# philgzl/brever

Hardware: AMD Instinct MI355X
Metric: utterances/sec (4 s @16 kHz) Conv-TasNet train (higher is better)
Workload: dtype bf16

## Files before the change

brever_amd/csrc/convtasnet.hip:

```cpp
#include <hip/hip_runtime.h>
#include <stdio.h>
#include <stdlib.h>
#include <string.h>
#include <algorithm>
#include <string>
#include <vector>

#include "../../include/brever_hip.h"
#include "status.h"
#include "ctn_layout.h"
#include "gemm_rows.cuh"
#include "gemm_wgrad.cuh"
#include "gemm_ws.cuh"
#include "dwpw2_fused.cuh"
#include "gemm_wgrad_full.cuh"
#include "gemm_wgrad_full128.cuh"

constexpr int kWgSplit = 4;
#include "prep.cuh"
#include "tcn_kernels.cuh"
#include "bwd_fused.cuh"
#include "pw1_bwd.cuh"
#include "cln_kernels.cuh"

using namespace brv;

namespace {

inline long long align_up(long long x, long long a) { return (x + a - 1)/a*a; }

const brv_launch_opts kDefaultOpts = {sizeof(brv_launch_opts), 0u, 8, 0, nullptr};
thread_local const brv_launch_opts* t_opts = &kDefaultOpts;
struct OptsScope {
  const brv_launch_opts* prev;
  explicit OptsScope(const brv_launch_opts* o) : prev(t_opts) {
    t_opts = (o && o->size >= sizeof(brv_launch_opts)) ? o : &kDefaultOpts;
  }
  ~OptsScope() { t_opts = prev; }
  int check() const {
    const uint32_t unknown = t_opts->flags & ~BRV_OPT_KNOWN;
    if (!unknown) return 0;
    char bits[16]; snprintf(bits, sizeof(bits), "0x%x", unknown);
    return fail(-1, std::string("unknown option bits ") + bits + " in brv_launch_opts.flags");
  }
};
inline bool opt(uint32_t flag) { return (t_opts->flags & flag) != 0; }
inline bool fwd_fuse_requested() { return !opt(BRV_OPT_NO_FWD_FUSE) && !opt(BRV_OPT_NO_WS); }
inline bool bwd_fuse_requested() { return !opt(BRV_OPT_NO_BWD_FUSE); }
inline bool pw1_rc_requested() { return !opt(BRV_OPT_NO_PW1_RC) && !opt(BRV_OPT_NO_DZ1_FUSE); }
inline bool pw1_rc_wgrad() { return opt(BRV_OPT_PW1_RC_WGRAD) || opt(BRV_OPT_PW1_RC_TILES); }

struct ProfEntry { const char* label; hipEvent_t a, b; double flops, bytes; };
struct Prof { std::vector<ProfEntry> entries; bool by_dil; };
struct ProfScope {
  hipStream_t st; Prof* prof;
  ProfScope(const char* label, double flops, double bytes, hipStream_t s)
      : st(s), prof(static_cast<Prof*>(t_opts->prof)) {
    if (!prof) return;
    ProfEntry e; e.label = label; e.flops = flops; e.bytes = bytes;
    (void)hipEventCreate(&e.a); (void)hipEventCreate(&e.b);
    (void)hipEventRecord(e.a, st);
    prof->entries.push_back(e);
  }
  ~ProfScope() { if (prof) (void)hipEventRecord(prof->entries.back().b, st); }
};
inline bool prof_by_dil() { return t_opts->prof && static_cast<Prof*>(t_opts->prof)->by_dil; }

struct BlockOff : CtnBlockOff {
  long long p_c1_f, p_c1_b, p_rs_f, p_rs_b;
  long long p_c1_fp, p_rs_fp, p_rs_bp;
  long long p_rs_g, p_rs_gp, p_lazy;
};

struct Layout : CtnLayout<BlockOff> {
  int Np, Kfp, Bnp, Hp, Scp;
  long long p_enc, p_dec_f, p_dec_b, p_bott_f, p_bott_b, p_out_f, p_out_b, p_stamp, n_prepared;

  bool fusable() const {
    return !causal && P == 3 && H == 512 && Bn == 128 && Sc == 128 && nb <= 24 ;
  }
  bool fused_fwd() const { return fusable() && fwd_fuse_requested(); }
  bool pw1_rc() const { return !causal && Hp == RC_H && Bnp == RC_N && pw1_rc_requested(); }

  static int limits(const brv_ctn_config* c) {
    return c->kernel_size < 1 || c->kernel_size > 5 ? fail(-2, "kernel_size must be in [1, 5] in the HIP path") : 0;
  }
  int init(const brv_ctn_config* c) {
    if (int r = CtnLayout::init(c, limits)) return r;
    Np = round_up(N, 64); Kfp = round_up(K, 64); Bnp = round_up(Bn, 64);
    Hp = round_up(H, 64); Scp = round_up(Sc, 64);
    long long q = 0;
    auto ptake = [&](long long n) { long long r = q; q += align_up(n, 128); return r; };
    p_enc = ptake((long long)Np*Kfp);
    p_dec_f = ptake((long long)Kfp*Np);
    p_dec_b = ptake((long long)Np*Kfp);
    p_bott_f = ptake((long long)Bnp*Np);
    p_bott_b = ptake((long long)Np*Bnp);
    for (int i = 0; i < nb; ++i) {
      const int rs = (i < nb - 1 ? Bnp : 0) + Scp;
      blk[i].p_c1_f = ptake((long long)Hp*Bnp);
      blk[i].p_c1_b = ptake((long long)Bnp*Hp);
      blk[i].p_rs_f = ptake((long long)rs*Hp);
      blk[i].p_rs_b = ptake((long long)Hp*rs);
      blk[i].p_c1_fp = ptake((long long)Hp*Bnp);
      blk[i].p_rs_fp = ptake((long long)rs*Hp);
      blk[i].p_rs_bp = ptake((long long)Hp*rs);
      blk[i].p_rs_g = ptake((long long)(Bnp + Scp)*Hp);
      blk[i].p_rs_gp = ptake((long long)(Bnp + Scp)*Hp);
      blk[i].p_lazy = ptake(4LL*(Bnp + Scp));
    }
    p_out_f = ptake((long long)S*Np*Scp);
    p_out_b = ptake((long long)Scp*S*Np);
    p_stamp = ptake(128);
    n_prepared = q;
    return 0;
  }
};

struct Workspace {
  long long w, x, z1, z2, skip, m, y, stats, sums, dpre, dw1, gskip, gout, eA, eB,
      e0, dwt, vg, gcopy, total;
  long long gcopy_stride, eB_stride;
  long long wgpart;
  long long h1, h2, wn, ctab, ctab_stride, cfs, cbt, ident, fake_stats, scratch_stats;
  long long vg_stride, vg_bytes;
  long long x_stride, z_stride;
  long long u, u_stride;
  long long stamp;
  long long stats_bytes;
  void init(const Layout& l, long long B, long long T) {
    long long o = 0;
    auto take = [&](long long bytes) { long long r = o; o += align_up(bytes, 256); return r; };
    const long long BT = B*T;
    w = take(BT*l.Np*2);
    x_stride = align_up(BT*l.Bnp*2, 256);
    x = take(x_stride*l.nb);
    z_stride = align_up(BT*l.Hp*2, 256);
    z1 = take(z_stride*l.nb);
    z2 = take(z_stride*l.nb);
    skip = take(BT*l.Scp*4);
    m = take(BT*l.S*l.Np*2);
    y = take(BT*l.S*l.Np*2);
    stats_bytes = (long long)(1 + 2*l.nb)*B*kStatStride*8;
    stats = take(stats_bytes);
    sums = take(stats_bytes);
    dpre = take(BT*l.S*l.Np*2);
    dw1 = take(BT*l.S*l.Np*2);
    gout = take(BT*(l.Bnp + l.Scp)*2);
    gskip = gout + (long long)l.Bnp*2;
    eA = take(BT*l.Hp*2);
    eB_stride = align_up(BT*l.Hp*2, 256);
    eB = take(eB_stride*l.nb);
    gcopy_stride = align_up(BT*l.Bnp*2, 256);
    gcopy = take(gcopy_stride*l.nb);
    e0 = take(BT*l.Np*2);
    dwt = take(BT*l.Np*2);
    vg_stride = align_up(2LL*l.N + (long long)l.nb*l.H*(5 + l.P) + 1 + 2*l.nb + 2LL*l.Hp, 64);
    vg_bytes = vg_stride*kReplicas*4;
    vg = take(vg_bytes);
    wgpart = take((long long)2*kWgSplit*l.nb*W2_G*l.H*4);
    u_stride = align_up(BT*(l.Bnp + l.Scp)*2, 256);
    u = l.fusable() ? take(u_stride*l.nb) : 0;
    stamp = take(256);
    h1 = h2 = wn = ctab = cfs = cbt = ident = fake_stats = scratch_stats = 0; ctab_stride = 0;
    if (l.causal) {
      h1 = take(z_stride*l.nb);
      h2 = take(z_stride*l.nb);
      wn = take(BT*l.Np*2);
      ctab_stride = align_up(BT*2*4, 256);
      ctab = take(ctab_stride*(1 + 2*l.nb));
      cfs = take(BT*2*4);
      cbt = take(BT*2*4);
      const long long cmax = l.Hp > l.Np ? l.Hp : l.Np;
      ident = take((2*cmax + 64)*4);
      fake_stats = take(B*kStatStride*8);
      scratch_stats = take(B*kStatStride*8);
    }
    total = o;
  }
};

struct Views {
  const Layout& l; Workspace ws; char* base; const bf16_t* prep; int B; long long T;
  Views(const Layout& l_, void* workspace, const void* prepared, int B_, long long T_)
      : l(l_), base((char*)workspace), prep((const bf16_t*)prepared), B(B_), T(T_) { ws.init(l, B, T); }
  double BT() const { return (double)B*(double)T; }
  int ldg() const { return l.Bnp + l.Scp; }
  bf16_t* bf(long long off) const { return (bf16_t*)(base + off); }
  float* f32(long long off) const { return (float*)(base + off); }
  double* stat(int i) const { return (double*)(base + ws.stats) + (long long)i*B*kStatStride; }
  double* sum(int i) const { return (double*)(base + ws.sums) + (long long)i*B*kStatStride; }
  bf16_t* w() const { return bf(ws.w); }
  bf16_t* x(int i) const { return bf(ws.x + ws.x_stride*i); }
  bf16_t* z1(int i) const { return bf(ws.z1 + ws.z_stride*i); }
  bf16_t* z2(int i) const { return bf(ws.z2 + ws.z_stride*i); }
  bf16_t* u(int i) const { return bf(ws.u + ws.u_stride*i); }
  float* skip() const { return f32(ws.skip); }
  bf16_t* m() const { return bf(ws.m); }
  bf16_t* y() const { return bf(ws.y); }
  bf16_t* dpre() const { return bf(ws.dpre); }
  bf16_t* dw1() const { return bf(ws.dw1); }
  bf16_t* gskip() const { return bf(ws.gskip); }
  bf16_t* gout() const { return bf(ws.gout); }
  bf16_t* eA() const { return bf(ws.eA); }
  bf16_t* eB(int i) const { return bf(ws.eB + ws.eB_stride*i); }
  bf16_t* gcopy(int i) const { return bf(ws.gcopy + ws.gcopy_stride*i); }
  bf16_t* e0() const { return bf(ws.e0); }
  bf16_t* dwt() const { return bf(ws.dwt); }
  float* vg() const { return f32(ws.vg); }
  float* vslot(int i) const { return vg() + 2LL*l.N + (long long)l.H*(5 + l.P)*i; }
  float* vslope() const { return vslot(l.nb); }
  float* vscratch() const { return vslope() + 1 + 2*l.nb; }
  bf16_t* wn() const { return bf(ws.wn); }
  bf16_t* h1(int i) const { return bf(ws.h1 + ws.z_stride*i); }
  bf16_t* h2(int i) const { return bf(ws.h2 + ws.z_stride*i); }
  long long cmax() const { return l.Hp > l.Np ? l.Hp : l.Np; }
  float* ones() const { return f32(ws.ident); }
  float* zeros() const { return ones() + cmax(); }
  float* one() const { return zeros() + cmax(); }
  double* fake_stats() const { return (double*)(base + ws.fake_stats); }
  double* scratch_stats() const { return (double*)(base + ws.scratch_stats); }
  float* cfs() const { return f32(ws.cfs); }
  float* cbt() const { return f32(ws.cbt); }
  float* tab(int i) const { return f32(ws.ctab + ws.ctab_stride*i); }
};

template <int BN, int AK, int EM>
int launch_gemm_rows_t(const GemmRowsParams& p0, int batch, hipStream_t st) {
  GemmRowsParams p = p0;
  p.n_ttiles = ceil_div(p.T, GR_BM); p.n_ntiles = ceil_div(p.Np, BN); p.batch = batch;
  dim3 grid(p.n_ttiles*p.n_ntiles*batch);
  hipLaunchKernelGGL((gemm_rows_kernel<BN, AK, EM>), grid, dim3(256), 0, st, p);
  BRV_HIP_OK(hipGetLastError());
  return 0;
}

#ifdef BRV_DIAG
__global__ void diag_stamp_kernel(long long* out, int slot) {
  const long long t = stamp_realtime();
  if (threadIdx.x == 0) {
    out[slot] = t;
    if (slot == 0) { out[2] = 0x7fffffffffffffffLL; out[3] = 0; }
  }
}
long long* debug_buffer() {
  static long long* buf = nullptr;
  if (!buf) {
    if (hipMalloc(&buf, 1 << 20) != hipSuccess) return nullptr;
    (void)hipMemset(buf, 0, 1 << 20);
  }
  return buf;
}
#endif

inline int mode_stamp(bool fused_fwd) { return fused_fwd ? 0x46555345 : 0x504c4149; }
__global__ void stamp_write_kernel(int* dst, int value) { *dst = value; }
__global__ void stamp_check_f64_kernel(const int* stamp, int expect, double* poison, long long n) {
  if (*stamp == expect) return;
  const double nan = __longlong_as_double(0x7ff8000000000000LL);
  for (long long i = threadIdx.x; i < n; i += blockDim.x) poison[i] = nan;
}
struct CallInitParams {
  double* a; long long a_n; void* b; long long b_bytes;
  const int* check; int expect; int* write; int value;
};
__global__ __launch_bounds__(256) void call_init_kernel(const CallInitParams p) {
  const bool bad = *p.check != p.expect;
  const double fill = bad ? __longlong_as_double(0x7ff8000000000000LL) : 0.0;
  const long long tid = (long long)blockIdx.x*256 + threadIdx.x, nth = (long long)gridDim.x*256;
  for (long long i = tid; i < p.a_n; i += nth) p.a[i] = fill;
  if (p.b) {
    unsigned char* b = (unsigned char*)p.b;
    long long head = (16 - ((unsigned long long)b & 15)) & 15;
    if (head > p.b_bytes) head = p.b_bytes;
    const long long n16 = (p.b_bytes - head) >> 4, tail0 = head + (n16 << 4);
    uint4* mid = reinterpret_cast<uint4*>(b + head);
    const uint4 z = make_uint4(0, 0, 0, 0);
    for (long long i = tid; i < n16; i += nth) mid[i] = z;
    for (long long i = tid*4; i < head; i += nth*4) *reinterpret_cast<unsigned int*>(b + i) = 0u;
    for (long long i = tail0 + tid*4; i < p.b_bytes; i += nth*4) *reinterpret_cast<unsigned int*>(b + i) = 0u;
  }
  if (tid == 0 && p.write) *p.write = p.value;
}
inline int launch_call_init(double* a, long long a_n, void* b, long long b_bytes, const int* check, int expect,
                            int* write, int value, hipStream_t st) {
  CallInitParams ip; ip.a = a; ip.a_n = a_n; ip.b = b; ip.b_bytes = b_bytes; ip.check = check; ip.expect = expect;
  ip.write = write; ip.value = value;
  const long long units = a_n + (b_bytes >> 4);
  int gx = (int)std::min<long long>(512, (units + 1023)/1024);
  if (gx < 1) gx = 1;
  hipLaunchKernelGGL(call_init_kernel, dim3(gx), dim3(256), 0, st, ip);
  BRV_HIP_OK(hipGetLastError());
  return 0;
}

int device_cus() {
  static const int n = [] {
    int dev = 0, v = 0;
    if (hipGetDevice(&dev) != hipSuccess ||
        hipDeviceGetAttribute(&v, hipDeviceAttributeMultiprocessorCount, dev) != hipSuccess || v <= 0)
      v = 256;
    return v;
  }();
  return n;
}
int num_cus() {
  const int n = device_cus();
  const int e = t_opts->cu_eighths >= 1 && t_opts->cu_eighths <= 8 ? t_opts->cu_eighths : 8;
  const int m = n*e/8/8*8;
  return m >= 8 ? m : n;
}

template <int KP, int NSL, int WM, int EM, int AT, bool CAT, int NW = 8>
int launch_gemm_ws(const GemmRowsParams& p0, int batch, hipStream_t st) {
  using C = GemmWsCfg<KP, NSL, WM, NW>;
  GemmRowsParams p = p0;
  p.batch = batch;
#ifdef BRV_DIAG
  if (const char* d = getenv("BRV_DBG")) p.dbg = atoi(d);
  if (p.dbg & (64 | 512)) p.dbg_out = debug_buffer();
#endif
  if (!CAT && p.a.K0 <= 0) {
    p.a.p0 = p.a.p1; p.a.ld0 = p.a.ld1; p.a.bs0 = p.a.bs1; p.a.K0 = 1 << 30;
  }
  const int total = ceil_div(p.T, C::BMW)*batch;
  const int groups = p.Np / C::NP;
  int grid = (NW == 8 ? num_cus() : 2*num_cus())/groups;
  if (grid > total) grid = total;
  if (grid < 1) grid = 1;
#ifdef BRV_DIAG
  if (p.dbg & 512) hipLaunchKernelGGL(diag_stamp_kernel, dim3(1), dim3(64), 0, st, debug_buffer() + 131000, 0);
#endif
  hipLaunchKernelGGL((gemm_ws_kernel<KP, NSL, WM, EM, AT, CAT, NW>), dim3(grid, groups),
                     dim3(64*NW), 0, st, p);
#ifdef BRV_DIAG
  if (p.dbg & 512) hipLaunchKernelGGL(diag_stamp_kernel, dim3(1), dim3(64), 0, st, debug_buffer() + 131000, 1);
#endif
  BRV_HIP_OK(hipGetLastError());
  return 0;
}

template <int AK, int EM>
int launch_gemm_rows(const GemmRowsParams& p, int batch, hipStream_t st,
                     const char* label = "gemm_rows", double bytes = 0) {
  if (p.T <= 0 || batch <= 0) return 0;
  ProfScope prof(label, 2.0*batch*p.T*(double)p.Np*p.Kp, bytes, st);
  if (AK == A_BF16 && p.a.nsrc <= 1 && !opt(BRV_OPT_NO_WS)) {
    const bool plain = p.a.slope == nullptr && p.a.stats == nullptr;
    const bool full = p.a.slope != nullptr && p.a.stats != nullptr;
    const bool one_src = p.a.K0 >= p.Kp || p.a.K0 <= 0;
    if ((EM == E_STORE || EM == E_GLN_BWD) && p.Kp == 128 && p.Np == 512 && plain && one_src)
      return launch_gemm_ws<128, 64, 1, (EM == E_STORE ? E_STORE : E_GLN_BWD), 0, false, 8>(p, batch, st);
    if (EM == E_RES_SKIP && p.Kp == 512 && p.Np == 256 && full && one_src)
      return launch_gemm_ws<512, 32, 1, E_RES_SKIP, 1, false>(p, batch, st);
    if (EM == E_GLN_BWD && p.Kp == 256 && p.Np == 512 && plain && one_src)
      return launch_gemm_ws<256, 32, 1, E_GLN_BWD, 0, false, 8>(p, batch, st);
  }
  if (p.Kp % GR_BK != 0 || p.Np % 64 != 0) return fail(-1, "gemm_rows: unpadded dims");
  if (p.Np % 128 == 0) return launch_gemm_rows_t<128, AK, EM>(p, batch, st);
  return launch_gemm_rows_t<64, AK, EM>(p, batch, st);
}

inline int wgrad_target(const char* label, int dflt) {
  (void)label;
  return t_opts->wg_target != 0 ? t_opts->wg_target : dflt;
}

template <int BH, int HK>
int launch_wgrad_t(WgradGroupParams& gp, hipStream_t st, int target) {
  WgradParams& p = gp.base;
  const int nprob = gp.nprob > 0 ? gp.nprob : 1;
  const int tiles = ceil_div(p.Gp, WG_BG)*(p.Hp/BH);
  const int total = p.B*ceil_div(p.T, WG_BT);
  int ns = ceil_div(target > 0 ? target : 384, tiles*nprob);
  if (target < 0) {
    int nb = p.B;
    while (tiles*nprob*nb > 2048 && nb % 2 == 0) nb /= 2;
    if (nb > ns) ns = nb;
  }
  if (ns > total) ns = total;
  if (ns < 1) ns = 1;
  p.nsplit = ns;
  dim3 grid(tiles, ns, nprob);
  hipLaunchKernelGGL((gemm_wgrad_kernel<BH, HK>), grid, dim3(256), 0, st, gp);
  BRV_HIP_OK(hipGetLastError());
  return 0;
}
template <int HK>
int launch_wgrad_group(WgradGroupParams& gp, hipStream_t st, const char* label,
                       double bytes, int target_dflt = 384) {
  const WgradParams& p = gp.base;
  if (p.T <= 0 || p.B <= 0) return 0;
  const int nprob = gp.nprob > 0 ? gp.nprob : 1;
  ProfScope prof(label, 2.0*nprob*p.B*p.T*(double)p.Gp*p.Hp, bytes*nprob, st);
  if (p.Hp % 64 != 0) return fail(-1, "wgrad: unpadded dims");
  const int target = wgrad_target(label, target_dflt);
  if (p.Hp % 128 == 0) return launch_wgrad_t<128, HK>(gp, st, target);
  return launch_wgrad_t<64, HK>(gp, st, target);
}
template <int HK>
int launch_wgrad(WgradParams& p, hipStream_t st, const char* label = "wgrad",
                 double bytes = 0, int target_dflt = 384) {
  WgradGroupParams gp;
  gp.base = p; gp.nprob = 0;
  return launch_wgrad_group<HK>(gp, st, label, bytes, target_dflt);
}

template <template <int> class F, typename... Args>
int dispatch_p(int P, Args&&... args) {
  switch (P) {
    case 1: return F<1>::run(args...);
    case 2: return F<2>::run(args...);
    case 3: return F<3>::run(args...);
    case 4: return F<4>::run(args...);
    case 5: return F<5>::run(args...);
  }
  return fail(-2, "unsupported kernel_size");
}
template <int P> struct DwFwd {
  static int run(const DwParams& p, hipStream_t st) {
    ProfScope prof("dwconv_fwd", 2.0*P*p.B*p.T*(double)p.Cp, 4.0*p.B*p.T*(double)p.Cp, st);
    dim3 grid(ceil_div(p.T, DW_TT_F)*p.B);
    hipLaunchKernelGGL((dwconv_fwd_kernel<P>), grid, dim3(256), 0, st, p);
    BRV_HIP_OK(hipGetLastError());
    return 0;
  }
};
template <int P> struct DwBwd {
  static int run(const DwParams& p, hipStream_t st) {
    if (p.z2in != nullptr) {
      static const char* by_dil[9] = {"dwconv_bwd_d1", "dwconv_bwd_d2", "dwconv_bwd_d4", "dwconv_bwd_d8", "dwconv_bwd_d16",
                                      "dwconv_bwd_d32", "dwconv_bwd_d64", "dwconv_bwd_d128", "dwconv_bwd_dx"};
      int lg = 0; while ((1 << lg) < p.dil && lg < 8) ++lg;
      ProfScope prof(prof_by_dil() ? by_dil[lg] : "dwconv_bwd", 4.0*P*p.B*p.T*(double)p.Cp, 8.0*p.B*p.T*(double)p.Cp, st);
      const int R = hl_rows_per_tooth(p.dil), K = HL_TT/R;
      const int tiles = ceil_div(p.dil, R)*ceil_div((p.T - 1)/p.dil + 1, K);
      dim3 grid(tiles*p.B*(p.Cp/HL_CG));
      const size_t lds = (size_t)hl_window_rows(p.dil, P)*HL_CG*2;
      hipLaunchKernelGGL((dwconv_bwd_halo_kernel<P>), grid, dim3(256), lds, st, p);
      BRV_HIP_OK(hipGetLastError());
      return 0;
    }
    ProfScope prof("dwconv_bwd", 4.0*P*p.B*p.T*(double)p.Cp, 6.0*p.B*p.T*(double)p.Cp, st);
    dim3 grid(ceil_div(p.T, DW_TT_B)*p.B);
    hipLaunchKernelGGL((dwconv_bwd_kernel<P>), grid, dim3(256), 0, st, p);
    BRV_HIP_OK(hipGetLastError());
    return 0;
  }
};

template <int P> struct DwBwdFused {
  static int run(const BwdFusedParams& p0, hipStream_t st) {
    BwdFusedParams p = p0;
    const DwParams& d = p.d;
#ifdef BF_STAMP
    p.dbg = debug_buffer();
#endif
    bf_tile_shape(d.T, d.dil, P, p.K, p.R);
    const int tiles = ceil_div(d.dil, p.R)*ceil_div((d.T - 1)/d.dil + 1, p.K);
    static const char* by_dil[9] = {"dwpw2_bwd_d1", "dwpw2_bwd_d2", "dwpw2_bwd_d4", "dwpw2_bwd_d8", "dwpw2_bwd_d16",
                                    "dwpw2_bwd_d32", "dwpw2_bwd_d64", "dwpw2_bwd_d128", "dwpw2_bwd_dx"};
    int lg = 0; while ((1 << lg) < d.dil && lg < 8) ++lg;
    ProfScope prof(prof_by_dil() ? by_dil[lg] : "dwpw2_bwd", 2.0*d.B*d.T*(double)d.Cp*(p.Kg + 2*P),
                   2.0*d.B*d.T*((double)p.Kg + 3.0*d.Cp), st);
    dim3 grid(ceil_div(tiles*d.B, 8)*8*(d.Cp/HL_CG));
    if (d.C != d.Cp) return fail(-1, "fused backward: channel count must be a multiple of 64");
    if (p.Kg == 256) hipLaunchKernelGGL((dwconv_bwd_fused_kernel<P, 256>), grid, dim3(256), BF_LDS, st, p);
    else if (p.Kg == 128) hipLaunchKernelGGL((dwconv_bwd_fused_kernel<P, 128>), grid, dim3(256), BF_LDS, st, p);
    else return fail(-1, "fused backward: unexpected [res | skip] width");
    BRV_HIP_OK(hipGetLastError());
    return 0;
  }
};

int launch_dz(const DzParams& p, hipStream_t st) {
  ProfScope prof("gln_prelu_bwd", 0, 6.0*p.B*p.T*(double)p.Cp, st);
  const long long per_item = (long long)p.T*(p.Cp/8);
  int gx = (int)((per_item + 256*8 - 1)/(256*8));
  const int cap = 1024/p.B > 1 ? 1024/p.B : 1;
  if (gx > cap) gx = cap;
  if (gx < 1) gx = 1;
  hipLaunchKernelGGL(dz_kernel, dim3(gx, p.B), dim3(256), 0, st, p);
  BRV_HIP_OK(hipGetLastError());
  return 0;
}

ASpec rows_bf16(const void* ptr, int ld, long long T) {
  ASpec a; memset(&a, 0, sizeof(a));
  a.p0 = ptr; a.ld0 = ld; a.bs0 = T*ld; a.K0 = 1 << 30; a.nsrc = 1;
  return a;
}
void set_affine(ASpec& a, const double* stats, const float* g, const float* b, int C,
                long long T) {
  a.stats = stats; a.gamma = g; a.beta = b; a.C = C;
  a.inv_n = 1.0/((double)T*(double)C); a.eps = 1e-8f;
}
ASpec frames_of(const float* wav, long long L, int hop, int K, long long stride = 0) {
  ASpec a; memset(&a, 0, sizeof(a));
  a.p0 = wav; a.hop = hop; a.Kf = K; a.wav_stride = stride > 0 ? stride : L; a.wav_len = (int)L;
  a.K0 = 1 << 30; a.nsrc = 1;
  return a;
}

struct PrepJobC { int src_off, dst_off, scale_off; unsigned short R, C, rows, cols, dst_ld, tr; };
constexpr int kPrepBatch = 168;
struct PrepBatch { PrepJobC jobs[kPrepBatch]; int n; };
static_assert(sizeof(PrepBatch) <= 4096, "kernel argument size");

struct PackJob { long long src_off, dst_off; int N, K, nsl; };
struct PackBatch { PackJob jobs[96]; int n; };
__global__ __launch_bounds__(256) void pack_frag_kernel(bf16_t* prepared, const PackBatch pb) {
  const PackJob j = pb.jobs[blockIdx.y];
  const long long total = (long long)j.N*j.K/8;
  const int KS = j.K/16;
  for (long long i = (long long)blockIdx.x*256 + threadIdx.x; i < total; i += (long long)gridDim.x*256) {
    const int n = (int)(i / (j.K/8)), k = (int)(i % (j.K/8))*8;
    const int slice = n / j.nsl, f = (n % j.nsl)/32, fr = n % 32, s = k/16, fh = (k % 16)/8;
    const long long dst = (long long)slice*j.nsl*j.K + ((long long)(f*KS + s)*64 + fr + 32*fh)*8;
    *reinterpret_cast<uint4*>(prepared + j.dst_off + dst) =
        *reinterpret_cast<const uint4*>(prepared + j.src_off + (long long)n*j.K + k);
  }
}
__global__ __launch_bounds__(256) void prep_weights_kernel(const float* params,
                                                           bf16_t* prepped,
                                                           const PrepBatch pb) {
  const PrepJobC& c = pb.jobs[blockIdx.y];
  PrepJob j;
  j.src_off = c.src_off; j.dst_off = c.dst_off; j.scale_off = c.scale_off;
  j.R = c.R; j.C = c.C; j.rows = c.rows; j.cols = c.cols; j.dst_ld = c.dst_ld; j.tr = c.tr;
  prep_job_run(params, prepped, j, blockIdx.x, gridDim.x);
}

struct LazyPrepBlk { long long res_w, res_b, skip_w, skip_b, beta, wg, out; };
struct LazyPrepParams {
  int nb, H, Hp, Bn, Sc, Bnp, Scp;
  int* stamp; int stamp_value;
  LazyPrepBlk blk[kWgMaxProb];
};
__global__ __launch_bounds__(256) void lazy_prep_kernel(const float* params, bf16_t* prepped,
                                                        const LazyPrepParams p) {
  const LazyPrepBlk& b = p.blk[blockIdx.y];
  float* out = reinterpret_cast<float*>(prepped + b.out);
  const int NP = p.Bnp + p.Scp;
  const int n = blockIdx.x*4 + (threadIdx.x >> 6), lane = threadIdx.x & 63;
  if (blockIdx.x == 0 && blockIdx.y == 0 && threadIdx.x == 0) *p.stamp = p.stamp_value;
  if (n >= NP) return;
  const bool res = n < p.Bnp;
  const int r = res ? n : n - p.Bnp;
  const bool ok = res ? (r < p.Bn && b.res_w >= 0) : r < p.Sc;
  float v0 = 0.f, v1 = 0.f;
  if (ok) {
    const float* W = params + (res ? b.res_w : b.skip_w) + (long long)r*p.H;
    const bf16_t* wg = prepped + b.wg + (long long)n*p.Hp;
    for (int k = lane; k < p.H; k += 64) {
      v0 = __builtin_fmaf(W[k], params[b.beta + k], v0);
      v1 += bf2f(wg[k]);
    }
  }
  for (int o = 32; o; o >>= 1) { v0 += __shfl_xor(v0, o); v1 += __shfl_xor(v1, o); }
  if (lane == 0) {
    out[n] = ok ? v0 + params[(res ? b.res_b : b.skip_b) + r] : 0.f;
    out[NP + n] = v1;
  }
}

struct SkipCombineParams {
  const bf16_t* u; long long u_stride;
  const double* stats; long long stats_stride;
  const bf16_t* prepared; long long lazy_off[kWgMaxProb];
  float* skip; int nb, B, T, Bnp, Scp; double inv_n; float eps;
};
__global__ __launch_bounds__(256) void skip_combine_kernel(const SkipCombineParams p) {
  __shared__ float rs[kWgMaxProb];
  __shared__ float cs[128];
  const int b = blockIdx.y, tid = threadIdx.x;
  const int NP = p.Bnp + p.Scp;
  __shared__ float ms[kWgMaxProb];
  for (int i = tid; i < p.nb; i += 256) {
    const NormStat ns = norm_stat(p.stats + (2 + 2*i)*p.stats_stride, b, p.inv_n, p.eps);
    rs[i] = ns.rstd; ms[i] = ns.mean*ns.rstd;
  }
  __syncthreads();
  for (int n = tid; n < p.Scp; n += 256) {
    float c = 0.f;
    int i = 0;
    for (; i + 8 <= p.nb; i += 8) {
      float a[8], v[8];
#pragma unroll
      for (int k = 0; k < 8; ++k) {
        const float* lz = reinterpret_cast<const float*>(p.prepared + p.lazy_off[i + k]);
        a[k] = lz[p.Bnp + n]; v[k] = lz[NP + p.Bnp + n];
      }
#pragma unroll
      for (int k = 0; k < 8; ++k) c += a[k] - ms[i + k]*v[k];
    }
    for (; i < p.nb; ++i) {
      const float* lz = reinterpret_cast<const float*>(p.prepared + p.lazy_off[i]);
      c += lz[p.Bnp + n] - ms[i]*lz[NP + p.Bnp + n];
    }
    cs[n] = c;
  }
  __syncthreads();
  const int cpr = p.Scp/8;
  const long long per_item = (long long)p.T*cpr;
  for (long long e = (long long)blockIdx.x*256 + tid; e < per_item; e += (long long)gridDim.x*256) {
    const int c0 = (int)(e % cpr)*8; const long long t = e / cpr;
    float acc[8];
#pragma unroll
    for (int j = 0; j < 8; ++j) acc[j] = cs[c0 + j];
    const bf16_t* src = p.u + ((long long)b*p.T + t)*NP + p.Bnp + c0;
    int i = 0;
    for (; i + 8 <= p.nb; i += 8) {
      uint4 q[8];
#pragma unroll
      for (int k = 0; k < 8; ++k) q[k] = *reinterpret_cast<const uint4*>(src + (i + k)*p.u_stride);
#pragma unroll
      for (int k = 0; k < 8; ++k) {
        float f[8];
        unpack8(q[k], f);
        const float r = rs[i + k];
#pragma unroll
        for (int j = 0; j < 8; ++j) acc[j] = __builtin_fmaf(r, f[j], acc[j]);
      }
    }
    for (; i < p.nb; ++i) {
      float f[8];
      unpack8(*reinterpret_cast<const uint4*>(src + i*p.u_stride), f);
      const float r = rs[i];
#pragma unroll
      for (int j = 0; j < 8; ++j) acc[j] = __builtin_fmaf(r, f[j], acc[j]);
    }
    float* dst = p.skip + ((long long)b*p.T + t)*p.Scp + c0;
    *reinterpret_cast<float4*>(dst) = make_float4(acc[0], acc[1], acc[2], acc[3]);
    *reinterpret_cast<float4*>(dst + 4) = make_float4(acc[4], acc[5], acc[6], acc[7]);
  }
}

}

int reduce_vector_grads(const Views& v, float* grads, hipStream_t st, int blk_lo = 0, int blk_hi = 1 << 30,
                        bool do_ln = true, bool do_tcn = true) {
  const Layout& l = v.l;
  const long long vper = (long long)l.H*(5 + l.P);
  {
    VgradParams vp; memset(&vp, 0, sizeof(vp));
    vp.vg = v.vg(); vp.grads = grads; vp.rep_stride = v.ws.vg_stride;
    vp.N = l.N; vp.H = l.H; vp.P = l.P; vp.nb = l.nb;
    vp.ln_g_off = l.ln_g; vp.blk0_off = l.blk[0].conv_w;
    vp.blk_full = l.nb > 1 ? l.blk[1].conv_w - l.blk[0].conv_w : 0;
    const BlockOff& b0 = l.blk[0];
    const BlockOff& bl = l.blk[l.nb - 1];
    vp.o_dconv_w = b0.dconv_w - b0.conv_w; vp.o_dconv_b = b0.dconv_b - b0.conv_w;
    vp.o_n1_g_full = b0.n1_g - b0.conv_w; vp.o_n1_g_last = bl.n1_g - bl.conv_w;
    vp.tcn_prelu_off = l.tcn_prelu;
    vp.blk_lo = blk_lo; vp.blk_hi = blk_hi; vp.do_ln = do_ln; vp.do_tcn = do_tcn;
    if (b0.prelu1 != b0.n1_g + 4LL*l.H || b0.prelu2 != b0.prelu1 + 1)
      return fail(-1, "vgrad_reduce: unexpected PReLU offsets");
    const long long total = 2LL*l.N + vper*l.nb + 1 + 2*l.nb;
    int gx = (int)((total + 255)/256);
    if (gx > 1024) gx = 1024;
    ProfScope prof("vgrad_reduce", 0, 4.0*total*(kReplicas + 2), st);
    hipLaunchKernelGGL(vgrad_reduce_kernel, dim3(gx), dim3(256), 0, st, vp);
    BRV_HIP_OK(hipGetLastError());
  }
  return 0;
}

__global__ void fill_identity_kernel(float* ones, float* zeros, float* one, int n,
                                     double* fake_stats, int B, double sumsq) {
  const int i = blockIdx.x*256 + threadIdx.x;
  if (i < n) { ones[i] = 1.f; zeros[i] = 0.f; }
  if (i == 0) *one = 1.f;
  if (i < B) { fake_stats[stat_sum(i)] = 0.0; fake_stats[stat_sq(i)] = sumsq; }
}

namespace {

int causal_init(const Views& v, hipStream_t st) {
  const Layout& l = v.l;
  const double sumsq = (1.0 - (double)1e-8f)*(double)v.T*(double)l.H;
  const int cmax = (int)v.cmax(), n = cmax > v.B ? cmax : v.B;
  hipLaunchKernelGGL(fill_identity_kernel, dim3((n + 255)/256), dim3(256), 0, st, v.ones(), v.zeros(),
                     v.one(), cmax, v.fake_stats(), v.B, sumsq);
  BRV_HIP_OK(hipGetLastError());
  BRV_HIP_OK(hipMemsetAsync(v.scratch_stats(), 0, (size_t)v.B*kStatStride*8, st));
  return 0;
}

int cln_forward(const Views& v, const bf16_t* z, const float* slope, const float* gain,
                const float* bias, bf16_t* y, float* table, int B, long long T, int Cp, int C,
                hipStream_t st) {
  ClnParams p; memset(&p, 0, sizeof(p));
  p.z = z; p.slope = slope; p.y = y; p.fsum = v.cfs(); p.table = table; p.gain = gain;
  p.bias = bias; p.B = B; p.T = (int)T; p.Cp = Cp; p.C = C; p.eps = 1e-8f;
  ProfScope prof("cln_fwd", 0, 6.0*B*T*(double)Cp, st);
  hipLaunchKernelGGL(cln_frame_sums_kernel, dim3(ceil_div((int)T, CLN_FPB)*B), dim3(256), 0, st, p);
  hipLaunchKernelGGL(cln_scan_kernel, dim3(B), dim3(256), 0, st, p);
  int gx = (int)(((long long)B*T*(Cp/8) + 255)/256);
  if (gx > 4096) gx = 4096;
  hipLaunchKernelGGL(cln_apply_kernel, dim3(gx), dim3(256), 0, st, p);
  BRV_HIP_OK(hipGetLastError());
  return 0;
}

int cln_backward(const Views& v, const bf16_t* g, const bf16_t* z, const float* slope,
                 const float* gain, const float* fwd_table, bf16_t* dz, const bf16_t* add_in,
                 int n_add, float* dgain, float* dbias, float* dslope, long long rep_stride,
                 int B, long long T, int Cp, int C, hipStream_t st) {
  ClnParams p; memset(&p, 0, sizeof(p));
  p.z = z; p.slope = slope; p.g = g; p.fsum = v.cfs(); p.table = v.cbt(); p.fwd_table = fwd_table;
  p.gain = gain; p.B = B; p.T = (int)T; p.Cp = Cp; p.C = C; p.eps = 1e-8f;
  p.dz = dz; p.add_in = add_in; p.n_add = n_add;
  p.dgain = dgain; p.dbias = dbias; p.dslope = dslope; p.rep_stride = rep_stride;
  ProfScope prof("cln_bwd", 0, 10.0*B*T*(double)Cp, st);
  hipLaunchKernelGGL(cln_bwd_sums_kernel, dim3(ceil_div((int)T, CLN_FPB)*B), dim3(256), 0, st, p);
  hipLaunchKernelGGL(cln_bwd_scan_kernel, dim3(B), dim3(256), 0, st, p);
  int gx = (int)(((long long)B*T*(Cp/8) + 255)/256);
  if (gx > 2048) gx = 2048;
  hipLaunchKernelGGL(cln_bwd_apply_kernel, dim3(gx), dim3(256), 0, st, p);
  BRV_HIP_OK(hipGetLastError());
  return 0;
}

int forward_encoder(const Views& v, const float* params, const float* wave, long long wave_stride, float* out,
                    long long L, hipStream_t st) {
  const Layout& l = v.l; const int B = v.B; const long long T = v.T; const double BT = v.BT();
  if (int r = launch_call_init(v.stat(0), (long long)(v.ws.stats_bytes/8), out, (long long)B*l.S*L*(long long)sizeof(float),
                               reinterpret_cast<const int*>(v.prep + l.p_stamp), mode_stamp(l.fused_fwd()),
                               reinterpret_cast<int*>(v.base + v.ws.stamp), mode_stamp(l.fused_fwd()), st))
    return fail(r, "forward: call_init launch");

  GemmRowsParams g;
  memset(&g, 0, sizeof(g));
  g.a = frames_of(wave, L, l.hop, l.K, wave_stride);
  g.W = v.prep + l.p_enc; g.T = (int)T; g.Np = l.Np; g.Kp = l.Kfp;
  g.e.out = v.w(); g.e.ldo = l.Np; g.e.N = l.N; g.e.stats_out = v.stat(0);
  if (int r = launch_gemm_rows<A_FRAMES, E_STORE>(g, B, st, "enc_fwd", 4.0*B*L + 2.0*BT*l.Np)) return r;
  memset(&g, 0, sizeof(g));
  g.a = rows_bf16(v.w(), l.Np, T);
  set_affine(g.a, v.stat(0), params + l.ln_g, params + l.ln_b, l.N, T);
  g.W = v.prep + l.p_bott_f; g.T = (int)T; g.Np = l.Bnp; g.Kp = l.Np;
  g.e.out = v.x(0); g.e.ldo = l.Bnp; g.e.bias = params + l.bott_b; g.e.N = l.Bn;
  if (int r = launch_gemm_rows<A_BF16, E_STORE>(g, B, st, "bottleneck_fwd", 2.0*BT*(l.Np + l.Bnp))) return r;
  return 0;
}

int forward_block_fused(const Views& v, const float* params, int i, hipStream_t st) {
  const Layout& l = v.l; const int B = v.B; const long long T = v.T; const double BT = v.BT();
  const int NPu = l.Bnp + l.Scp;
  GemmRowsParams g;
  const BlockOff& b = l.blk[i];
  const int dil = 1 << (i % l.layers);
  memset(&g, 0, sizeof(g));
  g.W = v.prep + b.p_c1_f; g.T = (int)T; g.Np = l.Hp; g.Kp = l.Bnp;
  g.Wp = v.prep + b.p_c1_fp; g.wp_nsl = 64;
  g.e.out = v.z1(i); g.e.ldo = l.Hp; g.e.bias = params + b.conv_b; g.e.N = l.H;
  g.e.stats_out = v.stat(1 + 2*i); g.e.stats_slope = params + b.prelu1;
  if (i == 0) {
    g.a = rows_bf16(v.x(0), l.Bnp, T);
    ProfScope prof("pw1_fwd", 2.0*BT*l.Hp*l.Bnp, 2.0*BT*(l.Bnp + l.Hp), st);
    if (int r = launch_gemm_ws<128, 64, 1, E_STORE, 0, false, 8>(g, B, st)) return r;
  } else {
    const BlockOff& pb = l.blk[i - 1];
    g.a = rows_bf16(v.x(i - 1), l.Bnp, T);
    g.a.p1 = v.u(i - 1); g.a.ld1 = NPu; g.a.bs1 = T*NPu;
    g.a.xout = v.x(i);
    g.a.stats = v.stat(2 + 2*(i - 1)); g.a.inv_n = 1.0/((double)T*l.H); g.a.eps = 1e-8f;
    const float* lz = reinterpret_cast<const float*>(v.prep + pb.p_lazy);
    g.a.lazy_v0 = lz; g.a.lazy_v1 = lz + NPu;
    ProfScope prof("pw1_fwd", 2.0*BT*l.Hp*l.Bnp, 2.0*BT*(3*l.Bnp + l.Hp), st);
#ifndef PW1F_NSL
#define PW1F_NSL 64
#define PW1F_WM 1
#endif
    if (int r = launch_gemm_ws<128, PW1F_NSL, PW1F_WM, E_STORE, 2, false, 8>(g, B, st)) return r;
  }
  memset(&g, 0, sizeof(g));
  g.a = rows_bf16(v.z1(i), l.Hp, T);
  g.a.slope = params + b.prelu1; g.a.stats = v.stat(1 + 2*i);
  g.a.gamma = params + b.n1_g; g.a.beta = params + b.n1_b; g.a.C = l.H;
  g.a.inv_n = 1.0/((double)T*l.H); g.a.eps = 1e-8f;
  g.a.z2out = v.z2(i); g.a.taps = params + b.dconv_w; g.a.dbias = params + b.dconv_b;
  g.a.slope2 = params + b.prelu2; g.a.stats2_out = v.stat(2 + 2*i);
  g.a.dil = dil; g.a.left = ((l.P - 1)*dil)/2;
  g.W = v.prep + b.p_rs_g; g.Wp = v.prep + b.p_rs_gp; g.wp_nsl = 32;
  g.T = (int)T; g.Np = NPu; g.Kp = l.Hp;
  g.e.out = v.u(i); g.e.ldo = NPu; g.e.N = NPu;
  {
    ProfScope prof("dwpw2_fwd", 2.0*BT*l.Hp*(NPu + l.P), 2.0*BT*(2*l.Hp + NPu), st);
    const bool old_stage = opt(BRV_OPT_DWPW2_WS);
    if (old_stage || l.Hp != DP_H || NPu != DP_N) {
      if (int r = launch_gemm_ws<512, 32, 1, E_STORE, 3, false, 8>(g, B, st)) return r;
    } else {
      DwPw2Params dp; memset(&dp, 0, sizeof(dp));
      dp.z1 = v.z1(i); dp.z2 = v.z2(i); dp.u = v.u(i);
      dp.Wp = v.prep + b.p_rs_gp;
      dp.slope1 = params + b.prelu1; dp.slope2 = params + b.prelu2;
      dp.stats1 = v.stat(1 + 2*i); dp.stats2 = v.stat(2 + 2*i);
      dp.gamma1 = params + b.n1_g; dp.beta1 = params + b.n1_b;
      dp.taps = params + b.dconv_w; dp.dbias = params + b.dconv_b;
      dp.B = B; dp.T = (int)T; dp.dil = dil; dp.left = ((l.P - 1)*dil)/2; dp.C = l.H;
      dp.inv_n = 1.0/((double)T*l.H); dp.eps = 1e-8f;
      const int n_tiles = B*(int)((T + DP_TT - 1)/DP_TT);
      const int cap = num_cus() >= 8 ? num_cus()/8*8 : 8;
      const int n_wg = n_tiles < cap ? (n_tiles + 7)/8*8 : cap;
      hipLaunchKernelGGL(dwpw2_fused_kernel, dim3(n_wg), dim3(512), 0, st, dp);
      BRV_HIP_OK(hipGetLastError());
    }
  }
  return 0;
}

int forward_skip_combine(const Views& v, hipStream_t st) {
  const Layout& l = v.l; const int B = v.B; const long long T = v.T; const double BT = v.BT();
  SkipCombineParams sc; memset(&sc, 0, sizeof(sc));
  sc.u = v.u(0); sc.u_stride = v.ws.u_stride/2; sc.stats = v.stat(0); sc.stats_stride = (long long)B*kStatStride;
  sc.prepared = v.prep; sc.skip = v.skip(); sc.nb = l.nb; sc.B = B; sc.T = (int)T; sc.Bnp = l.Bnp; sc.Scp = l.Scp;
  sc.inv_n = 1.0/((double)T*l.H); sc.eps = 1e-8f;
  for (int i = 0; i < l.nb; ++i) sc.lazy_off[i] = l.blk[i].p_lazy;
  {
    ProfScope prof("skip_combine", 0, 2.0*BT*l.Scp*l.nb + 4.0*BT*l.Scp, st);
    int gx = (int)((T*(l.Scp/8) + 255)/256);
    if (gx > 128) gx = 128;
    hipLaunchKernelGGL(skip_combine_kernel, dim3(gx, B), dim3(256), 0, st, sc);
    BRV_HIP_OK(hipGetLastError());
  }
  return 0;
}

int forward_block_plain(const Views& v, const float* params, int i, hipStream_t st) {
  const Layout& l = v.l; const int B = v.B; const long long T = v.T; const double BT = v.BT();
  GemmRowsParams g;
  const BlockOff& b = l.blk[i];
  const bool has_res = i < l.nb - 1;
  const int dil = 1 << (i % l.layers);
  memset(&g, 0, sizeof(g));
  g.a = rows_bf16(v.x(i), l.Bnp, T);
  g.W = v.prep + b.p_c1_f; g.T = (int)T; g.Np = l.Hp; g.Kp = l.Bnp;
  g.Wp = v.prep + b.p_c1_fp; g.wp_nsl = 64;
  g.e.out = v.z1(i); g.e.ldo = l.Hp; g.e.bias = params + b.conv_b; g.e.N = l.H;
  g.e.stats_out = v.stat(1 + 2*i); g.e.stats_slope = params + b.prelu1;
  if (int r = launch_gemm_rows<A_BF16, E_STORE>(g, B, st, "pw1_fwd", 2.0*BT*(l.Bnp + l.Hp))) return r;
  DwParams d; memset(&d, 0, sizeof(d));
  d.z1 = v.z1(i); d.z2 = v.z2(i); d.B = B; d.T = (int)T; d.Cp = l.Hp; d.C = l.H;
  d.slope1 = params + b.prelu1; d.stats1 = v.stat(1 + 2*i);
  d.gamma1 = params + b.n1_g; d.beta1 = params + b.n1_b;
  d.inv_n = 1.0/((double)T*l.H); d.eps = 1e-8f;
  d.taps = params + b.dconv_w; d.bias = params + b.dconv_b;
  d.dil = dil; d.left = ((l.P - 1)*dil)/2;
  d.stats2 = v.stat(2 + 2*i); d.slope2 = params + b.prelu2;
  if (int r = dispatch_p<DwFwd>(l.P, d, st)) return r;
  memset(&g, 0, sizeof(g));
  g.a = rows_bf16(v.z2(i), l.Hp, T);
  g.a.slope = params + b.prelu2;
  set_affine(g.a, v.stat(2 + 2*i), params + b.n2_g, params + b.n2_b, l.H, T);
  const int rs0 = has_res ? l.Bnp : 0;
  g.W = v.prep + b.p_rs_f; g.T = (int)T; g.Np = rs0 + l.Scp; g.Kp = l.Hp;
  g.Wp = v.prep + b.p_rs_fp; g.wp_nsl = 32;
  g.e.out = has_res ? v.x(i + 1) : nullptr; g.e.ldo = l.Bnp;
  g.e.bias = has_res ? params + b.res_b : nullptr; g.e.N = has_res ? l.Bn : 0;
  g.e.Nsplit = rs0; g.e.bias2 = params + b.skip_b; g.e.N2 = l.Sc;
  g.e.res_in = v.x(i); g.e.ld_res = l.Bnp;
  g.e.skip = v.skip(); g.e.ld_skip = l.Scp; g.e.skip_init = (i == 0);
  if (int r = launch_gemm_rows<A_BF16, E_RES_SKIP>(g, B, st, "pw2_fwd", 2.0*BT*(l.Hp + l.Bnp + rs0) + 4.0*BT*l.Scp*(i == 0 ? 1 : 2))) return r;
  return 0;
}

int forward_decoder(const Views& v, const float* params, float* out, long long L, hipStream_t st) {
  const Layout& l = v.l; const int B = v.B; const long long T = v.T; const double BT = v.BT();
  GemmRowsParams g;
  memset(&g, 0, sizeof(g));
  g.a = rows_bf16(v.skip(), l.Scp, T);
  g.a.slope = params + l.tcn_prelu;
  g.W = v.prep + l.p_out_f; g.T = (int)T; g.Np = l.S*l.Np; g.Kp = l.Scp;
  g.e.out = v.y(); g.e.ldo = l.Np; g.e.bias = params + l.out_b; g.e.N = l.N;
  g.e.w_in = v.w(); g.e.ld_w = l.Np; g.e.m_out = v.m(); g.e.S = l.S; g.e.Np_src = l.Np;
  if (int r = launch_gemm_rows<A_F32, E_MASK>(g, B, st, "mask_fwd", 4.0*BT*l.Scp + 2.0*BT*l.Np*(1 + 2*l.S))) return r;
  memset(&g, 0, sizeof(g));
  g.a = rows_bf16(v.y(), l.Np, T);
  g.W = v.prep + l.p_dec_f; g.T = (int)T; g.Np = l.Kfp; g.Kp = l.Np;
  g.e.wave_out = out; g.e.hop = l.hop; g.e.Kf = l.K; g.e.wave_stride = L;
  g.e.wave_len = (int)L;
  if (int r = launch_gemm_rows<A_BF16, E_OLA>(g, B*l.S, st, "dec_fwd", 2.0*BT*l.S*l.Np + 4.0*B*l.S*L)) return r;
  return 0;
}

int forward_causal(const Views& v, const float* params, const float* wave, long long wave_stride, float* out,
                   long long L, hipStream_t st) {
  const Layout& l = v.l; const int B = v.B; const long long T = v.T; const double BT = v.BT();
  if (int r = causal_init(v, st)) return r;
  BRV_HIP_OK(hipMemsetAsync(out, 0, (size_t)B*l.S*L*sizeof(float), st));

  GemmRowsParams g;
  memset(&g, 0, sizeof(g));
  g.a = frames_of(wave, L, l.hop, l.K, wave_stride);
  g.W = v.prep + l.p_enc; g.T = (int)T; g.Np = l.Np; g.Kp = l.Kfp;
  g.e.out = v.w(); g.e.ldo = l.Np; g.e.N = l.N;
  if (int r = launch_gemm_rows<A_FRAMES, E_STORE>(g, B, st, "enc_fwd", 4.0*B*L + 2.0*BT*l.Np)) return r;
  if (int r = cln_forward(v, v.w(), nullptr, params + l.ln_g, params + l.ln_b, v.wn(), v.tab(0), B, T,
                          l.Np, l.N, st)) return r;
  memset(&g, 0, sizeof(g));
  g.a = rows_bf16(v.wn(), l.Np, T);
  g.W = v.prep + l.p_bott_f; g.T = (int)T; g.Np = l.Bnp; g.Kp = l.Np;
  g.e.out = v.x(0); g.e.ldo = l.Bnp; g.e.bias = params + l.bott_b; g.e.N = l.Bn;
  if (int r = launch_gemm_rows<A_BF16, E_STORE>(g, B, st, "bottleneck_fwd", 2.0*BT*(l.Np + l.Bnp))) return r;

  for (int i = 0; i < l.nb; ++i) {
    const BlockOff& b = l.blk[i];
    const bool has_res = i < l.nb - 1;
    const int dil = 1 << (i % l.layers);
    memset(&g, 0, sizeof(g));
    g.a = rows_bf16(v.x(i), l.Bnp, T);
    g.W = v.prep + b.p_c1_f; g.T = (int)T; g.Np = l.Hp; g.Kp = l.Bnp;
    g.e.out = v.z1(i); g.e.ldo = l.Hp; g.e.bias = params + b.conv_b; g.e.N = l.H;
    if (int r = launch_gemm_rows<A_BF16, E_STORE>(g, B, st, "pw1_fwd", 2.0*BT*(l.Bnp + l.Hp))) return r;
    if (int r = cln_forward(v, v.z1(i), params + b.prelu1, params + b.n1_g, params + b.n1_b,
                            v.h1(i), v.tab(1 + 2*i), B, T, l.Hp, l.H, st)) return r;
    DwParams d; memset(&d, 0, sizeof(d));
    d.z1 = v.h1(i); d.z2 = v.z2(i); d.B = B; d.T = (int)T; d.Cp = l.Hp; d.C = l.H;
    d.slope1 = v.one(); d.stats1 = v.fake_stats(); d.gamma1 = v.ones(); d.beta1 = v.zeros();
    d.inv_n = 1.0/((double)T*l.H); d.eps = 1e-8f;
    d.taps = params + b.dconv_w; d.bias = params + b.dconv_b;
    d.dil = dil; d.left = (l.P - 1)*dil;
    d.stats2 = v.scratch_stats(); d.slope2 = v.one();
    if (int r = dispatch_p<DwFwd>(l.P, d, st)) return r;
    if (int r = cln_forward(v, v.z2(i), params + b.prelu2, params + b.n2_g, params + b.n2_b,
                            v.h2(i), v.tab(2 + 2*i), B, T, l.Hp, l.H, st)) return r;
    memset(&g, 0, sizeof(g));
    g.a = rows_bf16(v.h2(i), l.Hp, T);
    const int rs0 = has_res ? l.Bnp : 0;
    g.W = v.prep + b.p_rs_f; g.T = (int)T; g.Np = rs0 + l.Scp; g.Kp = l.Hp;
    g.e.out = has_res ? v.x(i + 1) : nullptr; g.e.ldo = l.Bnp;
    g.e.bias = has_res ? params + b.res_b : nullptr; g.e.N = has_res ? l.Bn : 0;
    g.e.Nsplit = rs0; g.e.bias2 = params + b.skip_b; g.e.N2 = l.Sc;
    g.e.res_in = v.x(i); g.e.ld_res = l.Bnp;
    g.e.skip = v.skip(); g.e.ld_skip = l.Scp; g.e.skip_init = (i == 0);
    if (int r = launch_gemm_rows<A_BF16, E_RES_SKIP>(g, B, st, "pw2_fwd", 2.0*BT*(l.Hp + l.Bnp + rs0) + 4.0*BT*l.Scp*(i == 0 ? 1 : 2))) return r;
  }
  return forward_decoder(v, params, out, L, st);
}

void wgrad_rs_prob(const Views& v, const float* params, float* grads, int i, WgradProb& pr) {
  const BlockOff& b = v.l.blk[i];
  const bool has_res = i < v.l.nb - 1;
  pr.g0 = has_res ? v.gcopy(i) : nullptr; pr.g1 = v.gskip(); pr.h = v.z2(i);
  pr.out0 = has_res ? grads + b.res_w : nullptr; pr.out1 = grads + b.skip_w;
  pr.gbias0 = has_res ? grads + b.res_b : nullptr; pr.gbias1 = grads + b.skip_b;
  pr.slope = params + b.prelu2; pr.stats = v.stat(2 + 2*i);
  pr.gamma = params + b.n2_g; pr.beta = params + b.n2_b;
}

int wgrad_rs_full(const Views& v, const float* params, float* grads, int blk_lo, int blk_hi, hipStream_t st) {
  const Layout& l = v.l; const int B = v.B; const long long T = v.T; const double BT = v.BT();
  const int ldg = v.ldg();
  WgradFullParams fp; memset(&fp, 0, sizeof(fp));
  const int nblk = blk_hi - blk_lo + 1;
  fp.B = B; fp.T = (int)T; fp.nprob = nblk; fp.n_htiles = l.Hp/W2_BH;
  fp.ldg0 = l.Bnp; fp.bsg0 = T*l.Bnp; fp.ldg1 = ldg; fp.bsg1 = T*ldg;
  fp.ldh = l.Hp; fp.bsh = T*l.Hp;
  fp.N0 = l.Bn; fp.N1 = l.Sc; fp.Kout = l.H; fp.ldo = l.H;
  fp.inv_n = 1.0/((double)T*l.H); fp.eps = 1e-8f;
  for (int i = blk_lo; i <= blk_hi; ++i) wgrad_rs_prob(v, params, grads, i, fp.prob[i - blk_lo]);
  ProfScope prof("pw2_wgrad", 2.0*nblk*BT*(double)(l.Bnp + l.Scp)*l.Hp,
                 2.0*BT*(l.Bnp + l.Scp + l.Hp)*nblk, st);
#ifdef BRV_DIAG
  if (const char* d = getenv("BRV_DBG_WG")) fp.dbg = atoi(d);
#endif
  fp.n_split = (B >= kWgSplit && !opt(BRV_OPT_NO_WGRAD_SPLIT)) ? kWgSplit : 1;
  fp.part = reinterpret_cast<float*>(v.base + v.ws.wgpart);
  const bool wide = !opt(BRV_OPT_NO_WGRAD_128) && l.Hp % W3_BH == 0;
  if (wide) {
    fp.n_htiles = l.Hp/W3_BH;
    if (fp.n_split > 1 && B >= 4*kWgSplit) fp.n_split = 2*kWgSplit;
    const int grid = 8*ceil_div(nblk, 8)*fp.n_htiles*fp.n_split;
    hipLaunchKernelGGL(wgrad_full128_kernel, dim3(grid), dim3(64*W2_NW), 0, st, fp);
  } else {
    const int grid = 8*ceil_div(nblk, 8)*fp.n_htiles*fp.n_split;
    hipLaunchKernelGGL(wgrad_full_kernel, dim3(grid), dim3(64*W2_NW), 0, st, fp);
  }
  if (fp.n_split > 1)
    hipLaunchKernelGGL(wgrad_full_reduce_kernel, dim3(128, (unsigned)nblk), dim3(256), 0, st, fp);
  BRV_HIP_OK(hipGetLastError());
  return 0;
}

int wgrad_rs_grouped(const Views& v, const float* params, float* grads, int i0, int n, hipStream_t st) {
  const Layout& l = v.l; const int B = v.B; const long long T = v.T; const double BT = v.BT();
  const int ldg = v.ldg(); WgradParams wg;
  WgradGroupParams gp; memset(&gp, 0, sizeof(gp));
  WgradParams& q = gp.base;
  q.g = rows_bf16(nullptr, l.Bnp, T); q.g.K0 = l.Bnp;
  q.g.ld1 = ldg; q.g.bs1 = T*ldg;
  q.h = rows_bf16(nullptr, l.Hp, T);
  set_affine(q.h, nullptr, nullptr, nullptr, l.H, T);
  q.B = B; q.T = (int)T; q.Gp = l.Bnp + l.Scp; q.Hp = l.Hp;
  q.G0p = l.Bnp; q.N0 = l.Bn; q.N1 = l.Sc; q.Kout = l.H; q.ldo = l.H;
  int np = 0;
  for (int i = i0; i < i0 + n; ++i)
    if (i != l.nb - 1) wgrad_rs_prob(v, params, grads, i, gp.prob[np++]);
  gp.nprob = np;
  if (np > 0)
    if (int r = launch_wgrad_group<A_BF16>(gp, st, "pw2_wgrad",
                                           2.0*BT*(l.Bnp + l.Scp + l.Hp))) return r;
  if (i0 + n == l.nb) {
    const BlockOff& b = l.blk[l.nb - 1];
    memset(&wg, 0, sizeof(wg));
    wg.g = rows_bf16(v.gskip(), ldg, T);
    wg.h = rows_bf16(v.z2(l.nb - 1), l.Hp, T); wg.h.slope = params + b.prelu2;
    set_affine(wg.h, v.stat(2 + 2*(l.nb - 1)), params + b.n2_g, params + b.n2_b, l.H, T);
    wg.B = B; wg.T = (int)T; wg.Gp = l.Scp; wg.Hp = l.Hp;
    wg.out1 = grads + b.skip_w; wg.G0p = 0; wg.N0 = 0; wg.N1 = l.Sc;
    wg.Kout = l.H; wg.ldo = l.H; wg.gbias1 = grads + b.skip_b;
    if (int r = launch_wgrad<A_BF16>(wg, st, "pw2_wgrad", 2.0*BT*(l.Scp + l.Hp))) return r;
  }
  return 0;
}

int wgrad_pw1(const Views& v, const float* params, float* grads, int i0, int n, hipStream_t st) {
  const Layout& l = v.l; const int B = v.B; const long long T = v.T; const double BT = v.BT();
  WgradGroupParams gp;
  memset(&gp, 0, sizeof(gp));
  WgradParams& q1 = gp.base;
  q1.g = rows_bf16(nullptr, l.Hp, T); q1.h = rows_bf16(nullptr, l.Bnp, T);
  q1.B = B; q1.T = (int)T; q1.Gp = l.Hp; q1.Hp = l.Bnp;
  q1.G0p = l.Hp; q1.N0 = l.H; q1.Kout = l.Bn; q1.ldo = l.Bn;
  for (int i = i0; i < i0 + n; ++i) {
    const BlockOff& b = l.blk[i];
    WgradProb& pr = gp.prob[i - i0];
    pr.g0 = v.eB(i); pr.h = v.x(i);
    pr.out0 = grads + b.conv_w; pr.gbias0 = grads + b.conv_b;
  }
  gp.nprob = n;
  if (l.pw1_rc() && pw1_rc_wgrad()) {
    Pw1WgradRcParams rp; memset(&rp, 0, sizeof(rp));
    rp.B = B; rp.T = (int)T; rp.nprob = n; rp.C = l.H; rp.Kout = l.Bn; rp.ldo = l.Bn;
    rp.lde = l.Hp; rp.ldx = l.Bnp; rp.bse = T*l.Hp; rp.bsx = T*l.Bnp;
    rp.inv_n = 1.0/((double)T*l.H); rp.eps = 1e-8f;
    for (int i = i0; i < i0 + n; ++i) {
      const BlockOff& b = l.blk[i];
      Pw1WgradRcProb& pr = rp.prob[i - i0];
      pr.e1 = v.eB(i); pr.x = v.x(i); pr.Wfp = v.prep + b.p_c1_fp; pr.bias = params + b.conv_b;
      pr.out = grads + b.conv_w; pr.gbias = grads + b.conv_b;
      pr.stats = v.stat(1 + 2*i); pr.sums = v.sum(1 + 2*i); pr.slope = params + b.prelu1;
    }
    const int tiles = l.Hp/WG_BG;
    int ns = B;
    while (tiles*n*ns > 2048 && ns % 2 == 0) ns /= 2;
    if (t_opts->wg_target > 0) ns = ceil_div(t_opts->wg_target, tiles*n);
    const int total = B*ceil_div((int)T, WG_BT);
    if (ns > total) ns = total;
    if (ns < 1) ns = 1;
    rp.nsplit = ns;
    ProfScope prof("pw1_wgrad", 2.0*n*BT*(double)l.Hp*l.Bnp*2, 2.0*BT*(l.Hp + l.Bnp)*n, st);
    hipLaunchKernelGGL(pw1_wgrad_rc_kernel, dim3(tiles, ns, n), dim3(256), 0, st, rp);
    BRV_HIP_OK(hipGetLastError());
  }
  else
  if (int r = launch_wgrad_group<A_BF16>(gp, st, "pw1_wgrad", 2.0*BT*(l.Hp + l.Bnp), -1))
    return r;
  return 0;
}

int deferred_wgrads(const Views& v, const float* params, float* grads, int blk_lo, int blk_hi, hipStream_t st) {
  const Layout& l = v.l;
  const bool full_rs = l.Bnp == 128 && l.Scp == 128 && l.Hp % W2_BH == 0 && l.nb <= kWgMaxProb &&
                       !opt(BRV_OPT_NO_WGRAD_FULL);
  if (full_rs && blk_lo <= blk_hi)
    if (int r = wgrad_rs_full(v, params, grads, blk_lo, blk_hi, st)) return r;
  for (int i0 = blk_lo; i0 <= blk_hi; i0 += kWgMaxProb) {
    const int n = std::min(kWgMaxProb, blk_hi + 1 - i0);
    if (!full_rs)
      if (int r = wgrad_rs_grouped(v, params, grads, i0, n, st)) return r;
    if (int r = wgrad_pw1(v, params, grads, i0, n, st)) return r;
  }
  return 0;
}

int backward_head(const Views& v, const float* params, const float* d_out, float* grads, long long L,
                  bool bwd_fused, hipStream_t st) {
  const Layout& l = v.l; const int B = v.B; const long long T = v.T; const double BT = v.BT();
  const int BS = B*l.S, ldg = v.ldg(); GemmRowsParams g; WgradParams wg;
  if (!l.causal)
    if (int r = launch_call_init(v.sum(0), (long long)(v.ws.stats_bytes/8), v.vg(), (long long)v.ws.vg_bytes,
                                 reinterpret_cast<const int*>(v.base + v.ws.stamp), mode_stamp(l.fused_fwd()), nullptr, 0, st))
      return fail(r, "backward: call_init launch");
  memset(&g, 0, sizeof(g));
  g.a = frames_of(d_out, L, l.hop, l.K);
  g.W = v.prep + l.p_dec_b; g.T = (int)T; g.Np = l.Np; g.Kp = l.Kfp;
  g.e.out = v.dpre(); g.e.ldo = l.Np; g.e.out2 = v.dw1(); g.e.w_in = v.w(); g.e.ld_w = l.Np;
  g.e.m_in = v.m(); g.e.S = l.S;
  if (int r = launch_gemm_rows<A_FRAMES, E_MASK_BWD>(g, BS, st, "dec_bwd", 4.0*BS*L + 2.0*BT*l.Np*(1 + 3*l.S))) return r;
  memset(&wg, 0, sizeof(wg));
  wg.g = rows_bf16(v.y(), l.Np, T); wg.h = frames_of(d_out, L, l.hop, l.K);
  wg.B = BS; wg.T = (int)T; wg.Gp = l.Np; wg.Hp = l.Kfp;
  wg.out0 = grads + l.dec_w; wg.G0p = l.Np; wg.N0 = l.N; wg.Kout = l.K; wg.ldo = l.K;
  if (int r = launch_wgrad<A_FRAMES>(wg, st, "wgrad_dec", 2.0*BT*l.S*l.Np + 4.0*BS*L, l.causal ? 384 : 768)) return r;
  memset(&g, 0, sizeof(g));
  g.a = rows_bf16(v.dpre(), l.Np, T); g.a.nsrc = l.S;
  g.W = v.prep + l.p_out_b; g.T = (int)T; g.Np = l.Scp; g.Kp = l.S*l.Np;
  g.e.out = v.gskip(); g.e.ldo = ldg; g.e.src_f32 = v.skip(); g.e.ld_srcf = l.Scp;
  g.e.src_slope = params + l.tcn_prelu; g.e.dslope = v.vslope();
  g.e.rep_stride = v.ws.vg_stride; g.e.n_rep = kReplicas;
  if (int r = launch_gemm_rows<A_BF16, E_PRELU_BWD>(g, B, st, "mask_bwd", 2.0*BT*l.S*l.Np + 6.0*BT*l.Scp)) return r;
  if (bwd_fused) {
    GuDotsParams gu; memset(&gu, 0, sizeof(gu));
    gu.g = v.gskip(); gu.ldg = ldg; gu.u = v.u(l.nb - 1) + l.Bnp; gu.ldu = ldg;
    gu.v1 = reinterpret_cast<const float*>(v.prep + l.blk[l.nb - 1].p_lazy) + ldg + l.Bnp;
    gu.ncols = l.Scp; gu.B = B; gu.T = (int)T; gu.out = v.sum(2 + 2*(l.nb - 1));
    ProfScope prof("gu_dots", 0, 4.0*BT*l.Scp, st);
    int gx = (int)((T*(l.Scp/8) + 255)/256);
    if (gx > 64) gx = 64;
    hipLaunchKernelGGL(gu_dots_kernel, dim3(gx, B), dim3(256), 0, st, gu);
    BRV_HIP_OK(hipGetLastError());
  }
  for (int s = 0; s < l.S; ++s) {
    memset(&wg, 0, sizeof(wg));
    wg.g = rows_bf16(v.dpre() + (long long)s*T*l.Np, l.Np, T); wg.g.bs0 = (long long)l.S*T*l.Np;
    wg.h = rows_bf16(v.skip(), l.Scp, T); wg.h.slope = params + l.tcn_prelu;
    wg.B = B; wg.T = (int)T; wg.Gp = l.Np; wg.Hp = l.Scp;
    wg.out0 = grads + l.out_w + (long long)s*l.N*l.Sc; wg.G0p = l.Np; wg.N0 = l.N;
    wg.Kout = l.Sc; wg.ldo = l.Sc; wg.gbias0 = grads + l.out_b + (long long)s*l.N;
    if (int r = launch_wgrad<A_F32>(wg, st, "wgrad_out", 2.0*BT*l.Np + 4.0*BT*l.Scp, l.causal ? 384 : 256)) return r;
  }
  return 0;
}

int backward_block_dw(const Views& v, const float* params, int i, bool bwd_fused, hipStream_t st) {
  const Layout& l = v.l; const int B = v.B; const long long T = v.T; const double BT = v.BT();
  const int ldg = v.ldg(); GemmRowsParams g;
  const BlockOff& b = l.blk[i];
  const bool has_res = i < l.nb - 1;
  const int dil = 1 << (i % l.layers);
  const int rs0 = has_res ? l.Bnp : 0;
  const bool blk_fused = bwd_fused && (((l.P - 1)*dil)/2) % dil == 0;
  if (!blk_fused) {
    memset(&g, 0, sizeof(g));
    g.a = rows_bf16(has_res ? v.gout() : v.gskip(), ldg, T);
    g.W = v.prep + b.p_rs_b; g.T = (int)T; g.Np = l.Hp; g.Kp = rs0 + l.Scp;
    g.Wp = v.prep + b.p_rs_bp; g.wp_nsl = 32;
    g.e.out = v.eA(); g.e.ldo = l.Hp; g.e.N = l.H;
    g.e.src = v.z2(i); g.e.ld_src = l.Hp; g.e.src_slope = params + b.prelu2;
    g.e.src_stats = v.stat(2 + 2*i); g.e.inv_n = 1.0/((double)T*l.H); g.e.eps = 1e-8f;
    g.e.gamma = params + b.n2_g;
    g.e.dgamma = v.vslot(i) + 2*l.H; g.e.dbeta = v.vslot(i) + 3*l.H;
    g.e.rep_stride = v.ws.vg_stride; g.e.n_rep = kReplicas;
    g.e.sums_out = v.sum(2 + 2*i);
    if (int r = launch_gemm_rows<A_BF16, E_GLN_BWD>(g, B, st, "pw2_dgrad", 2.0*BT*(rs0 + l.Scp + 2*l.Hp))) return r;
  }
  const bool fuse_dz2 = blk_fused || (!opt(BRV_OPT_NO_DZ_FUSE) && l.Hp % HL_CG == 0 &&
                        (((l.P - 1)*dil)/2) % dil == 0 && hl_window_rows(dil, l.P) <= HL_MAXROWS);
  DzParams dz; memset(&dz, 0, sizeof(dz));
  if (!fuse_dz2) {
    dz.e = v.eA(); dz.z = v.z2(i); dz.B = B; dz.T = (int)T; dz.Cp = l.Hp; dz.C = l.H;
    dz.slope = params + b.prelu2; dz.stats = v.stat(2 + 2*i); dz.sums = v.sum(2 + 2*i);
    dz.inv_n = 1.0/((double)T*l.H); dz.eps = 1e-8f; dz.dslope = v.vslope() + 2 + 2*i; dz.rep_stride = v.ws.vg_stride;
    if (int r = launch_dz(dz, st)) return r;
  }
  DwParams d; memset(&d, 0, sizeof(d));
  bf16_t* eB = v.eB(i);
  d.z1 = v.z1(i); d.dz2 = v.eA(); d.e1 = eB; d.B = B; d.T = (int)T; d.Cp = l.Hp; d.C = l.H;
  d.slope1 = params + b.prelu1; d.stats1 = v.stat(1 + 2*i);
  d.gamma1 = params + b.n1_g; d.beta1 = params + b.n1_b;
  d.inv_n = 1.0/((double)T*l.H); d.eps = 1e-8f;
  d.taps = params + b.dconv_w; d.dil = dil; d.left = ((l.P - 1)*dil)/2;
  d.dgamma1 = v.vslot(i); d.dbeta1 = v.vslot(i) + l.H;
  d.dtaps = v.vslot(i) + 4*l.H; d.dbias = v.vslot(i) + 4*l.H + (long long)l.H*l.P;
  d.rep_stride = v.ws.vg_stride; d.sums1 = v.sum(1 + 2*i);
  if (fuse_dz2) {
    d.z2in = v.z2(i); d.stats2 = v.stat(2 + 2*i); d.sums2 = v.sum(2 + 2*i);
    d.slope2 = params + b.prelu2; d.dslope2 = v.vslope() + 2 + 2*i;
  }
  if (blk_fused) {
    BwdFusedParams bf; memset(&bf, 0, sizeof(bf));
    bf.d = d; bf.d.dz2 = nullptr;
    bf.g = has_res ? v.gout() : v.gskip(); bf.ldg = ldg; bf.Kg = rs0 + l.Scp;
    bf.Wp = v.prep + b.p_rs_bp; bf.gamma2 = params + b.n2_g;
    bf.dgamma2 = v.vslot(i) + 2*l.H; bf.dbeta2 = v.vslot(i) + 3*l.H;
    if (int r = DwBwdFused<3>::run(bf, st)) return r;
  } else
  if (int r = dispatch_p<DwBwd>(l.P, d, st)) return r;
  return 0;
}

int backward_block_pw1_rc(const Views& v, const float* params, int i, const EpiSpec& e, bool bwd_fused,
                          hipStream_t st) {
  const Layout& l = v.l; const int B = v.B; const long long T = v.T; const double BT = v.BT();
  const BlockOff& b = l.blk[i];
  const bool has_res = i < l.nb - 1;
  bf16_t* eB = v.eB(i);
  Pw1DgradRcParams rp; memset(&rp, 0, sizeof(rp));
  rp.e1 = eB; rp.lde = l.Hp; rp.bse = T*l.Hp;
  rp.x = v.x(i); rp.ldx = l.Bnp; rp.bsx = T*l.Bnp;
  rp.Wfp = v.prep + b.p_c1_fp; rp.bias = params + b.conv_b; rp.Wb = v.prep + b.p_c1_b;
  rp.stats = v.stat(1 + 2*i); rp.sums = v.sum(1 + 2*i); rp.slope = params + b.prelu1;
  rp.inv_n = 1.0/((double)T*l.H); rp.eps = 1e-8f; rp.C = l.H;
  rp.T = (int)T; rp.n_ttiles = ceil_div((int)T, RC_BM); rp.batch = B;
  rp.e = e;
  rp.e.dslope = v.vslope() + 1 + 2*i; rp.e.rep_stride = v.ws.vg_stride; rp.e.n_rep = kReplicas;
  if (opt(BRV_OPT_PW1_RC_TILES)) {
    ProfScope prof("pw1_dgrad", 2.0*BT*(double)l.Hp*l.Bnp*2,
                   2.0*BT*(l.Hp + l.Bnp*(has_res ? 3 : 2)), st);
    hipLaunchKernelGGL(pw1_dgrad_rc_kernel, dim3(rp.n_ttiles*B), dim3(256), 0, st, rp);
  } else {
    Pw1DgradWsParams wp; wp.r = rp;
    wp.dz_out = pw1_rc_wgrad() ? nullptr : eB;
    wp.dbg = nullptr;
#ifdef WSD_STAMP
    wp.dbg = debug_buffer();
#endif
    const double companions = (i > 0 ? l.Bnp : 0) + (bwd_fused && i > 0 ? (double)l.Bnp + 2.0*l.Scp : 0.0);
    ProfScope prof("pw1_dgrad", 2.0*BT*(double)l.Hp*l.Bnp*2,
                   2.0*BT*(l.Hp*(wp.dz_out ? 2 : 1) + l.Bnp*(has_res ? 3 : 2) + companions), st);
    int grid = num_cus();
    const int total = ceil_div((int)T, WSD_TF)*B;
    if (grid > total) grid = total;
    if (l.H == RC_H) hipLaunchKernelGGL(pw1_dgrad_ws_kernel<true>, dim3(grid), dim3(512), 0, st, wp);
    else hipLaunchKernelGGL(pw1_dgrad_ws_kernel<false>, dim3(grid), dim3(512), 0, st, wp);
  }
  BRV_HIP_OK(hipGetLastError());
  return 0;
}

int backward_block_pw1(const Views& v, const float* params, int i, bool bwd_fused, hipStream_t st) {
  const Layout& l = v.l; const int B = v.B; const long long T = v.T; const double BT = v.BT();
  const BlockOff& b = l.blk[i];
  const bool has_res = i < l.nb - 1;
  const int ldg = v.ldg(); bf16_t* eB = v.eB(i); GemmRowsParams g; DzParams dz;
  const bool fuse_dz1 = !opt(BRV_OPT_NO_DZ1_FUSE) && (l.Bnp == 128 || l.Bnp == 64);
  if (!fuse_dz1) {
    memset(&dz, 0, sizeof(dz));
    dz.e = eB; dz.z = v.z1(i); dz.B = B; dz.T = (int)T; dz.Cp = l.Hp; dz.C = l.H;
    dz.slope = params + b.prelu1; dz.stats = v.stat(1 + 2*i); dz.sums = v.sum(1 + 2*i);
    dz.inv_n = 1.0/((double)T*l.H); dz.eps = 1e-8f; dz.dslope = v.vslope() + 1 + 2*i; dz.rep_stride = v.ws.vg_stride;
    if (int r = launch_dz(dz, st)) return r;
  }
  memset(&g, 0, sizeof(g));
  g.a = rows_bf16(eB, l.Hp, T);
  g.W = v.prep + b.p_c1_b; g.T = (int)T; g.Np = l.Bnp; g.Kp = l.Hp;
  g.e.out = v.gout(); g.e.ldo = ldg; g.e.add_in = has_res ? v.gout() : nullptr; g.e.ld_add = ldg;
  g.e.out2 = i > 0 ? v.gcopy(i - 1) : nullptr; g.e.ld_srcf = l.Bnp;
  if (bwd_fused && i > 0) {
    g.e.gu_u = v.u(i - 1); g.e.ld_gu = ldg; g.e.gu_gskip = v.gskip(); g.e.ld_gs = ldg;
    g.e.gu_v1 = reinterpret_cast<const float*>(v.prep + l.blk[i - 1].p_lazy) + ldg;
    g.e.gu_out = v.sum(2 + 2*(i - 1));
  }
  if (fuse_dz1 && l.pw1_rc()) return backward_block_pw1_rc(v, params, i, g.e, bwd_fused, st);
  if (fuse_dz1) {
    g.a.p1 = v.z1(i); g.a.ld1 = l.Hp; g.a.bs1 = T*l.Hp;
    g.a.slope = params + b.prelu1; g.a.stats = v.stat(1 + 2*i); g.a.sums = v.sum(1 + 2*i);
    g.a.inv_n = 1.0/((double)T*l.H); g.a.eps = 1e-8f; g.a.C = l.H;
    g.e.dslope = v.vslope() + 1 + 2*i; g.e.rep_stride = v.ws.vg_stride; g.e.n_rep = kReplicas;
    return launch_gemm_rows<A_DZ, E_ADD>(g, B, st, "pw1_dgrad", 2.0*BT*(3*l.Hp + l.Bnp*(has_res ? 2 : 1)));
  }
  return launch_gemm_rows<A_BF16, E_ADD>(g, B, st, "pw1_dgrad", 2.0*BT*(l.Hp + l.Bnp*(has_res ? 2 : 1)));
}

int backward_block(const Views& v, const float* params, int i, bool bwd_fused, hipStream_t st) {
  if (int r = backward_block_dw(v, params, i, bwd_fused, st)) return r;
  return backward_block_pw1(v, params, i, bwd_fused, st);
}

int backward_tail(const Views& v, const float* params, const float* wave, long long wave_stride, float* grads,
                  long long L, hipStream_t st) {
  const Layout& l = v.l; const int B = v.B; const long long T = v.T; const double BT = v.BT();
  const int ldg = v.ldg(); GemmRowsParams g; WgradParams wg;
  memset(&g, 0, sizeof(g));
  g.a = rows_bf16(v.gout(), ldg, T);
  g.W = v.prep + l.p_bott_b; g.T = (int)T; g.Np = l.Np; g.Kp = l.Bnp;
  g.e.out = v.e0(); g.e.ldo = l.Np; g.e.N = l.N;
  g.e.src = v.w(); g.e.ld_src = l.Np; g.e.src_stats = v.stat(0);
  g.e.inv_n = 1.0/((double)T*l.N); g.e.eps = 1e-8f;
  g.e.gamma = params + l.ln_g; g.e.dgamma = v.vg(); g.e.dbeta = v.vg() + l.N;
  g.e.rep_stride = v.ws.vg_stride; g.e.n_rep = kReplicas;
  g.e.sums_out = v.sum(0);
  if (int r = launch_gemm_rows<A_BF16, E_GLN_BWD>(g, B, st, "bottleneck_dgrad", 2.0*BT*(l.Bnp + 2*l.Np))) return r;
  memset(&wg, 0, sizeof(wg));
  wg.g = rows_bf16(v.gout(), ldg, T); wg.h = rows_bf16(v.w(), l.Np, T);
  set_affine(wg.h, v.stat(0), params + l.ln_g, params + l.ln_b, l.N, T);
  wg.B = B; wg.T = (int)T; wg.Gp = l.Bnp; wg.Hp = l.Np;
  wg.out0 = grads + l.bott_w; wg.G0p = l.Bnp; wg.N0 = l.Bn; wg.Kout = l.N; wg.ldo = l.N;
  wg.gbias0 = grads + l.bott_b;
  if (int r = launch_wgrad<A_BF16>(wg, st, "bottleneck_wgrad", 2.0*BT*(l.Bnp + l.Np), 256)) return r;
  CombineParams cb; memset(&cb, 0, sizeof(cb));
  cb.e0 = v.e0(); cb.w = v.w(); cb.dw1 = v.dw1(); cb.dw = v.dwt(); cb.B = B; cb.T = (int)T;
  cb.Cp = l.Np; cb.C = l.N; cb.S = l.S; cb.stats = v.stat(0); cb.sums = v.sum(0);
  cb.inv_n = 1.0/((double)T*l.N); cb.eps = 1e-8f;
  {
    const long long per_item = T*(l.Np/8);
    int gx = (int)((per_item + 1023)/1024);
    if (gx > 2048) gx = 2048;
    if (gx < 1) gx = 1;
    ProfScope prof("gln0_bwd", 0, 2.0*BT*l.Np*(3 + l.S), st);
    hipLaunchKernelGGL(gln0_bwd_combine_kernel, dim3(gx, B), dim3(256), 0, st, cb);
    BRV_HIP_OK(hipGetLastError());
  }
  memset(&wg, 0, sizeof(wg));
  wg.g = rows_bf16(v.dwt(), l.Np, T); wg.h = frames_of(wave, L, l.hop, l.K, wave_stride);
  wg.B = B; wg.T = (int)T; wg.Gp = l.Np; wg.Hp = l.Kfp;
  wg.out0 = grads + l.enc_w; wg.G0p = l.Np; wg.N0 = l.N; wg.Kout = l.K; wg.ldo = l.K;
  if (int r = launch_wgrad<A_FRAMES>(wg, st, "wgrad_enc", 2.0*BT*l.Np + 4.0*B*L, 768)) return r;
  return 0;
}

int backward_causal_block(const Views& v, const float* params, float* grads, int i, hipStream_t st) {
  const Layout& l = v.l; const int B = v.B; const long long T = v.T; const double BT = v.BT();
  const int ldg = v.ldg(); GemmRowsParams g; WgradParams wg;
  const BlockOff& b = l.blk[i];
  const bool has_res = i < l.nb - 1;
  const int dil = 1 << (i % l.layers);
  const int rs0 = has_res ? l.Bnp : 0;
  memset(&wg, 0, sizeof(wg));
  wg.g = rows_bf16(has_res ? v.gout() : v.gskip(), ldg, T);
  wg.h = rows_bf16(v.h2(i), l.Hp, T);
  wg.B = B; wg.T = (int)T; wg.Gp = rs0 + l.Scp; wg.Hp = l.Hp;
  wg.out0 = has_res ? grads + b.res_w : nullptr; wg.out1 = grads + b.skip_w;
  wg.G0p = rs0; wg.N0 = has_res ? l.Bn : 0; wg.N1 = l.Sc; wg.Kout = l.H; wg.ldo = l.H;
  wg.gbias0 = has_res ? grads + b.res_b : nullptr; wg.gbias1 = grads + b.skip_b;
  if (int r = launch_wgrad<A_BF16>(wg, st, "pw2_wgrad", 2.0*BT*(rs0 + l.Scp + l.Hp))) return r;
  memset(&g, 0, sizeof(g));
  g.a = rows_bf16(has_res ? v.gout() : v.gskip(), ldg, T);
  g.W = v.prep + b.p_rs_b; g.T = (int)T; g.Np = l.Hp; g.Kp = rs0 + l.Scp;
  g.e.out = v.eA(); g.e.ldo = l.Hp; g.e.N = l.H;
  if (int r = launch_gemm_rows<A_BF16, E_STORE>(g, B, st, "pw2_dgrad", 2.0*BT*(rs0 + l.Scp + l.Hp))) return r;
  if (int r = cln_backward(v, v.eA(), v.z2(i), params + b.prelu2, params + b.n2_g,
                           v.tab(2 + 2*i), v.eB(0), nullptr, 0, v.vslot(i) + 2*l.H, v.vslot(i) + 3*l.H,
                           v.vslope() + 2 + 2*i, v.ws.vg_stride, B, T, l.Hp, l.H, st)) return r;
  DwParams d; memset(&d, 0, sizeof(d));
  d.z1 = v.h1(i); d.dz2 = v.eB(0); d.e1 = v.eA(); d.B = B; d.T = (int)T; d.Cp = l.Hp; d.C = l.H;
  d.slope1 = v.one(); d.stats1 = v.fake_stats(); d.gamma1 = v.ones(); d.beta1 = v.zeros();
  d.inv_n = 1.0/((double)T*l.H); d.eps = 1e-8f;
  d.taps = params + b.dconv_w; d.dil = dil; d.left = (l.P - 1)*dil;
  d.dgamma1 = v.vscratch(); d.dbeta1 = v.vscratch() + l.Hp;
  d.dtaps = v.vslot(i) + 4*l.H; d.dbias = v.vslot(i) + 4*l.H + (long long)l.H*l.P;
  d.rep_stride = v.ws.vg_stride; d.sums1 = v.scratch_stats();
  if (int r = dispatch_p<DwBwd>(l.P, d, st)) return r;
  if (int r = cln_backward(v, v.eA(), v.z1(i), params + b.prelu1, params + b.n1_g,
                           v.tab(1 + 2*i), v.eB(0), nullptr, 0, v.vslot(i), v.vslot(i) + l.H,
                           v.vslope() + 1 + 2*i, v.ws.vg_stride, B, T, l.Hp, l.H, st)) return r;
  memset(&wg, 0, sizeof(wg));
  wg.g = rows_bf16(v.eB(0), l.Hp, T); wg.h = rows_bf16(v.x(i), l.Bnp, T);
  wg.B = B; wg.T = (int)T; wg.Gp = l.Hp; wg.Hp = l.Bnp;
  wg.out0 = grads + b.conv_w; wg.G0p = l.Hp; wg.N0 = l.H; wg.Kout = l.Bn; wg.ldo = l.Bn;
  wg.gbias0 = grads + b.conv_b;
  if (int r = launch_wgrad<A_BF16>(wg, st, "pw1_wgrad", 2.0*BT*(l.Hp + l.Bnp))) return r;
  memset(&g, 0, sizeof(g));
  g.a = rows_bf16(v.eB(0), l.Hp, T);
  g.W = v.prep + b.p_c1_b; g.T = (int)T; g.Np = l.Bnp; g.Kp = l.Hp;
  g.e.out = v.gout(); g.e.ldo = ldg; g.e.add_in = has_res ? v.gout() : nullptr; g.e.ld_add = ldg;
  if (int r = launch_gemm_rows<A_BF16, E_ADD>(g, B, st, "pw1_dgrad", 2.0*BT*(l.Hp + l.Bnp*(has_res ? 2 : 1)))) return r;
  return 0;
}

int backward_causal_tail(const Views& v, const float* params, const float* wave, long long wave_stride,
                         float* grads, long long L, hipStream_t st) {
  const Layout& l = v.l; const int B = v.B; const long long T = v.T; const double BT = v.BT();
  const int ldg = v.ldg(); GemmRowsParams g; WgradParams wg;
  memset(&wg, 0, sizeof(wg));
  wg.g = rows_bf16(v.gout(), ldg, T); wg.h = rows_bf16(v.wn(), l.Np, T);
  wg.B = B; wg.T = (int)T; wg.Gp = l.Bnp; wg.Hp = l.Np;
  wg.out0 = grads + l.bott_w; wg.G0p = l.Bnp; wg.N0 = l.Bn; wg.Kout = l.N; wg.ldo = l.N;
  wg.gbias0 = grads + l.bott_b;
  if (int r = launch_wgrad<A_BF16>(wg, st, "bottleneck_wgrad", 2.0*BT*(l.Bnp + l.Np))) return r;
  memset(&g, 0, sizeof(g));
  g.a = rows_bf16(v.gout(), ldg, T);
  g.W = v.prep + l.p_bott_b; g.T = (int)T; g.Np = l.Np; g.Kp = l.Bnp;
  g.e.out = v.e0(); g.e.ldo = l.Np; g.e.N = l.N;
  if (int r = launch_gemm_rows<A_BF16, E_STORE>(g, B, st, "bottleneck_dgrad", 2.0*BT*(l.Bnp + l.Np))) return r;
  if (int r = cln_backward(v, v.e0(), v.w(), nullptr, params + l.ln_g, v.tab(0), v.dwt(), v.dw1(), l.S, v.vg(),
                           v.vg() + l.N, nullptr, v.ws.vg_stride, B, T, l.Np, l.N, st)) return r;
  memset(&wg, 0, sizeof(wg));
  wg.g = rows_bf16(v.dwt(), l.Np, T); wg.h = frames_of(wave, L, l.hop, l.K, wave_stride);
  wg.B = B; wg.T = (int)T; wg.Gp = l.Np; wg.Hp = l.Kfp;
  wg.out0 = grads + l.enc_w; wg.G0p = l.Np; wg.N0 = l.N; wg.Kout = l.K; wg.ldo = l.K;
  if (int r = launch_wgrad<A_FRAMES>(wg, st, "wgrad_enc", 2.0*BT*l.Np + 4.0*B*L)) return r;
  return reduce_vector_grads(v, grads, st);
}

int backward_causal(const Views& v, const float* params, const float* wave, long long wave_stride,
                    const float* d_out, float* grads, long long L, hipStream_t st) {
  if (int r = causal_init(v, st)) return r;
  BRV_HIP_OK(hipMemsetAsync(v.vg(), 0, v.ws.vg_bytes, st));
  if (int r = backward_head(v, params, d_out, grads, L, false, st)) return r;
  for (int i = v.l.nb - 1; i >= 0; --i)
    if (int r = backward_causal_block(v, params, grads, i, st)) return r;
  return backward_causal_tail(v, params, wave, wave_stride, grads, L, st);
}

}

extern "C" {

#ifdef BRV_DIAG
int brv_debug_read(long long* out, int64_t n) {
  (void)hipDeviceSynchronize();
  const int r = (int)hipMemcpy(out, debug_buffer(), (size_t)n*8, hipMemcpyDeviceToHost);
  (void)hipMemset(debug_buffer(), 0, 1 << 20);
  return r;
}
#endif

void* brv_prof_create(int by_dilation) {
  Prof* p = new Prof();
  p->by_dil = by_dilation != 0;
  return p;
}
void brv_prof_destroy(void* prof) {
  Prof* p = static_cast<Prof*>(prof);
  if (!p) return;
  for (auto& e : p->entries) { (void)hipEventDestroy(e.a); (void)hipEventDestroy(e.b); }
  delete p;
}

int64_t brv_prof_collect(void* prof, char* buf, int64_t buflen) {
  Prof* p = static_cast<Prof*>(prof);
  if (!p) return 0;
  struct Agg { std::string label; long long calls; double ms, flops, bytes; };
  std::vector<Agg> agg;
  for (auto& e : p->entries) {
    (void)hipEventSynchronize(e.b);
    float ms = 0.f;
    (void)hipEventElapsedTime(&ms, e.a, e.b);
    Agg* a = nullptr;
    for (auto& x : agg) if (x.label == e.label) { a = &x; break; }
    if (!a) { agg.push_back({e.label, 0, 0, 0, 0}); a = &agg.back(); }
    a->calls += 1; a->ms += ms; a->flops += e.flops; a->bytes += e.bytes;
  }
  std::string out;
  char line[256];
  for (auto& a : agg) {
    snprintf(line, sizeof(line), "%s %lld %.6f %.6e %.6e\n", a.label.c_str(), a.calls, a.ms,
             a.flops, a.bytes);
    out += line;
  }
  if ((int64_t)out.size() + 1 <= buflen && buf) {
    memcpy(buf, out.c_str(), out.size() + 1);
    for (auto& e : p->entries) { (void)hipEventDestroy(e.a); (void)hipEventDestroy(e.b); }
    p->entries.clear();
  }
  return (int64_t)out.size() + 1;
}

int64_t brv_ctn_param_count(const brv_ctn_config* cfg) {
  Layout l; if (l.init(cfg)) return -1; return l.n_params;
}
int64_t brv_ctn_param_tensors(const brv_ctn_config* cfg) {
  Layout l; if (l.init(cfg)) return -1; return (int64_t)l.tensor_offsets.size();
}
int64_t brv_ctn_param_offset(const brv_ctn_config* cfg, int64_t index) {
  Layout l; if (l.init(cfg)) return -1;
  BRV_REFUSE(index < 0 || index >= (int64_t)l.tensor_offsets.size(), "index outside [0, brv_ctn_param_tensors)");
  return l.tensor_offsets[index];
}
int64_t brv_ctn_frames(const brv_ctn_config* cfg, int64_t length) {
  Layout l; if (l.init(cfg)) return -1; return l.frames(length);
}
int64_t brv_ctn_prepared_bytes(const brv_ctn_config* cfg) {
  Layout l; if (l.init(cfg)) return -1; return l.n_prepared*2;
}
int64_t brv_ctn_workspace_bytes(const brv_ctn_config* cfg, int64_t batch, int64_t length) {
  Layout l; if (l.init(cfg)) return -1;
  Workspace ws; ws.init(l, batch, l.frames(length));
  return ws.total;
}
int64_t brv_ctn_workspace_offset(const brv_ctn_config* cfg, int64_t batch, int64_t length,
                                 const char* name, int64_t index) {
  Layout l; if (l.init(cfg)) return -1;
  BRV_REFUSE(!name, "null name");
  Workspace ws; ws.init(l, batch, l.frames(length));
  const std::string n(name);
  if (n == "w") return ws.w;
  if (n == "x") return ws.x + ws.x_stride*index;
  if (n == "z1") return ws.z1 + ws.z_stride*index;
  if (n == "z2") return ws.z2 + ws.z_stride*index;
  if (n == "skip") return ws.skip;
  if (n == "m") return ws.m;
  if (n == "y") return ws.y;
  if (n == "stats") return ws.stats + index*batch*kStatStride*8;
  if (n == "sums") return ws.sums + index*batch*kStatStride*8;
  if (n == "dpre") return ws.dpre;
  if (n == "gskip") return ws.gskip;
  if (n == "gout") return ws.gout;
  if (n == "dwt") return ws.dwt;
  if (n == "h1" && l.causal) return ws.h1 + ws.z_stride*index;
  if (n == "h2" && l.causal) return ws.h2 + ws.z_stride*index;
  return fail(-1, "unknown workspace tensor " + n);
}

int brv_ctn_prepare(const brv_ctn_config* cfg, const float* params, void* prepared,
                    const brv_launch_opts* opts, brv_stream_t stream) {
  OptsScope scope(opts);
  if (int r = scope.check()) return r;
  Layout l; if (int r = l.init(cfg)) return r;
  hipStream_t st = (hipStream_t)stream;
  std::vector<PrepJob> jobs;
  const bool fused = l.fused_fwd();
  auto add = [&](long long src, long long dst, int R, int C, int rows, int cols, int ld,
                 int tr) {
    PrepJob j; j.src_off = src; j.dst_off = dst; j.R = R; j.C = C; j.rows = rows;
    j.cols = cols; j.dst_ld = ld; j.tr = tr; j.scale_off = -1; jobs.push_back(j);
  };
  add(l.enc_w, l.p_enc, l.N, l.K, l.Np, l.Kfp, l.Kfp, 0);
  add(l.dec_w, l.p_dec_f, l.N, l.K, l.Kfp, l.Np, l.Np, 1);
  add(l.dec_w, l.p_dec_b, l.N, l.K, l.Np, l.Kfp, l.Kfp, 0);
  add(l.bott_w, l.p_bott_f, l.Bn, l.N, l.Bnp, l.Np, l.Np, 0);
  add(l.bott_w, l.p_bott_b, l.Bn, l.N, l.Np, l.Bnp, l.Bnp, 1);
  for (int i = 0; i < l.nb; ++i) {
    const BlockOff& b = l.blk[i];
    const bool has_res = i < l.nb - 1;
    const int rs0 = has_res ? l.Bnp : 0, rs = rs0 + l.Scp;
    add(b.conv_w, b.p_c1_f, l.H, l.Bn, l.Hp, l.Bnp, l.Bnp, 0);
    add(b.conv_w, b.p_c1_b, l.H, l.Bn, l.Bnp, l.Hp, l.Hp, 1);
    if (has_res) add(b.res_w, b.p_rs_b, l.Bn, l.H, l.Hp, l.Bnp, rs, 1);
    add(b.skip_w, b.p_rs_b + rs0, l.Sc, l.H, l.Hp, l.Scp, rs, 1);
    if (fused) {
      add(has_res ? b.res_w : 0, b.p_rs_g, has_res ? l.Bn : 0, l.H, l.Bnp, l.Hp, l.Hp, 0);
      jobs.back().scale_off = b.n2_g;
      add(b.skip_w, b.p_rs_g + (long long)l.Bnp*l.Hp, l.Sc, l.H, l.Scp, l.Hp, l.Hp, 0);
      jobs.back().scale_off = b.n2_g;
    } else {
      if (has_res) add(b.res_w, b.p_rs_f, l.Bn, l.H, l.Bnp, l.Hp, l.Hp, 0);
      add(b.skip_w, b.p_rs_f + (long long)rs0*l.Hp, l.Sc, l.H, l.Scp, l.Hp, l.Hp, 0);
    }
  }
  for (int s = 0; s < l.S; ++s) {
    add(l.out_w + (long long)s*l.N*l.Sc, l.p_out_f + (long long)s*l.Np*l.Scp,
        l.N, l.Sc, l.Np, l.Scp, l.Scp, 0);
    add(l.out_w + (long long)s*l.N*l.Sc, l.p_out_b + (long long)s*l.Np,
        l.N, l.Sc, l.Scp, l.Np, l.S*l.Np, 1);
  }
  for (size_t i = 0; i < jobs.size(); i += kPrepBatch) {
    PrepBatch pb;
    pb.n = (int)std::min<size_t>(kPrepBatch, jobs.size() - i);
    for (int k = 0; k < pb.n; ++k) {
      const PrepJob& j = jobs[i + k];
      if (j.src_off > 0x7fffffffLL || j.dst_off > 0x7fffffffLL || j.scale_off > 0x7fffffffLL ||
          (j.R | j.C | j.rows | j.cols | j.dst_ld) > 0xffff)
        return fail(-1, "prepare: layout too large for the compact job form");
      PrepJobC& c = pb.jobs[k];
      c.src_off = (int)j.src_off; c.dst_off = (int)j.dst_off; c.scale_off = (int)j.scale_off;
      c.R = (unsigned short)j.R; c.C = (unsigned short)j.C; c.rows = (unsigned short)j.rows;
      c.cols = (unsigned short)j.cols; c.dst_ld = (unsigned short)j.dst_ld; c.tr = (unsigned short)j.tr;
    }
    hipLaunchKernelGGL(prep_weights_kernel, dim3(8, pb.n), dim3(256), 0, st, params,
                       (bf16_t*)prepared, pb);
    BRV_HIP_OK(hipGetLastError());
  }
  std::vector<PackJob> packs;
  auto pack = [&](long long src, long long dst, int N, int K, int nsl) {
    if (N % nsl || K % 16) return;
    PackJob j; j.src_off = src; j.dst_off = dst; j.N = N; j.K = K; j.nsl = nsl; packs.push_back(j);
  };
  for (int i = 0; i < l.nb; ++i) {
    const BlockOff& b = l.blk[i];
    const int rs = (i < l.nb - 1 ? l.Bnp : 0) + l.Scp;
    pack(b.p_c1_f, b.p_c1_fp, l.Hp, l.Bnp, 64);
    pack(b.p_rs_b, b.p_rs_bp, l.Hp, rs, 32);
    if (fused) pack(b.p_rs_g, b.p_rs_gp, l.Bnp + l.Scp, l.Hp, 32);
    else pack(b.p_rs_f, b.p_rs_fp, rs, l.Hp, 32);
  }
  for (size_t i = 0; i < packs.size(); i += 96) {
    PackBatch pb;
    pb.n = (int)std::min<size_t>(96, packs.size() - i);
    for (int k = 0; k < pb.n; ++k) pb.jobs[k] = packs[i + k];
    hipLaunchKernelGGL(pack_frag_kernel, dim3(16, pb.n), dim3(256), 0, st, (bf16_t*)prepared, pb);
    BRV_HIP_OK(hipGetLastError());
  }
  if (fused) {
    LazyPrepParams lp; memset(&lp, 0, sizeof(lp));
    lp.nb = l.nb; lp.H = l.H; lp.Hp = l.Hp; lp.Bn = l.Bn; lp.Sc = l.Sc; lp.Bnp = l.Bnp; lp.Scp = l.Scp;
    for (int i = 0; i < l.nb; ++i) {
      const BlockOff& b = l.blk[i];
      lp.blk[i].res_w = b.res_w; lp.blk[i].res_b = b.res_b; lp.blk[i].skip_w = b.skip_w;
      lp.blk[i].skip_b = b.skip_b; lp.blk[i].beta = b.n2_b; lp.blk[i].wg = b.p_rs_g; lp.blk[i].out = b.p_lazy;
    }
    lp.stamp = reinterpret_cast<int*>((bf16_t*)prepared + l.p_stamp); lp.stamp_value = mode_stamp(fused);
    hipLaunchKernelGGL(lazy_prep_kernel, dim3((l.Bnp + l.Scp + 3)/4, l.nb), dim3(256), 0, st, params,
                       (bf16_t*)prepared, lp);
    BRV_HIP_OK(hipGetLastError());
  } else {
    hipLaunchKernelGGL(stamp_write_kernel, dim3(1), dim3(1), 0, st,
                       reinterpret_cast<int*>((bf16_t*)prepared + l.p_stamp), mode_stamp(fused));
    BRV_HIP_OK(hipGetLastError());
  }
  return 0;
}

int brv_ctn_forward(const brv_ctn_config* cfg, const float* params, const void* prepared,
                    void* workspace, const float* wave, int64_t wave_stride, float* out, int64_t batch,
                    int64_t length, const brv_launch_opts* opts, brv_stream_t stream) {
  OptsScope scope(opts);
  if (int r = scope.check()) return r;
  if (wave_stride != 0 && wave_stride < length) return fail(-1, "wave_stride shorter than the rows");
  Layout l; if (int r = l.init(cfg)) return r;
  hipStream_t st = (hipStream_t)stream;
  const int B = (int)batch; const long long L = length;
  const long long T = l.frames(L);
  if (B < 1 || T < 1) return fail(-1, "empty batch or input shorter than one frame");
  const Views v(l, workspace, prepared, B, T);
  if (l.causal) return forward_causal(v, params, wave, wave_stride, out, L, st);
  if (int r = forward_encoder(v, params, wave, wave_stride, out, L, st)) return r;

  if (l.fused_fwd()) {
    for (int i = 0; i < l.nb; ++i)
      if (int r = forward_block_fused(v, params, i, st)) return r;
    if (int r = forward_skip_combine(v, st)) return r;
  } else {
    for (int i = 0; i < l.nb; ++i)
      if (int r = forward_block_plain(v, params, i, st)) return r;
  }
  return forward_decoder(v, params, out, L, st);
}

static void part_range(int nb, int part, int nparts, int& lo, int& hi) {
  lo = (int)((long long)nb*(nparts - 1 - part)/nparts);
  hi = (int)((long long)nb*(nparts - part)/nparts) - 1;
}

int brv_ctn_grad_bucket(const brv_ctn_config* cfg, int32_t part, int32_t nparts, int64_t* offset,
                        int64_t* count) {
  Layout l; if (int r = l.init(cfg)) return r;
  if (nparts < 1 || part < 0 || part >= nparts || !offset || !count) return fail(-1, "bad part");
  if (l.causal) {
    *offset = 0; *count = part == nparts - 1 ? l.n_params : 0;
    return 0;
  }
  int lo, hi; part_range(l.nb, part, nparts, lo, hi);
  const long long begin = part == nparts - 1 ? 0 : (lo <= hi ? l.blk[lo].conv_w : -1);
  int plo, phi; long long end = l.n_params;
  if (part > 0) {
    int q = part - 1;
    for (;; --q) { part_range(l.nb, q, nparts, plo, phi); if (plo <= phi || q == 0) break; }
    end = plo <= phi ? l.blk[plo].conv_w : l.n_params;
    if (plo > phi) end = l.tcn_prelu;
  }
  if (begin < 0) { *offset = 0; *count = 0; if (part == 0) { *offset = l.tcn_prelu; *count = l.n_params - l.tcn_prelu; } return 0; }
  *offset = begin; *count = end - begin;
  return 0;
}

int brv_ctn_backward(const brv_ctn_config* cfg, const float* params, const void* prepared,
                     void* workspace, const float* wave, int64_t wave_stride, const float* d_out,
                     float* grads, int64_t batch, int64_t length, const brv_launch_opts* opts,
                     brv_stream_t stream) {
  return brv_ctn_backward_part(cfg, params, prepared, workspace, wave, wave_stride, d_out, grads, batch,
                               length, 0, 1, opts, stream);
}

int brv_ctn_backward_part(const brv_ctn_config* cfg, const float* params, const void* prepared,
                          void* workspace, const float* wave, int64_t wave_stride, const float* d_out,
                          float* grads,
                          int64_t batch, int64_t length, int32_t part, int32_t nparts,
                          const brv_launch_opts* opts, brv_stream_t stream) {
  OptsScope scope(opts);
  if (int r = scope.check()) return r;
  Layout l; if (int r = l.init(cfg)) return r;
  hipStream_t st = (hipStream_t)stream;
  const int B = (int)batch; const long long L = length;
  const long long T = l.frames(L);
  if (B < 1 || T < 1) return fail(-1, "empty batch or input shorter than one frame");
  if (nparts < 1 || part < 0 || part >= nparts) return fail(-1, "bad part");
  const Views v(l, workspace, prepared, B, T);
  if (l.causal) {
    if (part != nparts - 1) return 0;
    return backward_causal(v, params, wave, wave_stride, d_out, grads, L, st);
  }
  int blk_lo, blk_hi; part_range(l.nb, part, nparts, blk_lo, blk_hi);
  const bool head = part == 0, tail = part == nparts - 1;
  const bool bwd_fused = l.fused_fwd() && bwd_fuse_requested() && l.Bnp == 128 && l.Scp == 128 &&
                         l.Hp % HL_CG == 0 && !opt(BRV_OPT_NO_DZ_FUSE) && bf_frames_ok(T);
  if (head)
    if (int r = backward_head(v, params, d_out, grads, L, bwd_fused, st)) return r;
  for (int i = blk_hi; i >= blk_lo; --i)
    if (int r = backward_block(v, params, i, bwd_fused, st)) return r;
  if (int r = deferred_wgrads(v, params, grads, blk_lo, blk_hi, st)) return r;
  if (tail)
    if (int r = backward_tail(v, params, wave, wave_stride, grads, L, st)) return r;
  return reduce_vector_grads(v, grads, st, blk_lo, blk_hi, tail, head);
}

}
```

brever_amd/csrc/gemm_rows.cuh:

```cuda
#pragma once
#include "common.cuh"

namespace brv {

enum AKind { A_BF16 = 0, A_F32 = 1, A_FRAMES = 2, A_DZ = 3 };
enum EMode {
  E_STORE = 0,
  E_RES_SKIP = 1,
  E_MASK = 2,
  E_OLA = 3,
  E_GLN_BWD = 4,
  E_ADD = 5,
  E_MASK_BWD = 6,
  E_PRELU_BWD = 7
};

struct ASpec {
  const void* p0; const void* p1;
  int ld0, ld1;
  long long bs0, bs1;
  int K0;
  int nsrc;
  int hop, Kf; long long wav_stride; int wav_len;
  const float* slope;
  const double* stats;
  const float* gamma; const float* beta; int C;
  double inv_n; float eps;
  const double* sums;
  void* xout; const float* lazy_v0; const float* lazy_v1;
  void* z2out; const float* taps; const float* dbias; const float* slope2; double* stats2_out;
  int dil, left;
};

struct EpiSpec {
  void* out; int ldo;
  const float* bias; const float* bias2; int N, Nsplit, N2;
  double* stats_out; const float* stats_slope;
  const bf16_t* res_in; int ld_res; float* skip; int ld_skip; int skip_init;
  const bf16_t* w_in; int ld_w; bf16_t* m_out; int S; int Np_src;
  float* wave_out; int hop, Kf; long long wave_stride; int wave_len;
  const bf16_t* src; int ld_src; const float* src_slope; const double* src_stats;
  double inv_n; float eps;
  const float* gamma; float* dgamma; float* dbeta; double* sums_out;
  long long rep_stride; int n_rep;
  const bf16_t* add_in; int ld_add;
  const bf16_t* m_in; bf16_t* out2;
  const float* src_f32; int ld_srcf; float* dslope;
  const bf16_t* gu_u; int ld_gu; const bf16_t* gu_gskip; int ld_gs; const float* gu_v1; double* gu_out;
};

struct GemmRowsParams {
  ASpec a;
  const bf16_t* W;
  const bf16_t* Wp;
  int wp_nsl;
  int T, Np, Kp;
  int n_ttiles, n_ntiles, batch;
#ifdef BRV_DIAG
  int dbg;
  long long* dbg_out;
#endif
  EpiSpec e;
};

__device__ __forceinline__ int xcd_remap(int id, int nwg) {
  const int xcd = id & 7, slot = id >> 3;
  const int q = nwg >> 3, r = nwg & 7;
  return (xcd < r ? xcd*(q + 1) : r*(q + 1) + (xcd - r)*q) + slot;
}

constexpr int GR_BM = 128;
constexpr int GR_BK = 64;
constexpr int GR_LDS_K = GR_BK + 8;

template <int BN>
struct GemmRowsSmem {
  static constexpr int kMain = (GR_BM + BN)*GR_LDS_K*2;
  static constexpr int kLdc = BN + 4;
  static constexpr int kEpi = GR_BM*kLdc*4;
  static constexpr int kBytes = kMain > kEpi ? kMain : kEpi;
};

template <int BN, int AK, int EM>
__global__ __launch_bounds__(256) void gemm_rows_kernel(const GemmRowsParams p) {
  __shared__ __attribute__((aligned(16))) unsigned char smem[GemmRowsSmem<BN>::kBytes];
  bf16_t* As = reinterpret_cast<bf16_t*>(smem);
  bf16_t* Ws = As + GR_BM*GR_LDS_K;
  float* Cs = reinterpret_cast<float*>(smem);
  constexpr int LDC = GemmRowsSmem<BN>::kLdc;
  constexpr int NT = BN/32;
  constexpr int WCH = BN/32;

  const int tid = threadIdx.x;
  const int lane = tid & 63, wid = tid >> 6;
  const int vid = xcd_remap(blockIdx.x, gridDim.x);
  const int n_tile = vid % p.n_ntiles;
  const int rest = vid / p.n_ntiles;
  const int b = rest / p.n_ttiles;
  const int t0 = (rest % p.n_ttiles)*GR_BM;
  const int n0 = n_tile*BN;
  const int T = p.T;

  const int kc = tid & 7;
  const int arow = tid >> 3;
  const ASpec& a = p.a;

  NormStat ns = {0.f, 1.f};
  const bool affine = AK != A_DZ && a.stats != nullptr;
  if (a.stats != nullptr) ns = norm_stat(a.stats, b, a.inv_n, a.eps);
  const float slope = a.slope ? *a.slope : 1.f;
  const bool has_prelu = AK != A_DZ && a.slope != nullptr;
  float dz_m1 = 0.f, dz_m2 = 0.f, dz_da = 0.f;
  if (AK == A_DZ) {
    dz_m1 = (float)(a.sums[stat_sum(b)]*a.inv_n);
    dz_m2 = (float)(a.sums[stat_sq(b)]*a.inv_n);
  }
  uint4 araw_z[(AK == A_DZ) ? 4 : 1];

  uint4 araw_b[4];
  float araw_f[(AK == A_BF16) ? 1 : 4][8];
  float asc[8], ash[8];
  uint4 wraw[WCH];

  auto load_tile = [&](int kt) {
    const int kbase = kt*GR_BK + kc*8;
    if (AK == A_FRAMES) {
      const float* wav = reinterpret_cast<const float*>(a.p0) + (long long)b*a.wav_stride;
#pragma unroll
      for (int ci = 0; ci < 4; ++ci) {
        const int t = t0 + arow + 32*ci;
#pragma unroll
        for (int j = 0; j < 8; ++j) {
          const int k = kbase + j;
          const long long idx = (long long)t*a.hop + k;
          float v = 0.f;
          if (t < T && k < a.Kf && idx < a.wav_len) v = wav[idx];
          araw_f[(AK == A_BF16) ? 0 : ci][j] = v;
        }
      }
    } else {
      bool first = kbase < a.K0;
      int ld = first ? a.ld0 : a.ld1;
      int kk = first ? kbase : kbase - a.K0;
      long long boff = (long long)b*(first ? a.bs0 : a.bs1);
      if (a.nsrc > 1) {
        first = true; ld = a.ld0;
        const int s = kbase / a.ld0;
        kk = kbase - s*a.ld0;
        boff = ((long long)b*a.nsrc + s)*a.bs0;
      }
#pragma unroll
      for (int ci = 0; ci < 4; ++ci) {
        const int t = t0 + arow + 32*ci;
        const long long off = boff + (long long)t*ld + kk;
        if (AK == A_DZ) {
          const long long o0 = (long long)b*a.bs0 + (long long)t*a.ld0 + kbase;
          const long long o1 = (long long)b*a.bs1 + (long long)t*a.ld1 + kbase;
          araw_b[ci] = (t < T) ? *reinterpret_cast<const uint4*>(reinterpret_cast<const bf16_t*>(a.p0) + o0)
                               : make_uint4(0, 0, 0, 0);
          araw_z[(AK == A_DZ) ? ci : 0] =
              (t < T) ? *reinterpret_cast<const uint4*>(reinterpret_cast<const bf16_t*>(a.p1) + o1)
                      : make_uint4(0, 0, 0, 0);
        } else if (AK == A_BF16) {
          const bf16_t* src = reinterpret_cast<const bf16_t*>(first ? a.p0 : a.p1);
          araw_b[ci] = (t < T) ? *reinterpret_cast<const uint4*>(src + off)
                               : make_uint4(0, 0, 0, 0);
        } else {
          const float* src = reinterpret_cast<const float*>(first ? a.p0 : a.p1);
          float4 lo = make_float4(0, 0, 0, 0), hi = lo;
          if (t < T) {
            lo = *reinterpret_cast<const float4*>(src + off);
            hi = *reinterpret_cast<const float4*>(src + off + 4);
          }
          float* d = araw_f[(AK == A_BF16) ? 0 : ci];
          d[0] = lo.x; d[1] = lo.y; d[2] = lo.z; d[3] = lo.w;
          d[4] = hi.x; d[5] = hi.y; d[6] = hi.z; d[7] = hi.w;
        }
      }
    }
    if (affine) {
      float g8[8], b8[8];
      load8_masked(a.gamma, kbase, a.C, g8);
      load8_masked(a.beta, kbase, a.C, b8);
#pragma unroll
      for (int j = 0; j < 8; ++j) {
        asc[j] = ns.rstd*g8[j];
        ash[j] = b8[j] - ns.mean*ns.rstd*g8[j];
      }
    }
#pragma unroll
    for (int ci = 0; ci < WCH; ++ci) {
      const int c = tid + 256*ci;
      const int wr = c >> 3;
      const int n = n0 + wr;
      wraw[ci] = (n < p.Np)
          ? *reinterpret_cast<const uint4*>(p.W + (long long)n*p.Kp + kt*GR_BK + kc*8)
          : make_uint4(0, 0, 0, 0);
    }
  };

  auto store_tile = [&](int kt) {
#pragma unroll
    for (int ci = 0; ci < 4; ++ci) {
      const int row = arow + 32*ci;
      uint4 q;
      if (AK == A_DZ) {
        float ev[8], zv[8], o[8];
        unpack8(araw_b[ci], ev);
        unpack8(araw_z[(AK == A_DZ) ? ci : 0], zv);
        const int kbase = kt*GR_BK + kc*8;
        const bool live = t0 + row < T;
#pragma unroll
        for (int j = 0; j < 8; ++j) {
          const bool pos = zv[j] > 0.f;
          const float pv = pos ? zv[j] : slope*zv[j];
          const float xh = (pv - ns.mean)*ns.rstd;
          const float dh = ns.rstd*(ev[j] - dz_m1 - xh*dz_m2);
          const bool ok = live && kbase + j < a.C;
          o[j] = ok ? (pos ? dh : slope*dh) : 0.f;
          if (ok && !pos) dz_da += dh*zv[j];
        }
        q = pack8(o);
        if (live)
          *reinterpret_cast<uint4*>(const_cast<bf16_t*>(reinterpret_cast<const bf16_t*>(a.p0))
              + (long long)b*a.bs0 + (long long)(t0 + row)*a.ld0 + kbase) = q;
      } else if (AK == A_BF16 && !affine && !has_prelu) {
        q = araw_b[ci];
      } else {
        float f[8];
        if (AK == A_BF16) unpack8(araw_b[ci], f);
        else {
#pragma unroll
          for (int j = 0; j < 8; ++j) f[j] = araw_f[(AK == A_BF16) ? 0 : ci][j];
        }
        if (has_prelu) {
#pragma unroll
          for (int j = 0; j < 8; ++j) f[j] = prelu(f[j], slope);
        }
        if (affine) {
#pragma unroll
          for (int j = 0; j < 8; ++j) f[j] = f[j]*asc[j] + ash[j];
        }
        if (t0 + row >= T) {
#pragma unroll
          for (int j = 0; j < 8; ++j) f[j] = 0.f;
        }
        q = pack8(f);
      }
      *reinterpret_cast<uint4*>(As + row*GR_LDS_K + kc*8) = q;
    }
#pragma unroll
    for (int ci = 0; ci < WCH; ++ci) {
      const int c = tid + 256*ci;
      *reinterpret_cast<uint4*>(Ws + (c >> 3)*GR_LDS_K + kc*8) = wraw[ci];
    }
  };

  f32x16 acc[NT];
#pragma unroll
  for (int j = 0; j < NT; ++j)
#pragma unroll
    for (int i = 0; i < 16; ++i) acc[j][i] = 0.f;

  const int nk = p.Kp/GR_BK;
  const int fr = lane & 31, fh = lane >> 5;
  load_tile(0);
  for (int kt = 0; kt < nk; ++kt) {
    __syncthreads();
    store_tile(kt);
    __syncthreads();
    if (kt + 1 < nk) load_tile(kt + 1);
#pragma unroll
    for (int s = 0; s < GR_BK/16; ++s) {
      const bf16x8 af = *reinterpret_cast<const bf16x8*>(
          As + (32*wid + fr)*GR_LDS_K + 16*s + 8*fh);
#pragma unroll
      for (int j = 0; j < NT; ++j) {
        const bf16x8 bfr = *reinterpret_cast<const bf16x8*>(
            Ws + (32*j + fr)*GR_LDS_K + 16*s + 8*fh);
        acc[j] = __builtin_amdgcn_mfma_f32_32x32x16_bf16(af, bfr, acc[j], 0, 0, 0);
      }
    }
  }

  __syncthreads();
#pragma unroll
  for (int j = 0; j < NT; ++j)
#pragma unroll
    for (int i = 0; i < 16; ++i) {
      const int row = 32*wid + (i & 3) + 8*(i >> 2) + 4*fh;
      Cs[row*LDC + 32*j + fr] = acc[j][i];
    }
  __syncthreads();

  constexpr int NCH = BN/8;
  constexpr int RG = 256/NCH;
  const int ch = tid % NCH, rg = tid / NCH;
  const int ncol = n0 + ch*8;
  const EpiSpec& e = p.e;
  const bool col_ok = ncol < p.Np;

  if (EM == E_OLA && p.n_ntiles == 1 && e.hop > 0) {
    const int rows = T - t0 < GR_BM ? T - t0 : GR_BM;
    const int hop = e.hop, Kf = e.Kf;
    const int nsamp = (rows - 1)*hop + Kf;
    float* wo = e.wave_out + (long long)b*e.wave_stride;
    const bool first = t0 == 0, last = t0 + rows >= T;
    for (int s = tid; s < nsamp; s += 256) {
      int r_hi = s / hop; if (r_hi > rows - 1) r_hi = rows - 1;
      int r_lo = s - Kf + 1 <= 0 ? 0 : (s - Kf + hop)/hop;
      float acc_s = 0.f;
      for (int r = r_lo; r <= r_hi; ++r) acc_s += Cs[r*LDC + (s - r*hop)];
      const long long idx = (long long)t0*hop + s;
      if (idx >= e.wave_len) continue;
      const bool owned = (first || s >= Kf - hop) && (last || s < rows*hop);
      if (owned) wo[idx] = acc_s; else atomic_add_f32(wo + idx, acc_s);
    }
    return;
  }

  double st_sum = 0.0, st_sq = 0.0;
  float colA[8], colB[8];
#pragma unroll
  for (int j = 0; j < 8; ++j) { colA[j] = 0.f; colB[j] = 0.f; }
  float red_f = 0.f;

  float biasv[8];
#pragma unroll
  for (int j = 0; j < 8; ++j) biasv[j] = 0.f;
  if (EM == E_STORE || EM == E_RES_SKIP) {
    if (EM == E_RES_SKIP && ncol >= e.Nsplit) load8_masked(e.bias2, ncol - e.Nsplit, e.N2, biasv);
    else load8_masked(e.bias, ncol, e.N, biasv);
  }
  int msrc = 0, mf = 0;
  if (EM == E_MASK) {
    msrc = ncol / e.Np_src; mf = ncol % e.Np_src;
    load8_masked(e.bias ? e.bias + msrc*e.N : nullptr, mf, e.N, biasv);
  }
  float guv[(EM == E_ADD) ? 16 : 1];
  if (EM == E_ADD && e.gu_out) {
#pragma unroll
    for (int j = 0; j < 8; ++j) {
      guv[(EM == E_ADD) ? j : 0] = e.gu_v1[ncol + j];
      guv[(EM == E_ADD) ? 8 + j : 0] = e.gu_v1[p.Np + ncol + j];
    }
  }
  NormStat es = {0.f, 1.f};
  float gam[8];
  if (EM == E_GLN_BWD) {
    es = norm_stat(e.src_stats, b, e.inv_n, e.eps);
    load8_masked(e.gamma, ncol, e.N, gam);
  }
  const float eslope = (EM == E_GLN_BWD && e.src_slope) ? *e.src_slope
                     : (EM == E_PRELU_BWD ? *e.src_slope
                     : (EM == E_STORE && e.stats_slope ? *e.stats_slope : 1.f));

  for (int row = rg; row < GR_BM; row += RG) {
    const int t = t0 + row;
    if (t >= T || !col_ok) continue;
    float v[8];
    {
      const float4 lo = *reinterpret_cast<const float4*>(Cs + row*LDC + ch*8);
      const float4 hi = *reinterpret_cast<const float4*>(Cs + row*LDC + ch*8 + 4);
      v[0] = lo.x; v[1] = lo.y; v[2] = lo.z; v[3] = lo.w;
      v[4] = hi.x; v[5] = hi.y; v[6] = hi.z; v[7] = hi.w;
    }
    const long long rowi = (long long)b*T + t;
    if (EM == E_STORE) {
#pragma unroll
      for (int j = 0; j < 8; ++j) v[j] += biasv[j];
      const uint4 q = pack8(v);
      *reinterpret_cast<uint4*>(reinterpret_cast<bf16_t*>(e.out) + rowi*e.ldo + ncol) = q;
      if (e.stats_out) {
        float r[8]; unpack8(q, r);
#pragma unroll
        for (int j = 0; j < 8; ++j) {
          if (ncol + j < e.N) {
            const float pv = e.stats_slope ? prelu(r[j], eslope) : r[j];
            st_sum += pv; st_sq += (double)pv*pv;
          }
        }
      }
    } else if (EM == E_RES_SKIP) {
#pragma unroll
      for (int j = 0; j < 8; ++j) v[j] += biasv[j];
      if (ncol < e.Nsplit) {
        float r[8];
        unpack8(*reinterpret_cast<const uint4*>(e.res_in + rowi*e.ld_res + ncol), r);
#pragma unroll
        for (int j = 0; j < 8; ++j) v[j] += r[j];
        *reinterpret_cast<uint4*>(reinterpret_cast<bf16_t*>(e.out) + rowi*e.ldo + ncol) = pack8(v);
      } else {
        float* sp = e.skip + rowi*e.ld_skip + (ncol - e.Nsplit);
        if (!e.skip_init) {
          const float4 lo = *reinterpret_cast<const float4*>(sp);
          const float4 hi = *reinterpret_cast<const float4*>(sp + 4);
          v[0] += lo.x; v[1] += lo.y; v[2] += lo.z; v[3] += lo.w;
          v[4] += hi.x; v[5] += hi.y; v[6] += hi.z; v[7] += hi.w;
        }
        *reinterpret_cast<float4*>(sp) = make_float4(v[0], v[1], v[2], v[3]);
        *reinterpret_cast<float4*>(sp + 4) = make_float4(v[4], v[5], v[6], v[7]);
      }
    } else if (EM == E_MASK) {
      float w[8], y[8];
      unpack8(*reinterpret_cast<const uint4*>(e.w_in + rowi*e.ld_w + mf), w);
#pragma unroll
      for (int j = 0; j < 8; ++j) {
        const float m = 1.f/(1.f + __expf(-(v[j] + biasv[j])));
        v[j] = m; y[j] = m*w[j];
      }
      const long long orow = ((long long)b*e.S + msrc)*T + t;
      *reinterpret_cast<uint4*>(e.m_out + orow*e.ldo + mf) = pack8(v);
      *reinterpret_cast<uint4*>(reinterpret_cast<bf16_t*>(e.out) + orow*e.ldo + mf) = pack8(y);
    } else if (EM == E_OLA) {
      float* wo = e.wave_out + (long long)b*e.wave_stride;
#pragma unroll
      for (int j = 0; j < 8; ++j) {
        const int n = ncol + j;
        const long long idx = (long long)t*e.hop + n;
        if (n < e.Kf && idx < e.wave_len) atomic_add_f32(wo + idx, v[j]);
      }
    } else if (EM == E_GLN_BWD) {
      float s[8], o[8];
      unpack8(*reinterpret_cast<const uint4*>(e.src + rowi*e.ld_src + ncol), s);
#pragma unroll
      for (int j = 0; j < 8; ++j) {
        const float pv = e.src_slope ? prelu(s[j], eslope) : s[j];
        const float xh = (pv - es.mean)*es.rstd;
        const float ev = gam[j]*v[j];
        o[j] = ev;
        st_sum += ev; st_sq += (double)ev*xh;
        colA[j] += v[j]*xh; colB[j] += v[j];
      }
      *reinterpret_cast<uint4*>(reinterpret_cast<bf16_t*>(e.out) + rowi*e.ldo + ncol) = pack8(o);
    } else if (EM == E_ADD) {
      if (e.add_in) {
        float r[8];
        unpack8(*reinterpret_cast<const uint4*>(e.add_in + rowi*e.ld_add + ncol), r);
#pragma unroll
        for (int j = 0; j < 8; ++j) v[j] += r[j];
// ... 98 lines not shown
```

brever_amd/csrc/gemm_wgrad.cuh:

```cuda
#pragma once
#include "gemm_rows.cuh"
#include "gfx950.cuh"

namespace brv {

struct WgradParams {
  ASpec g;
  ASpec h;
  int B, T;
  int Gp, Hp;
  float* out0; float* out1; int G0p;
  int N0, N1;
  int Kout, ldo;
  float* gbias0; float* gbias1;
  int nsplit;
};

constexpr int kWgMaxProb = 24;
struct WgradProb {
  const void* g0; const void* g1; const void* h;
  float* out0; float* out1; float* gbias0; float* gbias1;
  const float* slope; const double* stats; const float* gamma; const float* beta;
};
struct WgradGroupParams {
  WgradParams base;
  int nprob;
  WgradProb prob[kWgMaxProb];
};

constexpr int WG_BT = 64;
constexpr int WG_BG = 128;

typedef __attribute__((ext_vector_type(8))) short s16x8;

__device__ __forceinline__ bf16x8 tr_frag(const bf16_t* tile, int ld, int row0,
                                          int col0, int lane) {
  const int g4 = lane >> 4, i = lane & 15, q = i >> 2, pp = i & 3;
  const int col = col0 + 16*(g4 & 1) + 4*pp;
  const int row = row0 + 8*(g4 >> 1) + q;
  const bf16_t* p0 = tile + row*ld + col;
#ifndef BRV_WGRAD_SCALAR_FRAG
  const s16x4 lo = lds_read_tr_tracked(p0);
  const s16x4 hi = lds_read_tr_tracked(p0 + 4*ld);
  const s16x8 v = __builtin_shufflevector(lo, hi, 0, 1, 2, 3, 4, 5, 6, 7);
  return __builtin_bit_cast(bf16x8, v);
#else
  const int r = lane & 31, h = lane >> 5;
  s16x8 v;
#pragma unroll
  for (int j = 0; j < 8; ++j) v[j] = (short)tile[(row0 + 8*h + j)*ld + col0 + r];
  return __builtin_bit_cast(bf16x8, v);
#endif
}

template <int BH, int HK>
__global__ __launch_bounds__(256) void gemm_wgrad_kernel(const WgradGroupParams gp) {
  WgradParams p = gp.base;
  int bx = blockIdx.x, by = blockIdx.y, bz = blockIdx.z;
  {
    const int tiles = gridDim.x, pairs = gridDim.y*gridDim.z;
    if ((pairs & 7) == 0) {
      const int L = bx + tiles*(by + (int)gridDim.y*bz);
      const int xcd = L & 7, slot = L >> 3;
      const int pair = (slot / tiles)*8 + xcd;
      bx = slot % tiles; by = pair % (int)gridDim.y; bz = pair / (int)gridDim.y;
    }
  }
  if (gp.nprob > 0) {
    const WgradProb& q = gp.prob[bz];
    p.g.p0 = q.g0; p.g.p1 = q.g1; p.h.p0 = q.h;
    p.out0 = q.out0; p.out1 = q.out1; p.gbias0 = q.gbias0; p.gbias1 = q.gbias1;
    p.h.slope = q.slope; p.h.stats = q.stats; p.h.gamma = q.gamma; p.h.beta = q.beta;
  }
  constexpr int LDG = WG_BG + 32;
  constexpr int LDH = BH + 32;
  constexpr int NT = BH/32;
  constexpr int HCH = BH/32;
  constexpr int HCPR = BH/8;
  __shared__ __attribute__((aligned(16))) bf16_t Gs[WG_BT*LDG];
  __shared__ __attribute__((aligned(16))) bf16_t Hs[WG_BT*LDH];

  const int tid = threadIdx.x, lane = tid & 63, wid = tid >> 6;
  const int n_htiles = p.Hp/BH;
  const int gtile = bx / n_htiles, htile = bx % n_htiles;
  const int n0 = gtile*WG_BG, k0 = htile*BH;
  const int T = p.T;
  const int cpi = ceil_div(T, WG_BT);
  const int total = p.B*cpi;
  const int per = ceil_div(total, p.nsplit);
  const int c_begin = by*per;
  const int c_end = min(total, c_begin + per);

  const int gcc = tid & 15, grow = tid >> 4;
  const int hcc = tid % HCPR, hrow = tid / HCPR;
  constexpr int HRS = 256/HCPR;

  const ASpec& G = p.g;
  const ASpec& H = p.h;
  const int gch = n0 + gcc*8;
  const bool g_first = gch < G.K0;
  const bf16_t* gsrc = reinterpret_cast<const bf16_t*>(g_first ? G.p0 : G.p1);
  const int gld = g_first ? G.ld0 : G.ld1;
  const long long gbs = g_first ? G.bs0 : G.bs1;
  const int gk = g_first ? gch : gch - G.K0;
  const bool g_ok = gch < p.Gp;

  const int hch = k0 + hcc*8;
  const bool h_ok = hch < p.Hp;
  const bool h_aff = H.stats != nullptr;
  const bool h_prelu = H.slope != nullptr;
  const float hslope = h_prelu ? *H.slope : 1.f;
  float hg[8], hb[8];
  load8_masked(h_aff ? H.gamma : nullptr, hch, H.C, hg);
  load8_masked(h_aff ? H.beta : nullptr, hch, H.C, hb);

  uint4 graw[4];
  uint4 hraw_b[HCH];
  float hraw_f[(HK == A_BF16) ? 1 : HCH][8];
  float bias_acc[8];
#pragma unroll
  for (int j = 0; j < 8; ++j) bias_acc[j] = 0.f;

  auto load_chunk = [&](int c) {
    const int b = c / cpi, t0 = (c % cpi)*WG_BT;
#pragma unroll
    for (int ci = 0; ci < 4; ++ci) {
      const int t = t0 + grow + 16*ci;
      graw[ci] = (g_ok && t < T)
          ? *reinterpret_cast<const uint4*>(gsrc + (long long)b*gbs + (long long)t*gld + gk)
          : make_uint4(0, 0, 0, 0);
    }
#pragma unroll
    for (int ci = 0; ci < HCH; ++ci) {
      const int t = t0 + hrow + HRS*ci;
      if (HK == A_BF16) {
        hraw_b[ci] = (h_ok && t < T)
            ? *reinterpret_cast<const uint4*>(reinterpret_cast<const bf16_t*>(H.p0)
                                              + (long long)b*H.bs0 + (long long)t*H.ld0 + hch)
            : make_uint4(0, 0, 0, 0);
      } else if (HK == A_F32) {
        float4 lo = make_float4(0, 0, 0, 0), hi = lo;
        if (h_ok && t < T) {
          const float* s = reinterpret_cast<const float*>(H.p0) + (long long)b*H.bs0 + (long long)t*H.ld0 + hch;
          lo = *reinterpret_cast<const float4*>(s);
          hi = *reinterpret_cast<const float4*>(s + 4);
        }
        float* d = hraw_f[(HK == A_BF16) ? 0 : ci];
        d[0] = lo.x; d[1] = lo.y; d[2] = lo.z; d[3] = lo.w;
        d[4] = hi.x; d[5] = hi.y; d[6] = hi.z; d[7] = hi.w;
      } else {
        const float* wav = reinterpret_cast<const float*>(H.p0) + (long long)b*H.wav_stride;
#pragma unroll
        for (int j = 0; j < 8; ++j) {
          const int k = hch + j;
          const long long idx = (long long)t*H.hop + k;
          float v = 0.f;
          if (t < T && k < H.Kf && idx < H.wav_len) v = wav[idx];
          hraw_f[(HK == A_BF16) ? 0 : ci][j] = v;
        }
      }
    }
  };

  auto store_chunk = [&](int c) {
    const int b = c / cpi, t0 = (c % cpi)*WG_BT;
#pragma unroll
    for (int ci = 0; ci < 4; ++ci) {
      *reinterpret_cast<uint4*>(Gs + (grow + 16*ci)*LDG + gcc*8) = graw[ci];
      if (p.gbias0 || p.gbias1) {
        float f[8]; unpack8(graw[ci], f);
#pragma unroll
        for (int j = 0; j < 8; ++j) bias_acc[j] += f[j];
      }
    }
    NormStat ns = {0.f, 1.f};
    if (h_aff) ns = norm_stat(H.stats, b, H.inv_n, H.eps);
#pragma unroll
    for (int ci = 0; ci < HCH; ++ci) {
      const int row = hrow + HRS*ci;
      uint4 q;
      if (HK == A_BF16 && !h_aff && !h_prelu) {
        q = hraw_b[ci];
      } else {
        float f[8];
        if (HK == A_BF16) unpack8(hraw_b[ci], f);
        else {
#pragma unroll
          for (int j = 0; j < 8; ++j) f[j] = hraw_f[(HK == A_BF16) ? 0 : ci][j];
        }
        if (h_prelu) {
#pragma unroll
          for (int j = 0; j < 8; ++j) f[j] = prelu(f[j], hslope);
        }
        if (h_aff) {
#pragma unroll
          for (int j = 0; j < 8; ++j)
            f[j] = f[j]*(ns.rstd*hg[j]) + (hb[j] - ns.mean*ns.rstd*hg[j]);
        }
        if (t0 + row >= T) {
#pragma unroll
          for (int j = 0; j < 8; ++j) f[j] = 0.f;
        }
        q = pack8(f);
      }
      *reinterpret_cast<uint4*>(Hs + row*LDH + hcc*8) = q;
    }
  };

  f32x16 acc[NT];
#pragma unroll
  for (int j = 0; j < NT; ++j)
#pragma unroll
    for (int i = 0; i < 16; ++i) acc[j][i] = 0.f;

  if (c_begin < c_end) load_chunk(c_begin);
  for (int c = c_begin; c < c_end; ++c) {
    __syncthreads();
    store_chunk(c);
    __syncthreads();
    if (c + 1 < c_end) load_chunk(c + 1);
#pragma unroll
    for (int s = 0; s < WG_BT/16; ++s) {
      const bf16x8 af = tr_frag(Gs, LDG, 16*s, 32*wid, lane);
#pragma unroll
      for (int j = 0; j < NT; ++j) {
        const bf16x8 bfr = tr_frag(Hs, LDH, 16*s, 32*j, lane);
        acc[j] = __builtin_amdgcn_mfma_f32_32x32x16_bf16(af, bfr, acc[j], 0, 0, 0);
      }
    }
  }

  const int fr = lane & 31, fh = lane >> 5;
#pragma unroll
  for (int j = 0; j < NT; ++j) {
    const int k = k0 + 32*j + fr;
#pragma unroll
    for (int i = 0; i < 16; ++i) {
      const int n = n0 + 32*wid + (i & 3) + 8*(i >> 2) + 4*fh;
      if (k < p.Kout) {
        if (n < p.G0p) {
          if (n < p.N0) atomic_add_f32(p.out0 + (long long)n*p.ldo + k, acc[j][i]);
        } else {
          const int n1 = n - p.G0p;
          if (n1 < p.N1) atomic_add_f32(p.out1 + (long long)n1*p.ldo + k, acc[j][i]);
        }
      }
    }
  }
  if ((p.gbias0 || p.gbias1) && htile == 0) {
    __syncthreads();
    float* sc = reinterpret_cast<float*>(Gs);
#pragma unroll
    for (int j = 0; j < 8; ++j) sc[grow*WG_BG + gcc*8 + j] = bias_acc[j];
    __syncthreads();
    if (tid < WG_BG) {
      float s = 0.f;
      for (int r = 0; r < 16; ++r) s += sc[r*WG_BG + tid];
      const int n = n0 + tid;
      if (n < p.G0p) { if (p.gbias0 && n < p.N0) atomic_add_f32(p.gbias0 + n, s); }
      else if (p.gbias1 && n - p.G0p < p.N1) atomic_add_f32(p.gbias1 + (n - p.G0p), s);
    }
  }
}

}
```

brever_amd/hip.py:

```python
import ctypes
import os
import re

import torch

_HERE = os.path.dirname(os.path.abspath(__file__))


class _c_ptr(ctypes.c_void_p):

    @staticmethod
    def from_param(obj, _tensor=torch.Tensor, _void_p=ctypes.c_void_p, _other=ctypes.c_void_p.from_param):
        if isinstance(obj, _tensor):
            return _void_p(obj.data_ptr())
        return _other(obj)


_SCALARS = {'int64_t': ctypes.c_int64, 'int32_t': ctypes.c_int32, 'int': ctypes.c_int,
            'uint32_t': ctypes.c_uint32, 'float': ctypes.c_float}


def _ctype(decl, proto, ret=False):
    m = re.fullmatch(r'\s*(?:const\s+)?(\w+)\s*(\*?)\s*(\w*)\s*', decl)
    base, star, name = m.groups() if m else ('', '', '')
    if star:
        t = ctypes.c_char_p if base == 'char' else ctypes.c_void_p if ret else _c_ptr
        known = not ret or base in ('char', 'void')
    else:
        t = None if base == 'void' else _c_ptr if base == 'brv_stream_t' else _SCALARS.get(base)
        known = base in _SCALARS or base == ('void' if ret else 'brv_stream_t')
    if not known or (ret and name):
        raise RuntimeError(f'{proto}: no ctypes type for {decl.strip()!r}')
    return t


def parse_header(text):
    text = re.sub(r'/\*.*?\*/', ' ', text, flags=re.S)
    text = re.sub(r'//[^\n]*', ' ', text)
    text = re.sub(r'^[ \t]*#(?:.*\\\n)*.*$', ' ', text, flags=re.M)
    table = {}
    for ret, name, args in re.findall(r'([^;{}()]*)\b(brv_\w+)\s*\(([^;{}]*);', text):
        args = args.rstrip()
        if not args.endswith(')') or '(' in args or ')' in args[:-1]:
            raise RuntimeError(f'{name}: cannot split the argument list ({args!r}')
        args = args[:-1].strip()
        argtypes = [] if args in ('', 'void') else [_ctype(a, name) for a in args.split(',')]
        table[name] = (_ctype(ret, name, ret=True), argtypes)
    for name in re.findall(r'\b(brv_\w+)\s*\(', text):
        if name not in table:
            raise RuntimeError(f'{name}: not a prototype the parser can read')
    return table


def parse_constants(text):
    text = re.sub(r'/\*.*?\*/|//[^\n]*', ' ', text, flags=re.S).replace('\\\n', ' ')
    table = {}
    for name, params, value in re.findall(r'^[ \t]*#[ \t]*define[ \t]+(BRV_\w+)(\(?)(.*)$', text, flags=re.M):
        value = value.strip()
        if params or not value:
            continue
        inner = value[1:-1].strip() if value[0] == '(' and value[-1] == ')' else value
        m = re.fullmatch(r'(-?)\s*(0[xX][0-9a-fA-F]+|0|[1-9][0-9]*)[uUlL]*', inner)
        if not m:
            raise RuntimeError(f'{name}: {value!r} is not an integer literal the parser can read')
        table[name] = int(m.group(1) + m.group(2), 0)
    return table


def _extent(text, constants):
    m = re.fullmatch(r'\s*(?:(\d+)|(\d+)\s*\*\s*([A-Za-z_]\w*)|([A-Za-z_]\w*)(?:\s*\+\s*(\d+))?)\s*', text)
    n, k, scaled, plain, more = m.groups() if m else (None,)*5
    if n:
        return int(n)
    if scaled in constants:
        return int(k)*constants[scaled]
    return constants[plain] + int(more or 0) if plain in constants else None


def parse_structs(text, constants):
    text = re.sub(r'/\*.*?\*/|//[^\n]*', ' ', text, flags=re.S)
    text = re.sub(r'^[ \t]*#(?:.*\\\n)*.*$', ' ', text, flags=re.M)
    table = {}
    for tag, body, name in re.findall(r'\btypedef\s+struct\s+(\w+)\s*\{(.*?)\}\s*(\w*)\s*;', text, flags=re.S):
        *decls, rest = body.split(';')
        if name != tag or not tag.startswith('brv_') or '{' in body or rest.strip() or not decls:
            raise RuntimeError(f'struct {tag}: not a `typedef struct brv_x {{ fields; }} brv_x;`')
        fields = []
        for decl in decls:
            m = re.fullmatch(r'\s*(?:const\s+)?(\w+)\b(.*)', decl, flags=re.S)
            base, declarators = m.groups() if m else ('', decl)
            for d in declarators.split(','):
                m = re.fullmatch(r'\s*(\*?)\s*([A-Za-z_]\w*)\s*((?:\[[^\[\]]*\]\s*){0,3})', d)
                star, field, dims = m.groups() if m else ('', d.strip() or decl.strip(), '')
                t = ctypes.c_void_p if star else _SCALARS.get(base) if base != 'int' else None
                if not m or t is None:
                    raise RuntimeError(f'{tag}.{field}: no ctypes type for {decl.strip()!r}')
                for dim in reversed(re.findall(r'\[([^\[\]]*)\]', dims)):
                    n = _extent(dim, constants)
                    if n is None:
                        raise RuntimeError(f'{tag}.{field}: cannot read the array extent [{dim}]')
                    t = t*n
                fields.append((field, t))
        table[tag] = type(tag, (ctypes.Structure,), {'_fields_': fields, '__doc__': f'``{tag}`` of the C header.'})
    for tag in re.findall(r'\bstruct\s+(\w*)', text):
        if tag not in table:
            raise RuntimeError(f'struct {tag}: not a struct definition the parser can read')
    return table


def _header_text(path):
    if not os.path.exists(path):
        raise RuntimeError(f'{path} is missing: the binding is derived from the C header')
    with open(path) as f:
        return f.read()


class Library:

    def __init__(self, header, soname, env, what, last_error=None):
        self.header_path = os.path.join(os.path.dirname(_HERE), 'include', header)
        self.path = os.environ.get(env) or os.path.join(_HERE, 'csrc', soname)
        text = _header_text(self.header_path)
        self.signatures, self.constants = parse_header(text), parse_constants(text)
        self.structs = parse_structs(text, self.constants)
        if last_error is None:
            last_error, = (name for name in self.signatures if name.endswith('_last_error'))
        handle = None

        def lib():
            nonlocal handle
            if handle is None:
                if not os.path.exists(self.path):
                    raise RuntimeError(
                        f'{self.path} is missing: build it with '
                        '`python -c "import __graft_entry__ as g; g.build()"` or '
                        f'`make -C brever_amd/csrc` (needs hipcc, targets gfx950). {what}')
                loaded = ctypes.CDLL(self.path)
                for name, (restype, argtypes) in self.signatures.items():
                    fn = getattr(loaded, name)
                    fn.restype, fn.argtypes = restype, argtypes
                handle = loaded
            return handle

        def message():
            msg = getattr(lib(), last_error)()
            return msg.decode() if msg else ''

        def check(status, what):
            if status != 0:
                raise RuntimeError(f'{what} failed with status {status}: {message()}')

        def call(name, *args):
            status = getattr(handle or lib(), name)(*args)
            if status:
                check(status, name)

        def query(name, *args):
            n = getattr(handle or lib(), name)(*args)
            if n < 0:
                check(int(n), name)
            return n

        self.lib, self.last_error, self.check, self.call, self.query = lib, message, check, call, query


_LIB = Library('brever_hip.h', 'libbrever_hip.so', 'BRV_LIB_PATH',
               'brever_amd has no CPU/PyTorch fallback for its kernels.')
LIB_PATH, HEADER_PATH, SIGNATURES = _LIB.path, _LIB.header_path, _LIB.signatures
lib, last_error, check, call, query = _LIB.lib, _LIB.last_error, _LIB.check, _LIB.call, _LIB.query
CtnConfig, LaunchOpts = _LIB.structs['brv_ctn_config'], _LIB.structs['brv_launch_opts']
DccrnStreamConfig = _LIB.structs['brv_dccrn_stream_config']
DCCRN_STREAM_MAX_LEVELS = _LIB.constants['BRV_DCCRN_STREAM_MAX_LEVELS']
globals().update((name[4:], value) for name, value in _LIB.constants.items() if name.startswith('BRV_OPT_'))

_ENV_FLAGS = (('BRV_FWD_FUSE', OPT_NO_FWD_FUSE, '0'), ('BRV_BWD_FUSE', OPT_NO_BWD_FUSE, '0'),
              ('BRV_NO_WS', OPT_NO_WS, None), ('BRV_DWPW2_WS', OPT_DWPW2_WS, '1'),
              ('BRV_NO_DZ_FUSE', OPT_NO_DZ_FUSE, None), ('BRV_NO_DZ1_FUSE', OPT_NO_DZ1_FUSE, None),
              ('BRV_NO_WGRAD_FULL', OPT_NO_WGRAD_FULL, None), ('BRV_NO_WGRAD_SPLIT', OPT_NO_WGRAD_SPLIT, None),
              ('BRV_PW1_RC', OPT_NO_PW1_RC, '0'), ('BRV_PW1_RC_WGRAD', OPT_PW1_RC_WGRAD, '1'),
              ('BRV_PW1_RC_TILES', OPT_PW1_RC_TILES, '1'), ('BRV_WGRAD_128', OPT_NO_WGRAD_128, '0'))
_RETIRED_SWITCHES = ('BRV_DWPW2_V2', 'BRV_BWD_PERSIST')
_prof = None


def launch_opts(cu_eighths=8):
    for name in _RETIRED_SWITCHES:
        if os.environ.get(name) == '1':
            raise RuntimeError(f'{name}=1: this kernel variant was retired (DESIGN.md 5m / 5n); unset the switch')
    flags = 0
    for name, flag, on_value in _ENV_FLAGS:
        v = os.environ.get(name)
        if v is not None and (on_value is None or v == on_value):
            flags |= flag
    target = os.environ.get('BRV_WG_TARGET')
    return LaunchOpts(ctypes.sizeof(LaunchOpts), flags, int(cu_eighths),
                      int(target) if target else 0, _prof)


def opts_ptr(opts):
    return ctypes.byref(opts)


def require_device(*tensors):
    for t in tensors:
        if t is not None and not t.is_cuda:
            raise RuntimeError(
                'brever_amd kernels run on a ROCm device only; got a '
                f'{t.device} tensor (there is no CPU fallback)'
            )


def ptr(t):
    return None if t is None else ctypes.c_void_p(t.data_ptr())


def stream():
    return ctypes.c_void_p(torch.cuda.current_stream().cuda_stream)


def gemm_f32(a, b, d, batch, M, N, K, lda, ldb, ldd, a_bs, b_bs, d_bs, trans_a, trans_b, kbatch, a_kbs, b_kbs,
             bias, mode):
    if M >= 32 and N >= 32:
        nbytes = lib().brv_gemm_f32_workspace_bytes(batch, M, N, K, trans_a, trans_b, kbatch)
        if nbytes > 0:
            ws = torch.empty(nbytes//4, dtype=torch.float32, device=d.device)
            call('brv_gemm_f32_ws', a, b, d, batch, M, N, K, lda, ldb, ldd, a_bs, b_bs, d_bs, trans_a, trans_b,
                 kbatch, a_kbs, b_kbs, bias, mode, ws, nbytes, stream())
            return
    call('brv_gemm_f32', a, b, d, batch, M, N, K, lda, ldb, ldd, a_bs, b_bs, d_bs, trans_a, trans_b,
         kbatch, a_kbs, b_kbs, bias, mode, stream())


def prof_enable(mode):
    global _prof
    if _prof is not None:
        lib().brv_prof_destroy(_prof)
        _prof = None
    if mode:
        _prof = ctypes.c_void_p(lib().brv_prof_create(1 if mode == 2 else 0))


def profile_collect():
    if _prof is None:
        return {}
    n = lib().brv_prof_collect(_prof, None, 0)
    buf = ctypes.create_string_buffer(int(n) + 16)
    lib().brv_prof_collect(_prof, buf, len(buf))
    out = {}
    for line in buf.value.decode().splitlines():
        label, calls, ms, flops, nbytes = line.split()
        out[label] = dict(calls=int(calls), ms=float(ms), flops=float(flops),
                          bytes=float(nbytes))
    return out
```

include/brever_hip.h:

```cpp
#ifndef BREVER_HIP_H
#define BREVER_HIP_H

#include <stdint.h>

#ifdef __cplusplus
extern "C" {
#endif

typedef void* brv_stream_t;

int brv_version(void);
const char* brv_last_error(void);

void* brv_prof_create(int by_dilation);
int64_t brv_prof_collect(void* prof, char* buf, int64_t buflen);
void brv_prof_destroy(void* prof);

#define BRV_OPT_NO_FWD_FUSE     0x001u
#define BRV_OPT_NO_BWD_FUSE     0x002u
#define BRV_OPT_NO_WS           0x004u
#define BRV_OPT_DWPW2_WS        0x008u
#define BRV_OPT_NO_DZ_FUSE      0x010u
#define BRV_OPT_NO_DZ1_FUSE     0x020u
#define BRV_OPT_NO_WGRAD_FULL   0x040u
#define BRV_OPT_NO_WGRAD_SPLIT  0x080u
#define BRV_OPT_NO_PW1_RC       0x100u
#define BRV_OPT_PW1_RC_WGRAD    0x200u
#define BRV_OPT_PW1_RC_TILES    0x400u
#define BRV_OPT_NO_WGRAD_128   0x1000u
#define BRV_OPT_KNOWN          0x17ffu
typedef struct brv_launch_opts {
  uint32_t size;
  uint32_t flags;
  int32_t cu_eighths;
  int32_t wg_target;
  void* prof;
} brv_launch_opts;

typedef struct brv_ctn_config {
  int32_t filters, filter_length, bottleneck_channels, hidden_channels,
          skip_channels, kernel_size, layers, repeats, output_sources, causal;
} brv_ctn_config;

int64_t brv_ctn_param_count(const brv_ctn_config* cfg);
int64_t brv_ctn_param_tensors(const brv_ctn_config* cfg);
int64_t brv_ctn_param_offset(const brv_ctn_config* cfg, int64_t index);

int64_t brv_ctn_frames(const brv_ctn_config* cfg, int64_t length);

int64_t brv_ctn_prepared_bytes(const brv_ctn_config* cfg);
int64_t brv_ctn_workspace_bytes(const brv_ctn_config* cfg, int64_t batch,
                                int64_t length);
int64_t brv_ctn_workspace_offset(const brv_ctn_config* cfg, int64_t batch,
                                 int64_t length, const char* name, int64_t index);

int brv_ctn_prepare(const brv_ctn_config* cfg, const float* params,
                    void* prepared, const brv_launch_opts* opts, brv_stream_t stream);

int brv_ctn_forward(const brv_ctn_config* cfg, const float* params,
                    const void* prepared, void* workspace, const float* wave,
                    int64_t wave_stride, float* out, int64_t batch, int64_t length,
                    const brv_launch_opts* opts, brv_stream_t stream);

int brv_ctn_backward(const brv_ctn_config* cfg, const float* params,
                     const void* prepared, void* workspace, const float* wave,
                     int64_t wave_stride, const float* d_out, float* grads, int64_t batch,
                     int64_t length, const brv_launch_opts* opts, brv_stream_t stream);

int brv_ctn_backward_part(const brv_ctn_config* cfg, const float* params,
                          const void* prepared, void* workspace, const float* wave,
                          int64_t wave_stride, const float* d_out, float* grads, int64_t batch,
                          int64_t length, int32_t part, int32_t nparts,
                          const brv_launch_opts* opts, brv_stream_t stream);
int brv_ctn_grad_bucket(const brv_ctn_config* cfg, int32_t part, int32_t nparts,
                        int64_t* offset, int64_t* count);

int64_t brv_ctn_f32_workspace_bytes(const brv_ctn_config* cfg, int64_t batch,
                                    int64_t length);
int brv_ctn_f32_forward(const brv_ctn_config* cfg, const float* params,
                        void* workspace, const float* wave, float* out,
                        int64_t batch, int64_t length, brv_stream_t stream);
int brv_ctn_f32_backward(const brv_ctn_config* cfg, const float* params,
                         void* workspace, const float* wave, const float* d_out,
                         float* grads, int64_t batch, int64_t length,
                         brv_stream_t stream);
int brv_ctn_f32_backward_part(const brv_ctn_config* cfg, const float* params,
                              void* workspace, const float* wave, const float* d_out,
                              float* grads, int64_t batch, int64_t length,
                              int32_t part, int32_t nparts, brv_stream_t stream);

int64_t brv_ctn_stream_state_bytes(const brv_ctn_config* cfg);
int64_t brv_ctn_stream_workspace_bytes(const brv_ctn_config* cfg, int64_t n, int64_t hops, int32_t amp);
int brv_ctn_stream_reset(const brv_ctn_config* cfg, void* state, const int32_t* ids, int64_t n,
                         brv_stream_t stream);
int brv_ctn_stream_step(const brv_ctn_config* cfg, const float* params, void* state, const int32_t* ids,
                        int64_t n, const float* x, int64_t hops, float* y, int32_t amp, void* workspace,
                        int64_t workspace_bytes, const brv_launch_opts* opts, brv_stream_t stream);
int brv_ctn_stream_tail(const brv_ctn_config* cfg, const void* state, const int32_t* ids, int64_t n,
                        float* y, brv_stream_t stream);

#define BRV_DCCRN_STREAM_MAX_LEVELS 8
typedef struct brv_dccrn_stream_config {
  int32_t n_fft, hop, levels, kf, kt, sf, pf, opf;
  int32_t st, pt, opt, complex_bn;
  int32_t channels[BRV_DCCRN_STREAM_MAX_LEVELS];
  int32_t lstm_hidden, lstm_layers;
  float eps[2*BRV_DCCRN_STREAM_MAX_LEVELS];
  int64_t off_block[2*BRV_DCCRN_STREAM_MAX_LEVELS][7];
  int64_t off_lstm[4][2][4];
  int64_t off_linear[4];
  const float* run_mean[2*BRV_DCCRN_STREAM_MAX_LEVELS];
  const float* run_var[2*BRV_DCCRN_STREAM_MAX_LEVELS];
} brv_dccrn_stream_config;

int64_t brv_dccrn_stream_state_bytes(const brv_dccrn_stream_config* cfg);
int64_t brv_dccrn_stream_workspace_bytes(const brv_dccrn_stream_config* cfg, int64_t n, int64_t hops,
                                         int32_t amp);
int brv_dccrn_stream_reset(const brv_dccrn_stream_config* cfg, void* state, const int32_t* ids, int64_t n,
                           brv_stream_t stream);
int brv_dccrn_stream_step(const brv_dccrn_stream_config* cfg, const float* params, const float* window,
                          const double* basis, const double* synthesis, void* state, const int32_t* ids,
                          int64_t n, const float* x, int64_t hops, float* y, int32_t amp, void* workspace,
                          int64_t workspace_bytes, const brv_launch_opts* opts, brv_stream_t stream);
int brv_dccrn_stream_tail(const brv_dccrn_stream_config* cfg, const float* params, const float* window,
                          const double* basis, const double* synthesis, void* state, const int32_t* ids,
                          int64_t n, const float* rest, int64_t r, float* y, int32_t amp, void* workspace,
                          int64_t workspace_bytes, const brv_launch_opts* opts, brv_stream_t stream);

int64_t brv_loss_scratch_bytes(int64_t batch, int64_t sources);

int brv_snr_forward(const float* x, const float* y, const int64_t* lengths,
                    int64_t batch, int64_t sources, int64_t length,
                    int64_t stride, void* scratch, float* loss,
                    brv_stream_t stream);
int brv_snr_backward(const float* x, const float* y, const int64_t* lengths,
                     int64_t batch, int64_t sources, int64_t length,
                     int64_t stride, const void* scratch, const float* gscale,
                     float* dx, brv_stream_t stream);
int brv_snr_forward_strided(const float* x, const float* y, int64_t y_batch_stride,
                            int64_t y_source_stride, const int64_t* lengths, int64_t batch,
                            int64_t sources, int64_t length, int64_t stride, void* scratch,
                            float* loss, brv_stream_t stream);
int brv_snr_backward_strided(const float* x, const float* y, int64_t y_batch_stride,
                             int64_t y_source_stride, const int64_t* lengths, int64_t batch,
                             int64_t sources, int64_t length, int64_t stride, const void* scratch,
                             const float* gscale, float* dx, brv_stream_t stream);
int brv_sisnr_forward(const float* x, const float* y, const int64_t* lengths,
                      int64_t batch, int64_t sources, int64_t length,
                      int64_t stride, void* scratch, float* loss,
                      brv_stream_t stream);
int brv_sisnr_backward(const float* x, const float* y, const int64_t* lengths,
                       int64_t batch, int64_t sources, int64_t length,
                       int64_t stride, const void* scratch, const float* gscale,
                       float* dx, brv_stream_t stream);
int brv_mse_forward(const float* x, const float* y, const int64_t* lengths,
                    const float* weight, int64_t batch, int64_t sources,
                    int64_t length, int64_t stride, void* scratch, float* loss,
                    brv_stream_t stream);
int brv_mse_backward(const float* x, const float* y, const int64_t* lengths,
                     const float* weight, int64_t batch, int64_t sources,
                     int64_t length, int64_t stride, const float* gscale,
                     float* dx, brv_stream_t stream);

int64_t brv_stft_frames(int64_t length, int64_t frame_length, int64_t hop_length);
int brv_stft_forward(const float* x, const float* basis, float* spec, int64_t rows,
                     int64_t length, int64_t frame_length, int64_t hop_length,
                     float compression, float scale, brv_stream_t stream);
int brv_istft_backward(const float* spec, const float* inv_basis, const float* window,
                       float* frames_scratch, float* y, int64_t rows, int64_t frames,
                       int64_t frame_length, int64_t hop_length, float compression,
                       float scale, brv_stream_t stream);
int brv_stft_adjoint(const float* dspec, const float* basis, float* frames_scratch, float* dx,
                     int64_t rows, int64_t length, int64_t frame_length, int64_t hop_length,
                     float scale, brv_stream_t stream);
int brv_framed_dft_forward(const float* x, const float* basis, float* spec, int64_t rows,
                           int64_t length, int64_t frame_length, int64_t hop_length,
                           int64_t pad_left, int64_t frames, float compression, float scale,
                           brv_stream_t stream);
int brv_framed_dft_transpose(const float* spec, const float* basis, float* frames_scratch,
                             float* y, int64_t rows, int64_t frames, int64_t frame_length,
                             int64_t hop_length, int64_t pad_left, int64_t out_len,
                             float compression, float scale, brv_stream_t stream);
int brv_dft64_forward(const float* x, const double* basis, float* spec, int64_t rows,
                      int64_t length, int64_t n, int64_t hop, int64_t pad_left, int64_t frames,
                      int64_t bins, float compression, float scale, brv_stream_t stream);
int brv_dft64_synthesis(const float* spec, const double* tbasis, float* frames_out, int64_t rows,
                        int64_t frames, int64_t n, int64_t bins, float compression, float scale,
                        brv_stream_t stream);
int brv_overlap_add(const float* frames_in, const float* window, float* y, int64_t rows,
                    int64_t frames, int64_t n, int64_t hop, int64_t pad_left, int64_t out_len,
                    brv_stream_t stream);
int brv_spec_compress(const float* x, float* y, int64_t n, float compression, float scale,
                      brv_stream_t stream);
int brv_pad_signal(const float* x, float* y, int64_t rows, int64_t length, int64_t left,
                   int64_t out_len, int mode, brv_stream_t stream);
int brv_polar(const float* mag, const float* phase, float* out, int64_t n, brv_stream_t stream);
int brv_mag_phase(const float* x, float* mag, float* phase, int64_t n, brv_stream_t stream);
int brv_spec_compress_backward(const float* x, const float* gy, float* gx, int64_t n,
                               float compression, float scale, brv_stream_t stream);
int brv_matmul_f32(const float* a, const float* b, float* d, int64_t batch, int64_t M,
                   int64_t N, int64_t K, int64_t a_batch_stride, brv_stream_t stream);

int brv_gemm_f32(const float* a, const float* b, float* d, int64_t batch, int64_t M, int64_t N,
                 int64_t K, int64_t lda, int64_t ldb, int64_t ldd, int64_t a_batch_stride,
                 int64_t b_batch_stride, int64_t d_batch_stride, int trans_a, int trans_b,
                 int64_t kbatch, int64_t a_kbatch_stride, int64_t b_kbatch_stride,
                 const float* row_bias, int accumulate, brv_stream_t stream);
int64_t brv_gemm_f32_workspace_bytes(int64_t batch, int64_t M, int64_t N, int64_t K, int trans_a, int trans_b,
                                     int64_t kbatch);
int brv_gemm_f32_ws(const float* a, const float* b, float* d, int64_t batch, int64_t M, int64_t N,
                    int64_t K, int64_t lda, int64_t ldb, int64_t ldd, int64_t a_batch_stride,
                    int64_t b_batch_stride, int64_t d_batch_stride, int trans_a, int trans_b,
                    int64_t kbatch, int64_t a_kbatch_stride, int64_t b_kbatch_stride,
                    const float* row_bias, int accumulate, float* workspace, int64_t workspace_bytes,
                    brv_stream_t stream);
int brv_gemm_bf16(const float* a, const float* b, float* d, int64_t batch, int64_t M, int64_t N,
                  int64_t K, int64_t lda, int64_t ldb, int64_t ldd, int64_t a_batch_stride,
                  int64_t b_batch_stride, int64_t d_batch_stride, int trans_a, int trans_b,
                  int64_t kbatch, int64_t a_kbatch_stride, int64_t b_kbatch_stride,
                  const float* row_bias, int accumulate, brv_stream_t stream);
int brv_gemm_bf16_conv(const float* a, const float* image, float* d, int64_t batch, int64_t M,
                       int64_t N, int64_t K, int64_t lda, int64_t ldd, int64_t a_batch_stride,
                       int64_t image_batch_stride, int64_t d_batch_stride, int trans_a, int trans_b,
                       int64_t kbatch, int64_t a_kbatch_stride, int64_t image_kbatch_stride,
                       const float* row_bias, int accumulate, int mode, int64_t C, int64_t H,
                       int64_t W, int64_t kh, int64_t kw, int64_t sh, int64_t sw, int64_t ph,
                       int64_t pw, int64_t Ho, int64_t Wo, brv_stream_t stream);
int64_t brv_cconv_packed_bytes(int64_t M, int64_t C);
int brv_cconv_pack(const float* wc, void* wp, int64_t M, int64_t C, int64_t m_stride, int64_t c_stride,
                   brv_stream_t stream);
int brv_cconv_pack_complex(const float* wr, const float* wi, const float* br, const float* bi, int64_t R, int64_t C,
                           int64_t Cb, float sign, float* wc, float* bias, void* wp1, int64_t M1, int64_t C1,
                           int64_t m_stride1, int64_t c_stride1, void* wp2, int64_t M2, int64_t C2,
                           int64_t m_stride2, int64_t c_stride2, brv_stream_t stream);
int brv_cconv_rows(const float* in, const float* in2, int64_t in_seg, const void* wp, const float* bias, float* out,
                   float* out2, int64_t out_seg, int64_t B, int64_t C, int64_t M, int64_t Hin, int64_t Win,
                   int32_t transposed, brv_stream_t stream);
int64_t brv_cconv_wgrad_workspace_bytes(int64_t B, int64_t A, int64_t C, int64_t Hs);
int brv_cconv_wgrad(const float* small, const float* small2, const float* big, float* out, void* workspace,
                    int64_t B, int64_t A, int64_t C, int64_t Hs, int64_t Ws, int64_t seg, brv_stream_t stream);
int brv_cconv_rows_bf16(const void* in, const void* in2, int64_t in_seg, const void* wp, const float* bias, float* out,
                        float* out2, int64_t out_seg, int64_t B, int64_t C, int64_t M, int64_t Hin, int64_t Win,
                        int32_t transposed, brv_stream_t stream);
int brv_cconv_wgrad_bf16(const void* small, const void* small2, const void* big, float* out, void* workspace,
                         int64_t B, int64_t A, int64_t C, int64_t Hs, int64_t Ws, int64_t seg, brv_stream_t stream);
int brv_cconv_rows_ex(const void* in, const void* in2, int64_t in_seg, const void* wp, const float* bias, void* out,
                      void* out2, int64_t out_seg, int64_t B, int64_t C, int64_t M, int64_t Hin, int64_t Win,
                      int32_t transposed, int32_t in_bf16, int32_t out_bf16, brv_stream_t stream);
int brv_gemm_bf16_mixed(const void* a, const void* b, void* d, int64_t batch, int64_t M, int64_t N,
                        int64_t K, int64_t lda, int64_t ldb, int64_t ldd, int64_t a_batch_stride,
                        int64_t b_batch_stride, int64_t d_batch_stride, int trans_a, int trans_b,
                        int64_t kbatch, int64_t a_kbatch_stride, int64_t b_kbatch_stride,
                        const float* row_bias, int accumulate, int flags, brv_stream_t stream);
int brv_im2col_bf16(const float* x, void* col, int64_t B, int64_t C, int64_t H, int64_t W, int64_t kh,
                    int64_t kw, int64_t sh, int64_t sw, int64_t ph, int64_t pw, int64_t Ho,
                    int64_t Wo, brv_stream_t stream);
int brv_col2im_bf16(const void* col, const float* bias, float* y, int64_t B, int64_t C, int64_t H,
                    int64_t W, int64_t kh, int64_t kw, int64_t sh, int64_t sw, int64_t ph, int64_t pw,
                    int64_t Ho, int64_t Wo, brv_stream_t stream);

int brv_fbe_power(const float* spec, float* out, int64_t B, int64_t C, int64_t n, brv_stream_t stream);
int brv_compress(const float* x, float* out, int64_t n, int mode, float eps, brv_stream_t stream);
int brv_interaural_coherence(const float* spec, float* out, int64_t B, int64_t bins, int64_t F,
                             float alpha, brv_stream_t stream);
int brv_binaural(const float* spec, float* out, int64_t B, int64_t n, int mode, float eps,
                 brv_stream_t stream);
int brv_col_normalize(float* x, int64_t B, int64_t M, int64_t T, float eps, brv_stream_t stream);
int brv_deltas(const float* x, float* out, int64_t B, int64_t M, int64_t T, brv_stream_t stream);
int brv_irm(const float* fg, const float* bg, float* out, int64_t n, float eps, brv_stream_t stream);
int brv_stack_frames(const float* x, float* out, int64_t B, int64_t nf, int64_t T, int64_t stacks,
                     brv_stream_t stream);
int brv_static_norm(const float* x, const float* mean, const float* stdv, float* out, int64_t B,
                    int64_t rows, int64_t T, brv_stream_t stream);
int brv_cumulative_norm(const float* x, float* out, int64_t nrows, int64_t T, float eps,
                        brv_stream_t stream);
int brv_relu_dropout_forward(const float* x, const float* mask, float* out, int64_t n, float scale,
                             brv_stream_t stream);
int brv_relu_dropout_backward(const float* x, const float* mask, const float* dy, float* dx,
                              int64_t n, float scale, brv_stream_t stream);
int brv_dropout_apply(const float* x, const float* mask, float* out, int64_t n, float scale,
                      brv_stream_t stream);
int brv_sigmoid_forward(const float* x, float* out, int64_t n, brv_stream_t stream);
int brv_sigmoid_backward(const float* y, const float* dy, float* dx, int64_t n, brv_stream_t stream);
int brv_row_sum(const float* x, float* out, int64_t B, int64_t M, int64_t T, brv_stream_t stream);
int brv_masked_mean_spec(const float* spec, const float* mask, float* out, int64_t B, int64_t C,
                         int64_t n, brv_stream_t stream);

int brv_conv2d_forward(const float* x, const float* w, const float* bias, float* y, int64_t B,
                       int64_t Cin, int64_t H, int64_t W, int64_t Cout, int64_t kh, int64_t kw,
                       int64_t sh, int64_t sw, int64_t ph, int64_t pw, int64_t x_batch_stride,
                       int64_t y_batch_stride, int accumulate, float sign, brv_stream_t stream);
int brv_conv_transpose2d_forward(const float* x, const float* w, const float* bias, float* y,
                                 int64_t B, int64_t Cin, int64_t H, int64_t W, int64_t Cout,
                                 int64_t kh, int64_t kw, int64_t sh, int64_t sw, int64_t ph,
                                 int64_t pw, int64_t oph, int64_t opw, int64_t x_batch_stride,
                                 int64_t y_batch_stride, int accumulate, float sign,
                                 brv_stream_t stream);
int brv_batchnorm2d_forward(const float* x, const float* gamma, const float* beta,
                            float* running_mean, float* running_var, const float* prelu_slope,
                            float* y, float* save_mean, float* save_invstd, int64_t B, int64_t C,
                            int64_t HW, float eps, float momentum, int training,
                            brv_stream_t stream);
int brv_lstm_recurrent_forward(const float* gates_in, const float* w_hh, const float* bias,
                               float* y, float* act, float* cs, int64_t B, int64_t T, int64_t H,
                               int64_t groups, brv_stream_t stream);
int brv_conv2d_wgrad(const float* x, const float* dy, float* dw, float* dbias, int64_t B,
                     int64_t Cin, int64_t H, int64_t W, int64_t Cout, int64_t Ho, int64_t Wo,
                     int64_t kh, int64_t kw, int64_t sh, int64_t sw, int64_t ph, int64_t pw,
                     int64_t x_batch_stride, int64_t dy_batch_stride, int accumulate, float sign,
                     brv_stream_t stream);
int brv_batchnorm2d_backward(const float* x, const float* dy, const float* save_mean,
                             const float* save_invstd, const float* gamma, const float* beta,
                             const float* prelu_slope, float* dx, float* dgamma, float* dbeta,
                             float* dslope_partial, int64_t B, int64_t C, int64_t HW,
                             brv_stream_t stream);
int brv_batchnorm2d_forward_bf16(const float* x, const float* gamma, const float* beta,
                                 float* running_mean, float* running_var, const float* prelu_slope,
                                 void* y16, float* save_mean, float* save_invstd, int64_t B, int64_t C,
                                 int64_t HW, float eps, float momentum, int training,
                                 brv_stream_t stream);
int brv_batchnorm2d_backward_bf16(const float* x, const float* dy, const float* save_mean,
                                  const float* save_invstd, const float* gamma, const float* beta,
                                  const float* prelu_slope, void* dx16, float* dgamma, float* dbeta,
                                  float* dslope_partial, float* dx_sums, int64_t B, int64_t C, int64_t HW,
                                  brv_stream_t stream);
int brv_batchnorm2d_forward_bf16io(const void* x16, const float* gamma, const float* beta,
                                   float* running_mean, float* running_var, const float* prelu_slope,
                                   void* y16, float* save_mean, float* save_invstd, int64_t B, int64_t C,
                                   int64_t HW, float eps, float momentum, int training,
                                   brv_stream_t stream);
int brv_batchnorm2d_backward_bf16io(const void* x16, const float* dy, const float* save_mean,
                                    const float* save_invstd, const float* gamma, const float* beta,
                                    const float* prelu_slope, void* dx16, float* dgamma, float* dbeta,
// ... 274 lines not shown
```

Baseline: 2532.

## Fold head/tail weight-gradient GEMMs into grouped launches, store PReLU'd skip in bf16

Several backward-pass changes are bundled here. The skip-combine kernel now also writes a PReLU-applied bf16 copy of the skip sum, which the mask GEMM and output wgrad read in place of the fp32 buffer. The decoder wgrad is deferred out of the head into the tail, and the output and bottleneck wgrads can optionally join the grouped pw1 wgrad launch through per-problem shape tables. Waveform frame loads in the GEMMs use float4 when alignment allows. The aim is fewer small launches and less memory traffic, at the cost of an extra bf16 workspace buffer, a bigger kernel argument block, and more bf16 rounding of the skip activations.

```diff
diff --git a/brever_amd/csrc/convtasnet.hip b/brever_amd/csrc/convtasnet.hip
--- a/brever_amd/csrc/convtasnet.hip
+++ b/brever_amd/csrc/convtasnet.hip
@@ -38,7 +38,7 @@
   }
   ~OptsScope() { t_opts = prev; }
   int check() const {
-    const uint32_t unknown = t_opts->flags & ~BRV_OPT_KNOWN;
+    const uint32_t unknown = t_opts->flags & ~(BRV_OPT_KNOWN | (uint32_t)BRV_OPTX_KNOWN);
     if (!unknown) return 0;
     char bits[16]; snprintf(bits, sizeof(bits), "0x%x", unknown);
     return fail(-1, std::string("unknown option bits ") + bits + " in brv_launch_opts.flags");
@@ -49,6 +49,8 @@
 inline bool bwd_fuse_requested() { return !opt(BRV_OPT_NO_BWD_FUSE); }
 inline bool pw1_rc_requested() { return !opt(BRV_OPT_NO_PW1_RC) && !opt(BRV_OPT_NO_DZ1_FUSE); }
 inline bool pw1_rc_wgrad() { return opt(BRV_OPT_PW1_RC_WGRAD) || opt(BRV_OPT_PW1_RC_TILES); }
+inline bool wgrad_riders_requested() { return !opt(BRV_OPTX_NO_WGRAD_RIDERS); }
+inline bool wgrad_ride_pw1_requested() { return opt(BRV_OPTX_WGRAD_RIDE_PW1) && wgrad_riders_requested(); }
 
 struct ProfEntry { const char* label; hipEvent_t a, b; double flops, bytes; };
 struct Prof { std::vector<ProfEntry> entries; bool by_dil; };
@@ -81,6 +83,7 @@
   }
   bool fused_fwd() const { return fusable() && fwd_fuse_requested(); }
   bool pw1_rc() const { return !causal && Hp == RC_H && Bnp == RC_N && pw1_rc_requested(); }
+  bool bf16_skip() const { return fused_fwd() && wgrad_riders_requested(); }
 
   static int limits(const brv_ctn_config* c) {
     return c->kernel_size < 1 || c->kernel_size > 5 ? fail(-2, "kernel_size must be in [1, 5] in the HIP path") : 0;
@@ -126,6 +129,7 @@
   long long vg_stride, vg_bytes;
   long long x_stride, z_stride;
   long long u, u_stride;
+  long long skipb;
   long long stamp;
   long long stats_bytes;
   void init(const Layout& l, long long B, long long T) {
@@ -161,6 +165,7 @@
     wgpart = take((long long)2*kWgSplit*l.nb*W2_G*l.H*4);
     u_stride = align_up(BT*(l.Bnp + l.Scp)*2, 256);
     u = l.fusable() ? take(u_stride*l.nb) : 0;
+    skipb = l.fusable() ? take(BT*l.Scp*2) : 0;
     stamp = take(256);
     h1 = h2 = wn = ctab = cfs = cbt = ident = fake_stats = scratch_stats = 0; ctab_stride = 0;
     if (l.causal) {
@@ -196,6 +201,7 @@
   bf16_t* z2(int i) const { return bf(ws.z2 + ws.z_stride*i); }
   bf16_t* u(int i) const { return bf(ws.u + ws.u_stride*i); }
   float* skip() const { return f32(ws.skip); }
+  bf16_t* skipb() const { return bf(ws.skipb); }
   bf16_t* m() const { return bf(ws.m); }
   bf16_t* y() const { return bf(ws.y); }
   bf16_t* dpre() const { return bf(ws.dpre); }
@@ -254,6 +260,7 @@
 #endif
 
 inline int mode_stamp(bool fused_fwd) { return fused_fwd ? 0x46555345 : 0x504c4149; }
+inline int ws_stamp(const Layout& l) { return mode_stamp(l.fused_fwd()) + (l.bf16_skip() ? 1 : 0); }
 __global__ void stamp_write_kernel(int* dst, int value) { *dst = value; }
 __global__ void stamp_check_f64_kernel(const int* stamp, int expect, double* poison, long long n) {
   if (*stamp == expect) return;
@@ -371,7 +378,14 @@
   WgradParams& p = gp.base;
   const int nprob = gp.nprob > 0 ? gp.nprob : 1;
   const int tiles = ceil_div(p.Gp, WG_BG)*(p.Hp/BH);
-  const int total = p.B*ceil_div(p.T, WG_BT);
+  int minB = p.B;
+  for (int i = 0; i < gp.nprob; ++i) {
+    const WgradShape& s = gp.shape[i];
+    if (s.Hp % BH != 0 || ceil_div((int)s.Gp, WG_BG)*(s.Hp/BH) != tiles)
+      return fail(-1, "wgrad: the problems of a grouped launch need the same tile count");
+    minB = std::min(minB, (int)s.B);
+  }
+  const int total = minB*ceil_div(p.T, WG_BT);
   int ns = ceil_div(target > 0 ? target : 384, tiles*nprob);
   if (target < 0) {
     int nb = p.B;
@@ -386,13 +400,41 @@
   BRV_HIP_OK(hipGetLastError());
   return 0;
 }
+bool wgrad_shape_of(const WgradParams& p, WgradShape& s) {
+  const long long hbs = p.h.hop > 0 ? p.h.wav_stride : p.h.bs0;
+  const long long big = std::max({(long long)p.B, (long long)p.Gp, (long long)p.Hp, (long long)p.G0p, (long long)p.N0,
+                                  (long long)p.N1, (long long)p.Kout, (long long)p.ldo, (long long)p.g.ld0,
+                                  (long long)p.g.ld1, (long long)p.h.ld0, (long long)p.h.C});
+  if (big > 0xffff || p.g.bs0 > 0xffffffffLL || hbs > 0xffffffffLL || p.g.bs0 < 0 || hbs < 0) return false;
+  if (p.g.p1 != nullptr && p.g.bs1 != (long long)p.T*p.g.ld1) return false;
+  s.inv_n = p.h.inv_n; s.gbs0 = (unsigned int)p.g.bs0; s.hbs = (unsigned int)hbs;
+  s.Gp = p.Gp; s.Hp = p.Hp; s.G0p = p.G0p; s.N0 = p.N0; s.N1 = p.N1; s.Kout = p.Kout; s.ldo = p.ldo;
+  s.gld0 = p.g.ld0; s.gld1 = p.g.ld1; s.hld = p.h.ld0; s.C = p.h.C; s.B = p.B;
+  return true;
+}
+bool wgrad_add_prob(WgradGroupParams& gp, const WgradParams& p) {
+  if (gp.nprob >= kWgMaxGroup || !wgrad_shape_of(p, gp.shape[gp.nprob])) return false;
+  WgradProb& q = gp.prob[gp.nprob++];
+  q.g0 = p.g.p0; q.g1 = p.g.p1; q.h = p.h.p0; q.out0 = p.out0; q.out1 = p.out1;
+  q.gbias0 = p.gbias0; q.gbias1 = p.gbias1;
+  q.slope = p.h.slope; q.stats = p.h.stats; q.gamma = p.h.gamma; q.beta = p.h.beta;
+  if (p.h.stats) gp.base.h.eps = p.h.eps;
+  return true;
+}
+
 template <int HK>
 int launch_wgrad_group(WgradGroupParams& gp, hipStream_t st, const char* label,
-                       double bytes, int target_dflt = 384) {
+                       double bytes, int target_dflt = 384, int nbase = -1, double xflops = 0, double xbytes = 0) {
   const WgradParams& p = gp.base;
   if (p.T <= 0 || p.B <= 0) return 0;
   const int nprob = gp.nprob > 0 ? gp.nprob : 1;
-  ProfScope prof(label, 2.0*nprob*p.B*p.T*(double)p.Gp*p.Hp, bytes*nprob, st);
+  if (nbase < 0) nbase = gp.nprob;
+  for (int i = 0; i < nbase; ++i) {
+    WgradParams one = p; one.g.p1 = gp.prob[i].g1;
+    if (!wgrad_shape_of(one, gp.shape[i])) return fail(-1, "wgrad: dimensions too large for a grouped launch");
+  }
+  const int nb1 = gp.nprob > 0 ? nbase : 1;
+  ProfScope prof(label, 2.0*nb1*p.B*p.T*(double)p.Gp*p.Hp + xflops, bytes*nb1 + xbytes, st);
   if (p.Hp % 64 != 0) return fail(-1, "wgrad: unpadded dims");
   const int target = wgrad_target(label, target_dflt);
   if (p.Hp % 128 == 0) return launch_wgrad_t<128, HK>(gp, st, target);
@@ -499,6 +541,7 @@
   ASpec a; memset(&a, 0, sizeof(a));
   a.p0 = wav; a.hop = hop; a.Kf = K; a.wav_stride = stride > 0 ? stride : L; a.wav_len = (int)L;
   a.K0 = 1 << 30; a.nsrc = 1;
+  a.wav_vec = wgrad_riders_requested() ? 1 : 0;
   return a;
 }
 
@@ -569,6 +612,7 @@
   const double* stats; long long stats_stride;
   const bf16_t* prepared; long long lazy_off[kWgMaxProb];
   float* skip; int nb, B, T, Bnp, Scp; double inv_n; float eps;
+  bf16_t* skipb; const float* slope;
 };
 __global__ __launch_bounds__(256) void skip_combine_kernel(const SkipCombineParams p) {
   __shared__ float rs[kWgMaxProb];
@@ -633,6 +677,12 @@
     float* dst = p.skip + ((long long)b*p.T + t)*p.Scp + c0;
     *reinterpret_cast<float4*>(dst) = make_float4(acc[0], acc[1], acc[2], acc[3]);
     *reinterpret_cast<float4*>(dst + 4) = make_float4(acc[4], acc[5], acc[6], acc[7]);
+    if (p.skipb) {
+      const float slope = *p.slope;
+#pragma unroll
+      for (int j = 0; j < 8; ++j) acc[j] = prelu(acc[j], slope);
+      *reinterpret_cast<uint4*>(p.skipb + ((long long)b*p.T + t)*p.Scp + c0) = pack8(acc);
+    }
   }
 }
 
@@ -727,7 +777,7 @@
   const Layout& l = v.l; const int B = v.B; const long long T = v.T; const double BT = v.BT();
   if (int r = launch_call_init(v.stat(0), (long long)(v.ws.stats_bytes/8), out, (long long)B*l.S*L*(long long)sizeof(float),
                                reinterpret_cast<const int*>(v.prep + l.p_stamp), mode_stamp(l.fused_fwd()),
-                               reinterpret_cast<int*>(v.base + v.ws.stamp), mode_stamp(l.fused_fwd()), st))
+                               reinterpret_cast<int*>(v.base + v.ws.stamp), ws_stamp(l), st))
     return fail(r, "forward: call_init launch");
 
   GemmRowsParams g;
@@ -811,15 +861,16 @@
   return 0;
 }
 
-int forward_skip_combine(const Views& v, hipStream_t st) {
+int forward_skip_combine(const Views& v, const float* params, hipStream_t st) {
   const Layout& l = v.l; const int B = v.B; const long long T = v.T; const double BT = v.BT();
   SkipCombineParams sc; memset(&sc, 0, sizeof(sc));
   sc.u = v.u(0); sc.u_stride = v.ws.u_stride/2; sc.stats = v.stat(0); sc.stats_stride = (long long)B*kStatStride;
   sc.prepared = v.prep; sc.skip = v.skip(); sc.nb = l.nb; sc.B = B; sc.T = (int)T; sc.Bnp = l.Bnp; sc.Scp = l.Scp;
   sc.inv_n = 1.0/((double)T*l.H); sc.eps = 1e-8f;
   for (int i = 0; i < l.nb; ++i) sc.lazy_off[i] = l.blk[i].p_lazy;
+  if (l.bf16_skip()) { sc.skipb = v.skipb(); sc.slope = params + l.tcn_prelu; }
   {
-    ProfScope prof("skip_combine", 0, 2.0*BT*l.Scp*l.nb + 4.0*BT*l.Scp, st);
+    ProfScope prof("skip_combine", 0, 2.0*BT*l.Scp*l.nb + (sc.skipb ? 6.0 : 4.0)*BT*l.Scp, st);
     int gx = (int)((T*(l.Scp/8) + 255)/256);
     if (gx > 128) gx = 128;
     hipLaunchKernelGGL(skip_combine_kernel, dim3(gx, B), dim3(256), 0, st, sc);
@@ -870,11 +921,15 @@
   const Layout& l = v.l; const int B = v.B; const long long T = v.T; const double BT = v.BT();
   GemmRowsParams g;
   memset(&g, 0, sizeof(g));
-  g.a = rows_bf16(v.skip(), l.Scp, T);
-  g.a.slope = params + l.tcn_prelu;
+  const bool bf16_skip = l.bf16_skip();
+  g.a = rows_bf16(bf16_skip ? (const void*)v.skipb() : (const void*)v.skip(), l.Scp, T);
+  if (!bf16_skip) g.a.slope = params + l.tcn_prelu;
   g.W = v.prep + l.p_out_f; g.T = (int)T; g.Np = l.S*l.Np; g.Kp = l.Scp;
   g.e.out = v.y(); g.e.ldo = l.Np; g.e.bias = params + l.out_b; g.e.N = l.N;
   g.e.w_in = v.w(); g.e.ld_w = l.Np; g.e.m_out = v.m(); g.e.S = l.S; g.e.Np_src = l.Np;
+  if (bf16_skip) {
+    if (int r = launch_gemm_rows<A_BF16, E_MASK>(g, B, st, "mask_fwd", 2.0*BT*l.Scp + 2.0*BT*l.Np*(1 + 2*l.S))) return r;
+  } else
   if (int r = launch_gemm_rows<A_F32, E_MASK>(g, B, st, "mask_fwd", 4.0*BT*l.Scp + 2.0*BT*l.Np*(1 + 2*l.S))) return r;
   memset(&g, 0, sizeof(g));
   g.a = rows_bf16(v.y(), l.Np, T);
@@ -1016,7 +1071,49 @@
   return 0;
 }
 
-int wgrad_pw1(const Views& v, const float* params, float* grads, int i0, int n, hipStream_t st) {
+WgradParams bottleneck_wgrad_prob(const Views& v, const float* params, float* grads) {
+  const Layout& l = v.l; const long long T = v.T;
+  WgradParams wg; memset(&wg, 0, sizeof(wg));
+  wg.g = rows_bf16(v.gout(), v.ldg(), T); wg.h = rows_bf16(v.w(), l.Np, T);
+  set_affine(wg.h, v.stat(0), params + l.ln_g, params + l.ln_b, l.N, T);
+  wg.B = v.B; wg.T = (int)T; wg.Gp = l.Bnp; wg.Hp = l.Np;
+  wg.out0 = grads + l.bott_w; wg.G0p = l.Bnp; wg.N0 = l.Bn; wg.Kout = l.N; wg.ldo = l.N;
+  wg.gbias0 = grads + l.bott_b;
+  return wg;
+}
+WgradParams out_wgrad_prob(const Views& v, const float* params, float* grads, int s, bool bf16_h) {
+  const Layout& l = v.l; const long long T = v.T;
+  WgradParams wg; memset(&wg, 0, sizeof(wg));
+  wg.g = rows_bf16(v.dpre() + (long long)s*T*l.Np, l.Np, T); wg.g.bs0 = (long long)l.S*T*l.Np;
+  if (bf16_h) wg.h = rows_bf16(v.skipb(), l.Scp, T);
+  else { wg.h = rows_bf16(v.skip(), l.Scp, T); wg.h.slope = params + l.tcn_prelu; }
+  wg.B = v.B; wg.T = (int)T; wg.Gp = l.Np; wg.Hp = l.Scp;
+  wg.out0 = grads + l.out_w + (long long)s*l.N*l.Sc; wg.G0p = l.Np; wg.N0 = l.N;
+  wg.Kout = l.Sc; wg.ldo = l.Sc; wg.gbias0 = grads + l.out_b + (long long)s*l.N;
+  return wg;
+}
+
+struct WgradRiders {
+  bool out, bott;
+  int count(int S) const { return (out ? S : 0) + (bott ? 1 : 0); }
+};
+WgradRiders wgrad_riders(const Layout& l, int blk_lo, int blk_hi, bool head, bool tail) {
+  WgradRiders r = {false, false};
+  const int n = blk_hi - blk_lo + 1;
+  auto tiles = [](int Gp, int Hp) { return ceil_div(Gp, WG_BG)*(Hp/128); };
+  if (!wgrad_ride_pw1_requested() || l.causal || n < 1 || n > kWgMaxProb || (l.pw1_rc() && pw1_rc_wgrad()) ||
+      l.Bnp % 128 != 0 || l.Np % 128 != 0 || l.Scp % 128 != 0)
+    return r;
+  const int t1 = tiles(l.Hp, l.Bnp);
+  r.out = head && l.bf16_skip() && tiles(l.Np, l.Scp) == t1;
+  r.bott = tail && tiles(l.Bnp, l.Np) == t1;
+  if (n + r.count(l.S) > kWgMaxGroup) r.out = false;
+  if (n + r.count(l.S) > kWgMaxGroup) r.bott = false;
+  return r;
+}
+
+int wgrad_pw1(const Views& v, const float* params, float* grads, int i0, int n, hipStream_t st,
+              WgradRiders riders = {false, false}) {
   const Layout& l = v.l; const int B = v.B; const long long T = v.T; const double BT = v.BT();
   WgradGroupParams gp;
   memset(&gp, 0, sizeof(gp));
@@ -1055,13 +1152,27 @@
     hipLaunchKernelGGL(pw1_wgrad_rc_kernel, dim3(tiles, ns, n), dim3(256), 0, st, rp);
     BRV_HIP_OK(hipGetLastError());
   }
-  else
-  if (int r = launch_wgrad_group<A_BF16>(gp, st, "pw1_wgrad", 2.0*BT*(l.Hp + l.Bnp), -1))
-    return r;
-  return 0;
-}
-
-int deferred_wgrads(const Views& v, const float* params, float* grads, int blk_lo, int blk_hi, hipStream_t st) {
+  else {
+    double xflops = 0, xbytes = 0;
+    bool ok = true;
+    if (riders.out)
+      for (int s = 0; s < l.S; ++s) {
+        ok = ok && wgrad_add_prob(gp, out_wgrad_prob(v, params, grads, s, true));
+        xflops += 2.0*BT*(double)l.Np*l.Scp; xbytes += 2.0*BT*(l.Np + l.Scp);
+      }
+    if (riders.bott) {
+      ok = ok && wgrad_add_prob(gp, bottleneck_wgrad_prob(v, params, grads));
+      xflops += 2.0*BT*(double)l.Bnp*l.Np; xbytes += 2.0*BT*(l.Bnp + l.Np);
+    }
+    if (!ok) return fail(-1, "wgrad: a rider does not fit the grouped launch");
+    if (int r = launch_wgrad_group<A_BF16>(gp, st, "pw1_wgrad", 2.0*BT*(l.Hp + l.Bnp), -1, n, xflops, xbytes))
+      return r;
+  }
+  return 0;
+}
+
+int deferred_wgrads(const Views& v, const float* params, float* grads, int blk_lo, int blk_hi, hipStream_t st,
+                    WgradRiders riders = {false, false}) {
   const Layout& l = v.l;
   const bool full_rs = l.Bnp == 128 && l.Scp == 128 && l.Hp % W2_BH == 0 && l.nb <= kWgMaxProb &&
                        !opt(BRV_OPT_NO_WGRAD_FULL);
@@ -1071,18 +1182,27 @@
     const int n = std::min(kWgMaxProb, blk_hi + 1 - i0);
     if (!full_rs)
       if (int r = wgrad_rs_grouped(v, params, grads, i0, n, st)) return r;
-    if (int r = wgrad_pw1(v, params, grads, i0, n, st)) return r;
-  }
-  return 0;
+    if (int r = wgrad_pw1(v, params, grads, i0, n, st, riders)) return r;
+  }
+  return 0;
+}
+
+WgradParams dec_wgrad_prob(const Views& v, const float* d_out, float* grads, long long L) {
+  const Layout& l = v.l; const long long T = v.T;
+  WgradParams wg; memset(&wg, 0, sizeof(wg));
+  wg.g = rows_bf16(v.y(), l.Np, T); wg.h = frames_of(d_out, L, l.hop, l.K);
+  wg.B = v.B*l.S; wg.T = (int)T; wg.Gp = l.Np; wg.Hp = l.Kfp;
+  wg.out0 = grads + l.dec_w; wg.G0p = l.Np; wg.N0 = l.N; wg.Kout = l.K; wg.ldo = l.K;
+  return wg;
 }
 
 int backward_head(const Views& v, const float* params, const float* d_out, float* grads, long long L,
-                  bool bwd_fused, hipStream_t st) {
+                  bool bwd_fused, hipStream_t st, bool ride_out = false, bool defer_dec = false) {
   const Layout& l = v.l; const int B = v.B; const long long T = v.T; const double BT = v.BT();
   const int BS = B*l.S, ldg = v.ldg(); GemmRowsParams g; WgradParams wg;
   if (!l.causal)
     if (int r = launch_call_init(v.sum(0), (long long)(v.ws.stats_bytes/8), v.vg(), (long long)v.ws.vg_bytes,
-                                 reinterpret_cast<const int*>(v.base + v.ws.stamp), mode_stamp(l.fused_fwd()), nullptr, 0, st))
+                                 reinterpret_cast<const int*>(v.base + v.ws.stamp), ws_stamp(l), nullptr, 0, st))
       return fail(r, "backward: call_init launch");
   memset(&g, 0, sizeof(g));
   g.a = frames_of(d_out, L, l.hop, l.K);
@@ -1090,11 +1210,10 @@
   g.e.out = v.dpre(); g.e.ldo = l.Np; g.e.out2 = v.dw1(); g.e.w_in = v.w(); g.e.ld_w = l.Np;
   g.e.m_in = v.m(); g.e.S = l.S;
   if (int r = launch_gemm_rows<A_FRAMES, E_MASK_BWD>(g, BS, st, "dec_bwd", 4.0*BS*L + 2.0*BT*l.Np*(1 + 3*l.S))) return r;
-  memset(&wg, 0, sizeof(wg));
-  wg.g = rows_bf16(v.y(), l.Np, T); wg.h = frames_of(d_out, L, l.hop, l.K);
-  wg.B = BS; wg.T = (int)T; wg.Gp = l.Np; wg.Hp = l.Kfp;
-  wg.out0 = grads + l.dec_w; wg.G0p = l.Np; wg.N0 = l.N; wg.Kout = l.K; wg.ldo = l.K;
-  if (int r = launch_wgrad<A_FRAMES>(wg, st, "wgrad_dec", 2.0*BT*l.S*l.Np + 4.0*BS*L, l.causal ? 384 : 768)) return r;
+  if (!defer_dec) {
+    wg = dec_wgrad_prob(v, d_out, grads, L);
+    if (int r = launch_wgrad<A_FRAMES>(wg, st, "wgrad_dec", 2.0*BT*l.S*l.Np + 4.0*BS*L, l.causal ? 384 : 768)) return r;
+  }
   memset(&g, 0, sizeof(g));
   g.a = rows_bf16(v.dpre(), l.Np, T); g.a.nsrc = l.S;
   g.W = v.prep + l.p_out_b; g.T = (int)T; g.Np = l.Scp; g.Kp = l.S*l.Np;
@@ -1113,13 +1232,12 @@
     hipLaunchKernelGGL(gu_dots_kernel, dim3(gx, B), dim3(256), 0, st, gu);
     BRV_HIP_OK(hipGetLastError());
   }
-  for (int s = 0; s < l.S; ++s) {
-    memset(&wg, 0, sizeof(wg));
-    wg.g = rows_bf16(v.dpre() + (long long)s*T*l.Np, l.Np, T); wg.g.bs0 = (long long)l.S*T*l.Np;
-    wg.h = rows_bf16(v.skip(), l.Scp, T); wg.h.slope = params + l.tcn_prelu;
-    wg.B = B; wg.T = (int)T; wg.Gp = l.Np; wg.Hp = l.Scp;
-    wg.out0 = grads + l.out_w + (long long)s*l.N*l.Sc; wg.G0p = l.Np; wg.N0 = l.N;
-    wg.Kout = l.Sc; wg.ldo = l.Sc; wg.gbias0 = grads + l.out_b + (long long)s*l.N;
+  for (int s = 0; s < l.S && !ride_out; ++s) {
+    const bool bf16_h = l.bf16_skip();
+    wg = out_wgrad_prob(v, params, grads, s, bf16_h);
+    if (bf16_h) {
+      if (int r = launch_wgrad<A_BF16>(wg, st, "wgrad_out", 2.0*BT*l.Np + 2.0*BT*l.Scp, 256)) return r;
+    } else
     if (int r = launch_wgrad<A_F32>(wg, st, "wgrad_out", 2.0*BT*l.Np + 4.0*BT*l.Scp, l.causal ? 384 : 256)) return r;
   }
   return 0;
@@ -1261,7 +1379,7 @@
 }
 
 int backward_tail(const Views& v, const float* params, const float* wave, long long wave_stride, float* grads,
-                  long long L, hipStream_t st) {
+                  long long L, hipStream_t st, bool ride_bott, const float* dec_d_out) {
   const Layout& l = v.l; const int B = v.B; const long long T = v.T; const double BT = v.BT();
   const int ldg = v.ldg(); GemmRowsParams g; WgradParams wg;
   memset(&g, 0, sizeof(g));
@@ -1274,13 +1392,10 @@
   g.e.rep_stride = v.ws.vg_stride; g.e.n_rep = kReplicas;
   g.e.sums_out = v.sum(0);
   if (int r = launch_gemm_rows<A_BF16, E_GLN_BWD>(g, B, st, "bottleneck_dgrad", 2.0*BT*(l.Bnp + 2*l.Np))) return r;
-  memset(&wg, 0, sizeof(wg));
-  wg.g = rows_bf16(v.gout(), ldg, T); wg.h = rows_bf16(v.w(), l.Np, T);
-  set_affine(wg.h, v.stat(0), params + l.ln_g, params + l.ln_b, l.N, T);
-  wg.B = B; wg.T = (int)T; wg.Gp = l.Bnp; wg.Hp = l.Np;
-  wg.out0 = grads + l.bott_w; wg.G0p = l.Bnp; wg.N0 = l.Bn; wg.Kout = l.N; wg.ldo = l.N;
-  wg.gbias0 = grads + l.bott_b;
-  if (int r = launch_wgrad<A_BF16>(wg, st, "bottleneck_wgrad", 2.0*BT*(l.Bnp + l.Np), 256)) return r;
+  if (!ride_bott) {
+    wg = bottleneck_wgrad_prob(v, params, grads);
+    if (int r = launch_wgrad<A_BF16>(wg, st, "bottleneck_wgrad", 2.0*BT*(l.Bnp + l.Np), 256)) return r;
+  }
   CombineParams cb; memset(&cb, 0, sizeof(cb));
   cb.e0 = v.e0(); cb.w = v.w(); cb.dw1 = v.dw1(); cb.dw = v.dwt(); cb.B = B; cb.T = (int)T;
   cb.Cp = l.Np; cb.C = l.N; cb.S = l.S; cb.stats = v.stat(0); cb.sums = v.sum(0);
@@ -1298,6 +1413,14 @@
   wg.g = rows_bf16(v.dwt(), l.Np, T); wg.h = frames_of(wave, L, l.hop, l.K, wave_stride);
   wg.B = B; wg.T = (int)T; wg.Gp = l.Np; wg.Hp = l.Kfp;
   wg.out0 = grads + l.enc_w; wg.G0p = l.Np; wg.N0 = l.N; wg.Kout = l.K; wg.ldo = l.K;
+  if (dec_d_out) {
+    WgradGroupParams gp; gp.base = wg; gp.nprob = 0;
+    const double BS = (double)B*l.S;
+    if (!wgrad_add_prob(gp, wg) || !wgrad_add_prob(gp, dec_wgrad_prob(v, dec_d_out, grads, L)))
+      return fail(-1, "wgrad: the encoder / decoder pair does not fit a grouped launch");
+    return launch_wgrad_group<A_FRAMES>(gp, st, "wgrad_enc", 0, 2*768, 0, 2.0*BT*(1 + l.S)*(double)l.Np*l.Kfp,
+                                        2.0*BT*l.Np*(1 + l.S) + 4.0*(B + BS)*L);
+  }
   if (int r = launch_wgrad<A_FRAMES>(wg, st, "wgrad_enc", 2.0*BT*l.Np + 4.0*B*L, 768)) return r;
   return 0;
 }
@@ -1473,6 +1596,7 @@
   if (n == "z1") return ws.z1 + ws.z_stride*index;
   if (n == "z2") return ws.z2 + ws.z_stride*index;
   if (n == "skip") return ws.skip;
+  if (n == "skipb" && l.fusable()) return ws.skipb;
   if (n == "m") return ws.m;
   if (n == "y") return ws.y;
   if (n == "stats") return ws.stats + index*batch*kStatStride*8;
@@ -1603,7 +1727,7 @@
   if (l.fused_fwd()) {
     for (int i = 0; i < l.nb; ++i)
       if (int r = forward_block_fused(v, params, i, st)) return r;
-    if (int r = forward_skip_combine(v, st)) return r;
+    if (int r = forward_skip_combine(v, params, st)) return r;
   } else {
     for (int i = 0; i < l.nb; ++i)
       if (int r = forward_block_plain(v, params, i, st)) return r;
@@ -1668,13 +1792,16 @@
   const bool head = part == 0, tail = part == nparts - 1;
   const bool bwd_fused = l.fused_fwd() && bwd_fuse_requested() && l.Bnp == 128 && l.Scp == 128 &&
                          l.Hp % HL_CG == 0 && !opt(BRV_OPT_NO_DZ_FUSE) && bf_frames_ok(T);
+  const WgradRiders riders = wgrad_riders(l, blk_lo, blk_hi, head, tail);
+  const bool defer_dec = head && tail && wgrad_riders_requested();
   if (head)
-    if (int r = backward_head(v, params, d_out, grads, L, bwd_fused, st)) return r;
+    if (int r = backward_head(v, params, d_out, grads, L, bwd_fused, st, riders.out, defer_dec)) return r;
   for (int i = blk_hi; i >= blk_lo; --i)
     if (int r = backward_block(v, params, i, bwd_fused, st)) return r;
-  if (int r = deferred_wgrads(v, params, grads, blk_lo, blk_hi, st)) return r;
+  if (int r = deferred_wgrads(v, params, grads, blk_lo, blk_hi, st, riders)) return r;
   if (tail)
-    if (int r = backward_tail(v, params, wave, wave_stride, grads, L, st)) return r;
+    if (int r = backward_tail(v, params, wave, wave_stride, grads, L, st, riders.bott, defer_dec ? d_out : nullptr))
+      return r;
   return reduce_vector_grads(v, grads, st, blk_lo, blk_hi, tail, head);
 }
 
diff --git a/brever_amd/csrc/gemm_rows.cuh b/brever_amd/csrc/gemm_rows.cuh
--- a/brever_amd/csrc/gemm_rows.cuh
+++ b/brever_amd/csrc/gemm_rows.cuh
@@ -21,7 +21,7 @@
   long long bs0, bs1;
   int K0;
   int nsrc;
-  int hop, Kf; long long wav_stride; int wav_len;
+  int hop, Kf; long long wav_stride; int wav_len, wav_vec;
   const float* slope;
   const double* stats;
   const float* gamma; const float* beta; int C;
@@ -126,16 +126,26 @@
     const int kbase = kt*GR_BK + kc*8;
     if (AK == A_FRAMES) {
       const float* wav = reinterpret_cast<const float*>(a.p0) + (long long)b*a.wav_stride;
+      const bool vec = a.wav_vec && ((reinterpret_cast<unsigned long long>(a.p0) | (unsigned long long)a.wav_stride*4 |
+                                      (unsigned long long)a.hop*4) & 15) == 0;
 #pragma unroll
       for (int ci = 0; ci < 4; ++ci) {
         const int t = t0 + arow + 32*ci;
-#pragma unroll
-        for (int j = 0; j < 8; ++j) {
-          const int k = kbase + j;
-          const long long idx = (long long)t*a.hop + k;
-          float v = 0.f;
-          if (t < T && k < a.Kf && idx < a.wav_len) v = wav[idx];
-          araw_f[(AK == A_BF16) ? 0 : ci][j] = v;
+        float* d = araw_f[(AK == A_BF16) ? 0 : ci];
+        const long long idx0 = (long long)t*a.hop + kbase;
+        if (vec && t < T && kbase + 7 < a.Kf && idx0 + 7 < a.wav_len) {
+          const float4 lo = *reinterpret_cast<const float4*>(wav + idx0);
+          const float4 hi = *reinterpret_cast<const float4*>(wav + idx0 + 4);
+          d[0] = lo.x; d[1] = lo.y; d[2] = lo.z; d[3] = lo.w;
+          d[4] = hi.x; d[5] = hi.y; d[6] = hi.z; d[7] = hi.w;
+        } else {
+#pragma unroll
+          for (int j = 0; j < 8; ++j) {
+            const int k = kbase + j;
+            float v = 0.f;
+            if (t < T && k < a.Kf && idx0 + j < a.wav_len) v = wav[idx0 + j];
+            d[j] = v;
+          }
         }
       }
     } else {
diff --git a/brever_amd/csrc/gemm_wgrad.cuh b/brever_amd/csrc/gemm_wgrad.cuh
--- a/brever_amd/csrc/gemm_wgrad.cuh
+++ b/brever_amd/csrc/gemm_wgrad.cuh
@@ -22,11 +22,19 @@
   float* out0; float* out1; float* gbias0; float* gbias1;
   const float* slope; const double* stats; const float* gamma; const float* beta;
 };
+struct WgradShape {
+  double inv_n;
+  unsigned int gbs0, hbs;
+  unsigned short Gp, Hp, G0p, N0, N1, Kout, ldo, gld0, gld1, hld, C, B;
+};
+constexpr int kWgMaxGroup = kWgMaxProb + 3;
 struct WgradGroupParams {
   WgradParams base;
   int nprob;
-  WgradProb prob[kWgMaxProb];
-};
+  WgradProb prob[kWgMaxGroup];
+  WgradShape shape[kWgMaxGroup];
+};
+static_assert(sizeof(WgradGroupParams) <= 4096, "kernel arguments are limited to 4 KB");
 
 constexpr int WG_BT = 64;
 constexpr int WG_BG = 128;
@@ -71,6 +79,11 @@
     p.g.p0 = q.g0; p.g.p1 = q.g1; p.h.p0 = q.h;
     p.out0 = q.out0; p.out1 = q.out1; p.gbias0 = q.gbias0; p.gbias1 = q.gbias1;
     p.h.slope = q.slope; p.h.stats = q.stats; p.h.gamma = q.gamma; p.h.beta = q.beta;
+    const WgradShape& s = gp.shape[bz];
+    p.B = s.B; p.Gp = s.Gp; p.Hp = s.Hp; p.G0p = s.G0p; p.N0 = s.N0; p.N1 = s.N1;
+    p.Kout = s.Kout; p.ldo = s.ldo;
+    p.g.ld0 = s.gld0; p.g.bs0 = s.gbs0; p.g.ld1 = s.gld1; p.g.bs1 = (long long)p.T*s.gld1;
+    p.h.ld0 = s.hld; p.h.bs0 = s.hbs; p.h.wav_stride = s.hbs; p.h.C = s.C; p.h.inv_n = s.inv_n;
   }
   constexpr int LDG = WG_BG + 32;
   constexpr int LDH = BH + 32;
@@ -113,6 +126,10 @@
   float hg[8], hb[8];
   load8_masked(h_aff ? H.gamma : nullptr, hch, H.C, hg);
   load8_masked(h_aff ? H.beta : nullptr, hch, H.C, hb);
+
+  const bool frames_vec = HK == A_FRAMES && H.wav_vec &&
+                          ((reinterpret_cast<unsigned long long>(H.p0) | (unsigned long long)H.wav_stride*4 |
+                            (unsigned long long)H.hop*4) & 15) == 0;
 
   uint4 graw[4];
   uint4 hraw_b[HCH];
@@ -150,13 +167,21 @@
         d[4] = hi.x; d[5] = hi.y; d[6] = hi.z; d[7] = hi.w;
       } else {
         const float* wav = reinterpret_cast<const float*>(H.p0) + (long long)b*H.wav_stride;
-#pragma unroll
-        for (int j = 0; j < 8; ++j) {
-          const int k = hch + j;
-          const long long idx = (long long)t*H.hop + k;
-          float v = 0.f;
-          if (t < T && k < H.Kf && idx < H.wav_len) v = wav[idx];
-          hraw_f[(HK == A_BF16) ? 0 : ci][j] = v;
+        float* d = hraw_f[(HK == A_BF16) ? 0 : ci];
+        const long long idx0 = (long long)t*H.hop + hch;
+        if (frames_vec && t < T && hch + 7 < H.Kf && idx0 + 7 < H.wav_len) {
+          const float4 lo = *reinterpret_cast<const float4*>(wav + idx0);
+          const float4 hi = *reinterpret_cast<const float4*>(wav + idx0 + 4);
+          d[0] = lo.x; d[1] = lo.y; d[2] = lo.z; d[3] = lo.w;
+          d[4] = hi.x; d[5] = hi.y; d[6] = hi.z; d[7] = hi.w;
+        } else {
+#pragma unroll
+          for (int j = 0; j < 8; ++j) {
+            const int k = hch + j;
+            float v = 0.f;
+            if (t < T && k < H.Kf && idx0 + j < H.wav_len) v = wav[idx0 + j];
+            d[j] = v;
+          }
         }
       }
     }
diff --git a/brever_amd/hip.py b/brever_amd/hip.py
--- a/brever_amd/hip.py
+++ b/brever_amd/hip.py
@@ -179,6 +179,20 @@
               ('BRV_NO_WGRAD_FULL', OPT_NO_WGRAD_FULL, None), ('BRV_NO_WGRAD_SPLIT', OPT_NO_WGRAD_SPLIT, None),
               ('BRV_PW1_RC', OPT_NO_PW1_RC, '0'), ('BRV_PW1_RC_WGRAD', OPT_PW1_RC_WGRAD, '1'),
               ('BRV_PW1_RC_TILES', OPT_PW1_RC_TILES, '1'), ('BRV_WGRAD_128', OPT_NO_WGRAD_128, '0'))
+
+
+def parse_ext_options(text):
+    text = re.sub(r'/\*.*?\*/|//[^\n]*', ' ', text, flags=re.S)
+    body = re.search(r'enum\s+brv_opt_ext\s*\{(.*?)\}', text, flags=re.S)
+    if not body:
+        raise RuntimeError('enum brv_opt_ext is missing from the header')
+    return {name: int(value, 0) for name, value in re.findall(r'(BRV_OPTX_\w+)\s*=\s*(0[xX][0-9a-fA-F]+|\d+)', body.group(1))}
+
+
+with open(HEADER_PATH) as _f:
+    EXT_OPTIONS = parse_ext_options(_f.read())
+globals().update((name[4:], value) for name, value in EXT_OPTIONS.items())
+_ENV_EXT_FLAGS = (('BRV_WGRAD_RIDERS', OPTX_NO_WGRAD_RIDERS, '0'), ('BRV_WGRAD_RIDE_PW1', OPTX_WGRAD_RIDE_PW1, '1'))
 _RETIRED_SWITCHES = ('BRV_DWPW2_V2', 'BRV_BWD_PERSIST')
 _prof = None
 
@@ -188,7 +202,7 @@
         if os.environ.get(name) == '1':
             raise RuntimeError(f'{name}=1: this kernel variant was retired (DESIGN.md 5m / 5n); unset the switch')
     flags = 0
-    for name, flag, on_value in _ENV_FLAGS:
+    for name, flag, on_value in _ENV_FLAGS + _ENV_EXT_FLAGS:
         v = os.environ.get(name)
         if v is not None and (on_value is None or v == on_value):
             flags |= flag
diff --git a/include/brever_hip.h b/include/brever_hip.h
--- a/include/brever_hip.h
+++ b/include/brever_hip.h
@@ -29,6 +29,11 @@
 #define BRV_OPT_PW1_RC_TILES    0x400u
 #define BRV_OPT_NO_WGRAD_128   0x1000u
 #define BRV_OPT_KNOWN          0x17ffu
+enum brv_opt_ext {
+  BRV_OPTX_NO_WGRAD_RIDERS = 0x8000,
+  BRV_OPTX_WGRAD_RIDE_PW1 = 0x10000,
+  BRV_OPTX_KNOWN = 0x18000
+};
 typedef struct brv_launch_opts {
   uint32_t size;
   uint32_t flags;
```

New measurement: 2537 (median of 2 runs). About the same (+0.2%).
